# tomershay100/mp3-steganography-lib

Hardware: AMD Instinct MI355X
Metric: MP3 frames/sec (decode+re-encode) @44.1kHz stereo 128kbps, 1→8 GPU (higher is better)
Workload: dtype f64 (decode) / int32 (encode); 1 GPU; 10000-frame full decode->stego-embed->re-encode pipeline per MI355X (BASELINE configs[2]); MP3 main data + side info resident in HBM, MP3 frames out; the message cursor chain is decided and the serial chains of the rate loop are checked on the device inside every step; frames_per_gpu=10000, channels=2, message_bits=536, chain_verdict_units_to_redo=0, message_variant_entries=1874, parallelism=frames sharded over 1 GPU(s), no collective

## Files before the change

mp3-steganography-lib_amd/csrc/k_chain.hpp:

```cpp
#pragma once

namespace mp3s {

constexpr int CH_THREADS = 256;

struct ChainEl { int reset, tables, last[4]; };

__device__ __forceinline__ ChainEl chain_identity() { return ChainEl{0, 0, {-1, -1, -1, -1}}; }
__device__ __forceinline__ ChainEl chain_combine(const ChainEl &l, const ChainEl &r)
{
    if (r.reset) return r;
    ChainEl o;
    o.reset = l.reset;
    o.tables = l.tables + r.tables;
#pragma unroll
    for (int k = 0; k < 4; k++) o.last[k] = r.last[k] >= 0 ? r.last[k] : l.last[k];
    return o;
}
__device__ __forceinline__ ChainEl chain_shfl_up(const ChainEl &x, int d)
{
    ChainEl o;
    o.reset = __shfl_up(x.reset, d, 64);
    o.tables = __shfl_up(x.tables, d, 64);
#pragma unroll
    for (int k = 0; k < 4; k++) o.last[k] = __shfl_up(x.last[k], d, 64);
    return o;
}

__device__ __forceinline__ ChainEl chain_block_scan(ChainEl x, ChainEl (&wave_tot)[CH_THREADS / 64], ChainEl *total)
{
    const int lane = threadIdx.x & 63, wave = threadIdx.x >> 6;
#pragma unroll
    for (int d = 1; d < 64; d <<= 1) {
        const ChainEl o = chain_shfl_up(x, d);
        if (lane >= d) x = chain_combine(o, x);
    }
    __syncthreads();
    if (lane == 63) wave_tot[wave] = x;
    __syncthreads();
    ChainEl pre = chain_identity();
#pragma unroll
    for (int w = 0; w < CH_THREADS / 64; w++) {
        if (w < wave) pre = chain_combine(pre, wave_tot[w]);
    }
    x = chain_combine(pre, x);
    if (total) {
        ChainEl t = wave_tot[0];
#pragma unroll
        for (int w = 1; w < CH_THREADS / 64; w++) t = chain_combine(t, wave_tot[w]);
        *total = t;
    }
    return x;
}

__device__ __forceinline__ ChainEl chain_element(const mp3s_gr_out *__restrict__ gr, const mp3s_rate_frame *__restrict__ rf,
                                                 const mp3s_chain_seg *__restrict__ segs, int f, int n_frames)
{
    ChainEl e = chain_identity();
    if (f >= n_frames) return e;
    e.reset = segs[rf[f].stream].first_frame == f ? 1 : 0;
#pragma unroll
    for (int k = 0; k < 4; k++) {
        const mp3s_gr_out &g = gr[(long)f * 4 + k];
        if (g.flags & MP3S_RF_ACTIVE) { e.tables += g.n_tables; e.last[k] = f * 4 + k; }
    }
    return e;
}

__global__ __launch_bounds__(CH_THREADS) void k_chain_sum(const mp3s_gr_out *__restrict__ gr, const mp3s_rate_frame *__restrict__ rf,
                                                          const mp3s_chain_seg *__restrict__ segs, int n_frames,
                                                          ChainEl *__restrict__ agg, int32_t *__restrict__ verdict,
                                                          mp3s_chain_seg_out *__restrict__ seg_out, int32_t *__restrict__ redo,
                                                          const int32_t *__restrict__ only_after)
{
    __shared__ ChainEl wave_tot[CH_THREADS / 64];
    if (only_after && only_after[0] == 0) {
        if (redo && blockIdx.x == 0 && threadIdx.x == 0) redo[0] = 0;
        return;
    }
    const int f = blockIdx.x * CH_THREADS + threadIdx.x;
    if (f == 0) { verdict[0] = 0; verdict[1] = 0; }
    if (redo) {
        if (f == 0) redo[0] = 0;
        if (f == 0 && !only_after) redo[REDO_WORDS] = 0;
    }
    if (f < n_frames && segs[rf[f].stream].first_frame == f) seg_out[rf[f].stream].carry_used = 0;
    ChainEl total;
    chain_block_scan(chain_element(gr, rf, segs, f, n_frames), wave_tot, &total);
    if (threadIdx.x == 0) agg[blockIdx.x] = total;
}

__global__ __launch_bounds__(CH_THREADS) void k_chain_apply(mp3s_gr_out *__restrict__ gr, const mp3s_rate_frame *__restrict__ rf,
                                                            const mp3s_chain_seg *__restrict__ segs, int n_frames,
                                                            const ChainEl *__restrict__ agg, int32_t *__restrict__ cursor_in,
                                                            const int32_t *__restrict__ state_in, int32_t *__restrict__ verdict,
                                                            mp3s_chain_seg_out *__restrict__ seg_out, int32_t *__restrict__ redo_list,
                                                            const int32_t *__restrict__ only_after)
{
    if (only_after && only_after[0] == 0) return;
    __shared__ ChainEl wave_tot[CH_THREADS / 64];
    const int f = blockIdx.x * CH_THREADS + threadIdx.x;
    ChainEl before = chain_identity();
    for (int c0 = 0; c0 < (int)blockIdx.x; c0 += CH_THREADS) {
        const int j = c0 + (int)threadIdx.x;
        ChainEl total;
        chain_block_scan(j < (int)blockIdx.x ? agg[j] : chain_identity(), wave_tot, &total);
        before = chain_combine(before, total);
    }
    const ChainEl own_el = chain_element(gr, rf, segs, f, n_frames);
    const ChainEl incl = chain_block_scan(own_el, wave_tot, nullptr);
    ChainEl excl = chain_shfl_up(incl, 1);
    if ((threadIdx.x & 63) == 0) {
        excl = chain_identity();
        for (int w = 0; w < (int)(threadIdx.x >> 6); w++) excl = chain_combine(excl, wave_tot[w]);
    }
    excl = chain_combine(before, excl);
    int redo_here = 0, err_here = 0;
    if (f < n_frames) {
        const int s = rf[f].stream;
        const mp3s_chain_seg sg = segs[s];
        const bool first = sg.first_frame == f;
        if (first) excl = chain_identity();
        long cur = (long)sg.hide_begin + excl.tables;
        const long end = sg.hide_end;
        const bool hiding = sg.hide_end > sg.hide_base;
        int carry_used = first && cur < end ? 1 : 0;
#pragma unroll
        for (int k = 0; k < 4; k++) {
            const long u = (long)f * 4 + k;
            mp3s_gr_out &g = gr[u];
            int32_t ch[4];
            const bool own = excl.last[k] >= 0;
            if (own) {
                const mp3s_gr_out &p = gr[excl.last[k]];
                ch[0] = p.address[0]; ch[1] = p.address[1]; ch[2] = p.address[2]; ch[3] = p.quantizer_step;
            } else {
#pragma unroll
                for (int j = 0; j < 4; j++) ch[j] = sg.chain_in[k][j];
            }
            const int flags = g.flags;
            const bool active = flags & MP3S_RF_ACTIVE;
            if (!own && (!active || (flags & MP3S_RF_USED_ADDR_IN))) carry_used = 1;
            bool redo = false;
            if (hiding && active) {
                const long used = cursor_in[u];
                if (used != cur && (used < cur ? used : cur) < end) redo = true;
            }
            if (flags & MP3S_RF_USED_ADDR_IN) {
                const int32_t given = state_in ? state_in[u * 4] | (state_in[u * 4 + 1] << 10) | (state_in[u * 4 + 2] << 20) : g.reserved0;
                if (given != (ch[0] | (ch[1] << 10) | (ch[2] << 20))) redo = true;
            }
            redo_here += redo ? 1 : 0;
            if (redo && redo_list) {
                const int at = atomicAdd(&redo_list[0], 1);
                if (at < REDO_CAP) {
                    const int32_t c = (int32_t)(cur < (long)MP3S_NO_CURSOR ? cur : (long)MP3S_NO_CURSOR);
                    redo_list[REDO_HEAD + at] = (int32_t)u;
                    g.flags = flags | MP3S_RF_LISTED;
                    redo_list[REDO_HEAD + REDO_CAP + at] = hiding ? c : (cursor_in ? cursor_in[u] : 0);
                    if (hiding) cursor_in[u] = c;
#pragma unroll
                    for (int j = 0; j < 4; j++) redo_list[REDO_HEAD + 2 * REDO_CAP + 4 * at + j] = ch[j];
                }
            } else if (flags & MP3S_RF_LISTED) {
                g.flags = flags & ~MP3S_RF_LISTED;
            }
            if (flags & MP3S_RF_STEP_RANGE) err_here = 1;
            if (active) cur += g.n_tables;
            else {
                g.address[0] = ch[0]; g.address[1] = ch[1]; g.address[2] = ch[2];
                g.quantizer_step = ch[3];
            }
        }
        if (carry_used) atomicOr(&seg_out[s].carry_used, 1);
        if (f == sg.first_frame + sg.n_frames - 1) {
            seg_out[s].cursor = cur;
#pragma unroll
            for (int k = 0; k < 4; k++) {
                const mp3s_gr_out &g = gr[(long)f * 4 + k];
                seg_out[s].chain[k][0] = g.address[0]; seg_out[s].chain[k][1] = g.address[1];
                seg_out[s].chain[k][2] = g.address[2]; seg_out[s].chain[k][3] = g.quantizer_step;
            }
        }
    }
    const int n_redo = (int)wave_add_u32((uint32_t)redo_here);
    const bool any_err = __ballot(err_here != 0) != 0;
    if ((threadIdx.x & 63) == 0) {
        if (n_redo) atomicAdd(&verdict[0], n_redo);
        if (any_err) atomicOr(&verdict[1], 1);
    }
}

constexpr int SEL_THREADS = 1024, SEL_WAVES = SEL_THREADS / 64, SEL_D = 128;
constexpr int SEL_ROUND = SEL_THREADS;
constexpr int SEL_SAFE = 32;
constexpr int SEL_NONE = MP3S_SELECT_VARIANTS;

__host__ __device__ inline size_t select_lds_bytes(int reach)
{
    const int rs = reach < SEL_ROUND ? reach : SEL_ROUND;
    return (size_t)rs * (SEL_NONE + 1) + (size_t)(3 * rs + SEL_D + 8) + (size_t)rs + SEL_WAVES * SEL_D + 64;
}

__global__ __launch_bounds__(SEL_THREADS) void k_chain_select(const mp3s_chain_seg *__restrict__ segs, const mp3s_select_span *__restrict__ spans,
                                                              int max_reach, const uint8_t *__restrict__ hide,
                                                              const uint8_t *__restrict__ tabv, const mp3s_gr_out *__restrict__ out,
                                                              int32_t *__restrict__ cursor, int2 *__restrict__ pairs)
{
    extern __shared__ uint8_t sel_lds[];
    __shared__ int overflow, d_next, d_try, sat_round;
    const int s = blockIdx.x;
    const mp3s_select_span sp = spans[s];
    const int R = sp.reach;
    const int tid = threadIdx.x, lane = tid & 63, wave = __builtin_amdgcn_readfirstlane(tid >> 6);
    int2 *my_pairs = pairs + (long)s * max_reach;
    if (R <= 0) {
        for (int j = tid; j < max_reach; j += SEL_THREADS) my_pairs[j] = make_int2(-1, 0);
        return;
    }
    const mp3s_chain_seg sg = segs[s];
    const long c0 = sg.hide_begin, end = sg.hide_end;
    const long u0 = (long)sg.first_frame * 4;
    const int RS = min(R, SEL_ROUND);
    const long left = end - c0;
    const int tail = (int)MP3S_SELECT_TAIL_FIRST(left, (long)R), R2 = R - tail;
    const long row8 = (long)sp.first_entry + 8L * R - tail;
    uint8_t *tabs = sel_lds;
    uint8_t *code = tabs + (size_t)RS * (SEL_NONE + 1);
    uint8_t *delta = code + 3 * RS + SEL_D + 8;
    uint8_t *tot = delta + RS;
    if (tid == 0) { overflow = 0; d_next = 0; }
    int size = SEL_ROUND;
    for (int J = 0; J < R;) {
        __syncthreads();
        if (tid == 0) sat_round = 0;
        const int Rs = min(size, R - J);
        const int d0 = d_next;
        const long rel0 = 3L * J - d0 - (SEL_D - 1);
        if (c0 + rel0 >= end) {
            for (int jj = tid; jj < Rs; jj += SEL_THREADS) my_pairs[J + jj] = make_int2(-1, 0);
            J += Rs;
            continue;
        }
        for (int v = 0; v < 8; v++)
            for (int jj = tid; jj < Rs; jj += SEL_THREADS) tabs[v * RS + jj] = tabv[sp.first_entry + (long)v * R + J + jj];
        for (int v = 8; v < SEL_NONE; v++)
            for (int jj = tid; jj < Rs; jj += SEL_THREADS) tabs[v * RS + jj] = J + jj >= tail ? tabv[row8 + (long)(v - 8) * R2 + J + jj] : (uint8_t)0;
        for (int jj = tid; jj < Rs; jj += SEL_THREADS) tabs[SEL_NONE * RS + jj] = (uint8_t)out[u0 + J + jj].n_tables;
        for (int p = tid; p < 3 * Rs + SEL_D + 8; p += SEL_THREADS) {
            const long rel = rel0 + p, cur = c0 + rel;
            int v = SEL_NONE;
            if (rel >= 0) {
                if (cur + 3 <= end) v = (hide[cur] & 1) * 4 + (hide[cur + 1] & 1) * 2 + (hide[cur + 2] & 1);
                else if (cur == end - 2) v = 8;
                else if (cur == end - 1) v = 9;
            }
            code[p] = (uint8_t)v;
        }
        __syncthreads();
        auto step = [&](int jj, int d) -> int {
            const int v = code[3 * jj + (SEL_D - 1) - d];
            return v == SEL_NONE ? d : min(d + 3 - (int)tabs[v * RS + jj], SEL_D - 1);
        };
        const int chunk = (Rs + SEL_WAVES - 1) / SEL_WAVES, j0 = wave * chunk, j1 = min(Rs, j0 + chunk);
        {
            int m0 = lane, m1 = lane + 64;
            for (int jj = j0; jj < j1; jj++) { m0 = step(jj, m0); m1 = step(jj, m1); }
            tot[wave * SEL_D + lane] = (uint8_t)m0;
            tot[wave * SEL_D + 64 + lane] = (uint8_t)m1;
        }
        __syncthreads();
        {
            int d = 0;
            for (int w = 0; w < wave; w++) d = tot[w * SEL_D + d];
            bool sat = false;
            for (int jj = j0; jj < j1; jj++) {
                if (lane == 0) delta[jj] = (uint8_t)d;
                sat |= d >= SEL_D - 1;
                d = step(jj, d);
            }
            if (sat && lane == 0) sat_round = 1;
            if (wave == SEL_WAVES - 1 && lane == 0) d_try = d0 + d;
        }
        __syncthreads();
        if (sat_round) {
            if (size > SEL_SAFE) { size = SEL_SAFE; continue; }
            if (tid == 0) overflow = 1;
        }
        for (int jj = tid; jj < Rs; jj += SEL_THREADS) {
            const int p = 3 * jj + (SEL_D - 1) - (int)delta[jj];
            const int v = code[p];
            const int j = J + jj;
            if (v >= 8 && v != SEL_NONE && j < tail) overflow = 1;
            my_pairs[j] = v == SEL_NONE ? make_int2(-1, 0)
                                        : make_int2(v < 8 ? sp.first_entry + v * R + j : (int)(row8 + (long)(v - 8) * R2 + j), (int)(rel0 + p));
        }
        if (tid == 0) d_next = d_try;
        J += Rs;
        if (size == SEL_SAFE && J % SEL_ROUND == 0) size = SEL_ROUND;
    }
    __syncthreads();
    const bool bad = overflow != 0;
    for (int j = tid; j < max_reach; j += SEL_THREADS) {
        int src = -1;
        if (j < R && !bad) {
            const int2 pr = my_pairs[j];
            src = pr.x;
            if (src >= 0) cursor[u0 + j] = (int32_t)(c0 + pr.y);
        }
        my_pairs[j] = make_int2(src, (int)(u0 + j));
    }
}

}
```

mp3-steganography-lib_amd/csrc/k_rate.hpp:

```cpp
#pragma once
#ifndef MP3S_RL_STATS
#define MP3S_RL_STATS 0
#endif
#ifndef MP3S_RL_OCC
#define MP3S_RL_OCC 6
#endif
#if MP3S_RL_STATS
__device__ unsigned long long g_rl_stats[128];
extern "C" __attribute__((visibility("default"))) int mp3s_debug_rl_stats(unsigned long long *out, int clear)
{
    (void)hipDeviceSynchronize();
    int rc = (int)hipMemcpyFromSymbol(out, HIP_SYMBOL(g_rl_stats), sizeof(unsigned long long) * 128);
    if (clear) { unsigned long long z[128] = {}; rc |= (int)hipMemcpyToSymbol(HIP_SYMBOL(g_rl_stats), z, sizeof z); }
    return rc;
}
#define RL_STAT(i, v) do { if ((threadIdx.x & 63) == 0) atomicAdd(&g_rl_stats[(i)], (unsigned long long)(v)); } while (0)
#define RL_CLK() __builtin_readcyclecounter()
#else
#define RL_STAT(i, v) do { } while (0)
#endif

namespace mp3s {

#define RL_DPP(v, ctrl, rm) ((uint32_t)__builtin_amdgcn_update_dpp(0, (int)(v), ctrl, rm, 0xf, false))
// ... 359 lines not shown
    static_assert(offsetof(RlTables, hl) % 16 == 0 && offsetof(RlTables, subdiv) % 16 == 0 && sizeof(tb.subdiv) % 16 == 0, "16-byte pieces in LDS");
    constexpr int I2I_CHUNKS = (int)(sizeof(tb.int2idx) / 16), I2I_ROUNDS = (I2I_CHUNKS + RL_WAVES * 64 - 1) / (RL_WAVES * 64);
    constexpr int HL_CHUNKS = (int)(sizeof(tb.hl) / 16), SD_CHUNKS = (int)(sizeof(tb.subdiv) / 16);
    static_assert(HL_CHUNKS + SD_CHUNKS <= RL_WAVES * 64 && HL_CHUNKS % 64 == 0, "pair words and region table: one piece per thread");
    uint32_t t_c1w = 0, t_tr = 0;
    {
        typedef const __attribute__((address_space(1))) void *gsrc;
        typedef __attribute__((address_space(3))) void *ldst;
        char *const lds0 = reinterpret_cast<char *>(&tb);
        const char *const g_i2i = reinterpret_cast<const char *>(c_tab.int2idx);
#pragma unroll
        for (int r = 0; r < I2I_ROUNDS; r++) {
            const int base = (r * RL_WAVES + wave) * 64;
            if (base + lane < I2I_CHUNKS)
                __builtin_amdgcn_global_load_lds((gsrc)(g_i2i + (size_t)(base + lane) * 16), (ldst)(lds0 + offsetof(RlTables, int2idx) + base * 16), 16, 0, 0);
        }
        {
            const int base = wave * 64;
            const bool is_hl = base < HL_CHUNKS;
            const char *src = is_hl ? reinterpret_cast<const char *>(c_tab.rl_hl) + (size_t)(base + lane) * 16
                                    : reinterpret_cast<const char *>(c_tab.subdiv_lut[sr_wg]) + (size_t)(base - HL_CHUNKS + lane) * 16;
            char *dst = is_hl ? lds0 + offsetof(RlTables, hl) + base * 16 : lds0 + offsetof(RlTables, subdiv) + (base - HL_CHUNKS) * 16;
            if (is_hl || base - HL_CHUNKS + lane < SD_CHUNKS) __builtin_amdgcn_global_load_lds((gsrc)src, (ldst)dst, 16, 0, 0);
        }
        if (threadIdx.x < 16) t_c1w = c_tab.rl_c1w[threadIdx.x];
        if (threadIdx.x < 64) t_tr = c_tab.transform[threadIdx.x >> 1][threadIdx.x & 1];
    }
    auto tables_in = [&]() {
        if (threadIdx.x < 16) tb.c1w[threadIdx.x] = t_c1w;
        if (threadIdx.x < 64) tb.transform[threadIdx.x] = (uint8_t)t_tr;
        __builtin_amdgcn_s_waitcnt(0);
        __syncthreads();
    };
    if (CHAIN) tables_in();

    int li0 = blockIdx.x * RL_WAVES + wave;
    if (li0 >= n_total) { if (!CHAIN) tables_in(); return; }
    do {
    int li = li0;
    uint8_t *tables_out = nullptr;
    if (li >= n_list) {
        li -= n_list;
        tables_out = var.tables;
        unit_list = var.unit; cursor_in = var.cursor; state_in = nullptr;
        ix_out = var.ix; out = var.out; en_out = var.en;
        compact = 2;
    }
    int u = CHAIN ? __builtin_amdgcn_readfirstlane(unit_list ? unit_list[li] : li) : u_pre;
    if (u < 0 || u >= n_units) { if (CHAIN) continue; tables_in(); return; }
    bool chained = false;
    int ch_cursor = 0, ch_state[4] = {0, 0, 0, 0};
    for (int steps = 0; ; steps++) {
    if (CHAIN) __builtin_amdgcn_wave_barrier();
    const mp3s_rate_frame fr = frames[u >> 2];
    const int sr = sr_wg;
    const int max_bits = fr.max_bits;
    const int ci = compact ? li : u;
    const int cursor = chained ? ch_cursor : ((n_hide_all > 0 && cursor_in) ? cursor_in[ci] : 0);
    const int n_hide = min(n_hide_all, fr.hide_end);

    const int32_t *xr = mdct + (long)u * 576;
    uint32_t xa[2 * RL_NP];
    uint32_t negmask = 0, lmax = 0, esum = 0;
    uint32_t pk[2 * RL_NP - 1];
#pragma unroll
    for (int m = 0; m < RL_NP; m++) {
        const int p = p0 + m;
        int2 v = make_int2(0, 0);
        if (!CHAIN) v = xpre[m];
        else if (p < 288) v = *reinterpret_cast<const int2 *>(xr + 2 * p);
        const int32_t vv[2] = {v.x, v.y};
#pragma unroll
        for (int e = 0; e < 2; e++) {
            const uint32_t a = vv[e] < 0 ? (0u - (uint32_t)vv[e]) : (uint32_t)vv[e];
            xa[2 * m + e] = a;
            if (vv[e] < 0) negmask |= 1u << (2 * m + e);
            lmax = max(lmax, a);
            const int32_t sq = (int32_t)(((uint64_t)a * a + (1ull << 30)) >> 31);
            const int32_t e10 = sq >> 10;
            esum += (uint32_t)e10;
            if (2 * m + e < 2 * RL_NP - 1) pk[2 * m + e] = esum;
        }
    }
    uint32_t xrmax = lmax, etot = 0;
    {
        const uint32_t incl = wave_scan_u32(esum);
        etot = (uint32_t)__builtin_amdgcn_readlane((int)incl, 63);
        xrmax = wave_max_u32(lmax);
        const int bj = c_tab.sfb_long[sr][lane < 22 ? lane : 22];
        const int qj = (bj * 6554) >> 16, rj = bj - 10 * qj;
        uint32_t S = (uint32_t)__builtin_amdgcn_ds_bpermute(qj << 2, (int)(incl - esum)), part = 0;
#pragma unroll
        for (int k = 0; k < 2 * RL_NP - 1; k++) {
            const uint32_t v = (uint32_t)__builtin_amdgcn_ds_bpermute(qj << 2, (int)pk[k]);
            part = rj == k + 1 ? v : part;
        }
        S += part;
        const uint32_t Sn = (uint32_t)__builtin_amdgcn_update_dpp(0, (int)S, 0x130, 0xf, 0xf, false);
        const int32_t temp = lane < 21 ? (int32_t)(Sn - S) : (lane == 21 ? (int32_t)etot : 0);
        int32_t en = 0;
        if (lane < 22 && temp > 0) {
            const int k = 31 - __builtin_clz((unsigned)temp);
            en = c_tab.en_base[k] + (temp >= c_tab.en_step[k] ? 1 : 0);
        }
        if (lane < 22) en_out[(long)(compact == 2 ? li : u - out_base) * 22 + lane] = en;
        RlState st;
        st.big_values = st.count1 = st.c1sel = st.r0c = st.r1c = 0;
        const int in_a1 = __builtin_amdgcn_readfirstlane(chained ? ch_state[0] : (state_in ? state_in[(long)ci * 4 + 0] : 0));
        const int in_a2 = __builtin_amdgcn_readfirstlane(chained ? ch_state[1] : (state_in ? state_in[(long)ci * 4 + 1] : 0));
        const int in_a3 = __builtin_amdgcn_readfirstlane(chained ? ch_state[2] : (state_in ? state_in[(long)ci * 4 + 2] : 0));
        const int in_given = in_a1 | (in_a2 << 10) | (in_a3 << 20);
        st.a1 = in_a1; st.a2 = in_a2; st.a3 = in_a3;
        int qstep = chained ? ch_state[3] : (state_in ? state_in[(long)ci * 4 + 3] : 0);
        st.ts0 = st.ts1 = st.ts2 = 0;
        st.addr_fresh = false; st.used_addr_in = false;
        int32_t ix[2 * RL_NP];
#pragma unroll
        for (int e = 0; e < 2 * RL_NP; e++) ix[e] = 0;
        int bits = 0, flags = 0;
        bool err = false;

#if MP3S_RL_STATS
        const unsigned long long clk1 = RL_CLK();
#endif
        if (!CHAIN) tables_in();
#if MP3S_RL_STATS
        const unsigned long long clk2 = RL_CLK();
        unsigned long long clk3 = clk2, clk4 = clk2, clk5 = clk2;
        RL_STAT(54, clk1 - clk0); RL_STAT(55, clk2 - clk1); RL_STAT(60, 1);
        int probe_j = 0;
#endif
        if (xrmax) {
            flags |= MP3S_RF_ACTIVE;
            RL_STAT(35, 1);
            int next = -120, count = 120;
            int body_step = 1 << 20, body_bits = 0;
            uint32_t sc = rl_scale_of(next + count / 2);
            asm volatile("s_mov_b32 %0, %0" : "+s"(sc));
            {
                const uint32_t sc_lo = rl_scale_of(next + 30), sc_hi = rl_scale_of(next + 90);
                bool q_early;
                const int bit = rl_precheck(tb, xa, p0, st, next + 60, sc, xrmax, max_bits, q_early);
                if (bit >= 0) {
                    if (bit < max_bits) { count = 60; sc = sc_lo; }
                    else { next += 60; count -= 60; sc = sc_hi; }
                    asm volatile("s_mov_b32 %0, %0" : "+s"(sc));
#if MP3S_RL_STATS
                    RL_STAT(0 * 5 + 0, 1); RL_STAT(40, 1); RL_STAT(47, 1); probe_j = 1;
#endif
                }
            }
#if MP3S_RL_STATS
            clk3 = RL_CLK();
#endif
            do {
                const int half = count / 2;
                const uint32_t sc_lo = rl_scale_of(next + half / 2), sc_hi = rl_scale_of(next + half + (count - half) / 2);
                const int q = rl_quantize(tb, xa, ix, next + half, sc, xrmax);
                int bit;
                if (q < 0) { err = true; break; }
                if (q > 8192) { bit = 100000; if (q != 16384) body_step = 1 << 20; RL_STAT(probe_j * 5 + 1, 1); }
                else {
                    bool full;
                    bit = rl_body(tb, ix, p0, st, hide, n_hide, cursor, max_bits, half > 1, full);
                    if (full) { body_step = next + half; body_bits = bit; } else body_step = 1 << 20;
#if MP3S_RL_STATS
                    RL_STAT(probe_j * 5 + (full ? 4 : (bit >= max_bits ? 2 : 3)), 1);
                    RL_STAT(62, 1); if (st.count1 > 0) RL_STAT(61, 1);
#endif
                }
#if MP3S_RL_STATS
                if (bit >= max_bits) {
                    RlState st2 = st; bool qe;
                    const int pb = rl_precheck(tb, xa, p0, st2, next + half, sc, xrmax, max_bits, qe);
                    RL_STAT(40 + probe_j, 1); if (pb >= max_bits) RL_STAT(47 + probe_j, 1);
                }
                probe_j++;
#endif
                if (bit < max_bits) { count = half; sc = sc_lo; }
                else { next += half; count -= half; sc = sc_hi; }
            } while (count > 1);
            qstep = next;
#if MP3S_RL_STATS
            clk4 = RL_CLK();
#endif
            if (!err) {
                if (max_bits < 0) qstep -= 1;
                do {
                    if (qstep + 1 == body_step) {
                        qstep += 1;
                        bits = body_bits;
                        body_step = 1 << 20;
                        RL_STAT(37, 1);
                        continue;
                    }
                    int q;
                    while ((q = rl_quantize(tb, xa, ix, qstep + 1, rl_scale_of(qstep + 1), xrmax)) > 8192) qstep += 1;
                    if (q < 0) { err = true; break; }
                    qstep += 1;
                    bool full;
                    bits = rl_body(tb, ix, p0, st, hide, n_hide, cursor, max_bits + 1, false, full);
#if MP3S_RL_STATS
                    RL_STAT(36, 1); RL_STAT(full ? 39 : 38, 1); RL_STAT(62, 1); if (st.count1 > 0) RL_STAT(61, 1);
#endif
                } while (bits > max_bits);
            }
            if (err) flags |= MP3S_RF_STEP_RANGE;
#if MP3S_RL_STATS
            clk5 = RL_CLK();
            RL_STAT(56, clk3 - clk2); RL_STAT(57, clk4 - clk3); RL_STAT(58, clk5 - clk4);
#endif
        }
        if (st.used_addr_in) flags |= MP3S_RF_USED_ADDR_IN;
        if (CHAIN && !chained) flags |= MP3S_RF_LISTED;

        int16_t *ixo = ix_out + (long)(compact == 2 ? li : u - out_base) * 576;
#pragma unroll
        for (int m = 0; m < RL_NP; m++) {
            const int p = p0 + m;
            if (p < 288) {
                int a = xrmax ? ix[2 * m] : 0, b = xrmax ? ix[2 * m + 1] : 0;
                if ((negmask >> (2 * m)) & 1) a = -a;
                if ((negmask >> (2 * m + 1)) & 1) b = -b;
                *reinterpret_cast<uint32_t *>(ixo + 2 * p) = ((uint32_t)(uint16_t)(int16_t)a) | ((uint32_t)(uint16_t)(int16_t)b << 16);
            }
        }
        if (lane == 0) {
            mp3s_gr_out o;
            const bool act = xrmax != 0;
            o.part2_3_length = act ? bits : 0;
            o.big_values = act ? st.big_values : 0;
            o.count1 = act ? st.count1 : 0;
            o.quantizer_step = qstep;
            o.region0_count = act ? st.r0c : 0;
            o.region1_count = act ? st.r1c : 0;
            o.count1table_select = act ? st.c1sel : 0;
            o.table_select[0] = act ? st.ts0 : 0;
            o.table_select[1] = act ? st.ts1 : 0;
            o.table_select[2] = act ? st.ts2 : 0;
            o.address[0] = st.a1; o.address[1] = st.a2; o.address[2] = st.a3;
            o.n_tables = act ? (st.ts0 > 0) + (st.ts1 > 0) + (st.ts2 > 0) : 0;
            o.flags = flags;
            o.reserved0 = (state_in || chained) ? in_given : 0;
            o.xrmax = (int32_t)xrmax;
            o.reserved = 0;
            out[compact == 1 || compact == 2 ? li : u - out_base] = o;
            if (tables_out) tables_out[li] = (uint8_t)o.n_tables;
        }
#if MP3S_RL_STATS
        RL_STAT(59, RL_CLK() - clk5);
#endif
        if (!CHAIN) break;
        ch_state[0] = __builtin_amdgcn_readfirstlane(st.a1); ch_state[1] = __builtin_amdgcn_readfirstlane(st.a2);
        ch_state[2] = __builtin_amdgcn_readfirstlane(st.a3); ch_state[3] = __builtin_amdgcn_readfirstlane(qstep);
        bool go = false;
        int un = u;
        for (;;) {
            un += 4;
            if (++steps >= REDO_CHAIN_MAX || un >= n_units || frames[un >> 2].stream != fr.stream) break;
            const int f2 = __builtin_amdgcn_readfirstlane(__hip_atomic_load(&out[un - out_base].flags, __ATOMIC_RELAXED, __HIP_MEMORY_SCOPE_AGENT));
            if (f2 & MP3S_RF_LISTED) break;
            if (!(f2 & MP3S_RF_ACTIVE)) continue;
            const int given = __builtin_amdgcn_readfirstlane(__hip_atomic_load(&out[un - out_base].reserved0, __ATOMIC_RELAXED, __HIP_MEMORY_SCOPE_AGENT));
            go = (f2 & MP3S_RF_USED_ADDR_IN) && given != (ch_state[0] | (ch_state[1] << 10) | (ch_state[2] << 20));
            break;
        }
        if (!go) break;
        u = un; chained = true;
        ch_cursor = (n_hide_all > 0 && cursor_all) ? cursor_all[u] : 0;
    }
    }
    } while (CHAIN && (li0 += (int)gridDim.x * RL_WAVES) < n_total);
}

__global__ __launch_bounds__(RL_WAVES * 64, MP3S_RL_OCC) void k_rate_loop(
    const int32_t *__restrict__ mdct, const mp3s_rate_frame *__restrict__ frames, int n_units,
    const uint8_t *__restrict__ hide, int n_hide, const int32_t *__restrict__ cursor_in,
    const int32_t *__restrict__ state_in, const int32_t *__restrict__ unit_list, int n_list,
    int16_t *__restrict__ ix_out, mp3s_gr_out *__restrict__ out, int32_t *__restrict__ en_out, int out_base, int compact,
    RateVariants var)
{
    rate_units(mdct, frames, n_units, hide, n_hide, cursor_in, state_in, unit_list, n_list, ix_out, out, en_out, out_base, compact, var);
}

__global__ __launch_bounds__(RL_WAVES * 64, 4) void k_rate_redo(
    const int32_t *__restrict__ mdct, const mp3s_rate_frame *__restrict__ frames, int n_units,
    const uint8_t *__restrict__ hide, int n_hide, const int32_t *__restrict__ redo, int16_t *__restrict__ ix_out,
    mp3s_gr_out *__restrict__ out, int32_t *__restrict__ en_out, const int32_t *__restrict__ cursor_all)
{
    const int32_t *unit_list = redo + REDO_HEAD;
    const int n_list = min(__builtin_amdgcn_readfirstlane(__hip_atomic_load(&redo[0], __ATOMIC_RELAXED, __HIP_MEMORY_SCOPE_AGENT)), REDO_CAP);
    if ((int)blockIdx.x * RL_WAVES >= n_list) return;
    const RateVariants none = {nullptr, nullptr, 0, nullptr, nullptr, nullptr, nullptr};
    rate_units<true>(mdct, frames, n_units, hide, n_hide, unit_list + REDO_CAP, unit_list + 2 * REDO_CAP, unit_list, n_list, ix_out, out, en_out,
                  0, 3, none, cursor_all);
}

__global__ __launch_bounds__(256) void k_gather_tables(const mp3s_gr_out *__restrict__ outv, int n, uint8_t *__restrict__ tables)
{
    const int i = blockIdx.x * 256 + threadIdx.x;
    if (i < n) tables[i] = (uint8_t)outv[i].n_tables;
}

__global__ __launch_bounds__(256) void k_scatter_entries(const int2 *__restrict__ pairs, int n_pairs, const int16_t *__restrict__ ixv,
                                                         const int32_t *__restrict__ env, const mp3s_gr_out *__restrict__ outv,
                                                         int16_t *__restrict__ ix, int32_t *__restrict__ en, mp3s_gr_out *__restrict__ out)
{
    const int wave = __builtin_amdgcn_readfirstlane(threadIdx.x >> 6), lane = threadIdx.x & 63;
    const int j = blockIdx.x * 4 + wave;
    if (j >= n_pairs) return;
    const int2 pr = pairs[j];
    if (pr.x < 0) return;
    const long src = pr.x, dst = pr.y;
    const uint32_t *a = reinterpret_cast<const uint32_t *>(ixv + src * 576);
    uint32_t *b = reinterpret_cast<uint32_t *>(ix + dst * 576);
    for (int i = lane; i < 288; i += 64) b[i] = a[i];
    if (lane < 22) en[dst * 22 + lane] = env[src * 22 + lane];
    static_assert(sizeof(mp3s_gr_out) % 4 == 0, "GrInfo is copied by words");
    if (lane < (int)(sizeof(mp3s_gr_out) / 4))
        reinterpret_cast<uint32_t *>(out + dst)[lane] = reinterpret_cast<const uint32_t *>(outv + src)[lane];
}

}
```

mp3-steganography-lib_amd/csrc/mp3s_api.cpp:

```cpp
#include "mp3s_internal.h"

namespace {
thread_local std::string g_err;
}

int mp3s::fail(int code, const char *fmt, ...)
{
    char buf[512];
    va_list ap;
    va_start(ap, fmt);
    vsnprintf(buf, sizeof buf, fmt, ap);
    va_end(ap);
    g_err = buf;
    return code;
}

int max_part2_3(const mp3s_frame_side *side, long n)
{
    int m = 0;
    for (long f = 0; f < n; f++)
        for (int k = 0; k < 4; k++) m = std::max<int>(m, side[f].unit[k >> 1][k & 1].part2_3_length);
    return m;
}

void select_entries(int first_unit, int reach, int first_entry, int hide_end, int64_t bits_left, int32_t *ent_unit, int32_t *ent_cursor)
{
    const int tail = (int)MP3S_SELECT_TAIL_FIRST(bits_left, (int64_t)reach);
    int at = first_entry;
    for (int v = 0; v < MP3S_SELECT_VARIANTS; v++) {
        const int32_t cur = v < 8 ? 4 * v : hide_end - (10 - v);
        for (int j = v < 8 ? 0 : tail; j < reach; j++) {
            ent_unit[at] = first_unit + j;
            ent_cursor[at++] = cur;
        }
    }
}

extern "C" {

const char *mp3s_last_error(void) { return g_err.c_str(); }
const char *mp3s_version(void) { return "mp3s-hip 0.1 (gfx950)"; }
void mp3s_buf_free(mp3s_buf *b) { delete b; }
const void *mp3s_debug_tables(size_t *bytes)
{
    if (bytes) *bytes = sizeof(DevTables);
    return &host_tables().dev;
}

int mp3s_debug_scfsi_energies(const int32_t *xr576, int sr_idx, int32_t *en22)
{
    if (!xr576 || !en22 || sr_idx < 0 || sr_idx > 2) return fail(MP3S_E_ARG, "bad argument");
    host_scfsi_energies(xr576, sr_idx, en22);
    return MP3S_OK;
}

int mp3s_debug_parse_scanned_frame(const void *frame_side, const uint8_t *blob, int16_t *is2304, mp3s_granule_si *si4)
{
    if (!frame_side || !blob || !is2304 || !si4) return fail(MP3S_E_ARG, "null pointer");
    const int rc = parse_scanned_frame(*static_cast<const mp3s_frame_side *>(frame_side), blob, is2304, si4);
    return rc ? fail(rc, "malformed main data") : MP3S_OK;
}

int mp3s_debug_walk_rate(const uint8_t *file, size_t len, double seconds, double *frames_per_s, int64_t *frames_per_pass)
{
    if (!file || !frames_per_s || seconds <= 0) return fail(MP3S_E_ARG, "bad argument");
    std::vector<FrameRef> refs(len / 24 + 16);
    std::vector<uint8_t> tables(refs.size() * 4);
    const double t0 = now_ms();
    int64_t frames = 0, per_pass = 0;
    double t = t0;
    do {
        FrameWalker w;
        if (w.open(file, len)) return fail(MP3S_E_MALFORMED, "malformed or unsupported MP3 stream");
        w.tables_wanted = 1000;
        long n = 0;
        while (!w.ended && !w.irregular && (size_t)n < refs.size()) n += w.next(refs.data() + n, (long)refs.size() - n, tables.data() + (size_t)n * 4, 0, 0);
        if (w.irregular) return fail(MP3S_E_UNSUPPORTED, "not a stream the walk takes");
        frames += n; per_pass = n;
        t = now_ms();
    } while (t - t0 < seconds * 1e3);
    *frames_per_s = (double)frames / ((t - t0) * 1e-3);
    if (frames_per_pass) *frames_per_pass = per_pass;
    return MP3S_OK;
}

int mp3s_device_count(int *n)
{
    if (!n) return fail(MP3S_E_ARG, "n is null");
    int k = 0;
    *n = hipGetDeviceCount(&k) == hipSuccess && k > 0 ? k : 0;
    return MP3S_OK;
}

int mp3s_ctx_create(int device, mp3s_ctx **out)
{
    if (!out) return fail(MP3S_E_ARG, "out is null");
    *out = nullptr;
    int n = 0;
    hipError_t e = hipGetDeviceCount(&n);
    if (e != hipSuccess || n <= 0)
        return fail(MP3S_E_NO_DEVICE, "no HIP device available (%s); the transforms have no CPU fallback",
                    e == hipSuccess ? "device count 0" : hipGetErrorString(e));
    if (device < 0 || device >= n) return fail(MP3S_E_ARG, "device %d out of range (0..%d)", device, n - 1);
    e = hipSetDevice(device);
    if (e != hipSuccess) return fail(MP3S_E_NO_DEVICE, "hipSetDevice(%d): %s", device, hipGetErrorString(e));
    mp3s_ctx *c = new mp3s_ctx();
    c->device = device;
    {
        auto env = [](const char *name, int64_t dflt) { const char *v = getenv(name); return v && *v ? (int64_t)atoll(v) : dflt; };
        c->opt[MP3S_OPT_SELECT] = getenv("MP3S_NO_SELECT") ? 0 : 1;
        c->opt[MP3S_OPT_REDO] = getenv("MP3S_NO_REDO") ? 0 : 1;
        c->opt[MP3S_OPT_FAST_IMDCT] = env("MP3S_FAST_IMDCT", 1) != 0;
        c->opt[MP3S_OPT_PIPE_TAIL] = std::min<int64_t>(2, std::max<int64_t>(0, env("MP3S_PIPE_TAIL", 1)));
        c->opt[MP3S_OPT_CHUNK_FRAMES] = std::max<int64_t>(0, env("MP3S_CHUNK_FRAMES", 0));
        c->opt[MP3S_OPT_DEVICE_PARSE] = env("MP3S_DEVICE_PARSE", 1) != 0;
        c->opt[MP3S_OPT_FILE_PIPELINE] = env("MP3S_FILE_PIPELINE", 1) != 0;
        c->opt[MP3S_OPT_SCAN_THREADS] = std::max<int64_t>(0, env("MP3S_SCAN_THREADS", 0));
        c->opt[MP3S_OPT_FIRST_CHUNK_FRAMES] = std::max<int64_t>(0, env("MP3S_FIRST_CHUNK_FRAMES", 0));
        c->opt[MP3S_OPT_FILE_UP] = getenv("MP3S_NO_FILE_UP") ? 0 : 1;
        c->opt[MP3S_OPT_HUF_LANES] = std::max<int64_t>(0, env("MP3S_HUF_LANES", 0));
        c->opt[MP3S_OPT_NUMA] = getenv("MP3S_NO_NUMA") ? 0 : 1;
        c->opt[MP3S_OPT_FLOAT_FAST] = env("MP3S_FLOAT_FAST", 0) != 0;
        c->opt[MP3S_OPT_FAIL_CHUNK] = 0;
        c->opt[MP3S_OPT_FUSED_DECODE] = env("MP3S_FUSED_DECODE", 1) != 0;
        c->opt[MP3S_OPT_FUSED_ENCODE] = env("MP3S_FUSED_ENCODE", 0) != 0;
        c->opt[MP3S_OPT_PIPE_DEC] = env("MP3S_PIPE_DEC", 0) != 0;
        c->opt[MP3S_OPT_RATE_SIGNALS] = env("MP3S_RATE_SIGNALS", 0) != 0;
        c->opt[MP3S_OPT_PIPE_SIGNALS] = env("MP3S_PIPE_SIGNALS", 0) & 3;
    }
    if (hipStreamCreateWithFlags(&c->stream, hipStreamNonBlocking) != hipSuccess ||
        hipEventCreate(&c->ev0) != hipSuccess || hipEventCreate(&c->ev1) != hipSuccess ||
        hipEventCreateWithFlags(&c->ev_order, hipEventDisableTiming) != hipSuccess) {
        mp3s_ctx_destroy(c);
        return fail(MP3S_E_NO_DEVICE, "stream/event creation failed");
    }
    if (hipMalloc((void **)&c->d_sync, 32) != hipSuccess || hipMemsetAsync(c->d_sync, 0, 32, c->stream) != hipSuccess) {
        mp3s_ctx_destroy(c);
        return fail(MP3S_E_NO_DEVICE, "device scratch allocation failed");
    }
    const int rc = dev_upload_tables(c->stream);
    if (rc) {
        mp3s_ctx_destroy(c);
        return fail(MP3S_E_NO_DEVICE, "constant table upload failed: %s (is this a gfx950 device?)",
                    hipGetErrorString((hipError_t)rc));
    }
    *out = c;
    return MP3S_OK;
}

void mp3s_ctx_destroy(mp3s_ctx *c)
{
    if (!c) return;
    hipSetDevice(c->device);
    destroy_own_pipe(c);
    if (c->stream) hipStreamSynchronize(c->stream);
    if (c->scratch) hipFree(c->scratch);
    if (c->scratch_enc) hipFree(c->scratch_enc);
    if (c->d_sync) hipFree(c->d_sync);
    for (void *q : c->pool) if (q) hipFree(q);
    if (c->ev0) hipEventDestroy(c->ev0);
    if (c->ev1) hipEventDestroy(c->ev1);
    if (c->ev_order) hipEventDestroy(c->ev_order);
    if (c->ev_sel) hipEventDestroy(c->ev_sel);
    if (c->stream) hipStreamDestroy(c->stream);
    delete c;
}

int mp3s_ctx_host_share(mp3s_ctx *c, mp3s_host_share *out)
{
    if (!out) return fail(MP3S_E_ARG, "null pointer");
    size_t held = 0, cap = 0;
    PinnedBlock::pool_state(&held, &cap);
    out->pinned_pooled_bytes = held; out->pinned_pool_cap_bytes = cap;
    out->local_world_size = local_world_size();
    out->cpus_allowed = host_cpus_allowed();
    out->gpu_node_cpus = c ? (int32_t)gpu_node_cpus(c->device).size() : 0;
    out->reserved = 0;
    return MP3S_OK;
}

int mp3s_ctx_set_option(mp3s_ctx *c, int option, int64_t value)
{
    if (!c || option <= 0 || option >= MP3S_OPT_COUNT) return fail(MP3S_E_ARG, "unknown option %d", option);
    if (value < 0 || ((option == MP3S_OPT_CHUNK_FRAMES || option == MP3S_OPT_FIRST_CHUNK_FRAMES) && value != 0 && value < 4) || (option == MP3S_OPT_SCAN_THREADS && value > 64))
        return fail(MP3S_E_ARG, "option %d: value %lld out of range", option, (long long)value);
    const bool number = option == MP3S_OPT_CHUNK_FRAMES || option == MP3S_OPT_SCAN_THREADS || option == MP3S_OPT_FIRST_CHUNK_FRAMES ||
                        option == MP3S_OPT_HUF_LANES || option == MP3S_OPT_FAIL_CHUNK || option == MP3S_OPT_PIPE_SIGNALS;
    c->opt[option] = number ? value : (option == MP3S_OPT_PIPE_TAIL ? std::min<int64_t>(value, 2) : (value != 0));
    return MP3S_OK;
}

int mp3s_ctx_run_stats(mp3s_ctx *c, mp3s_run_stats *out)
{
    if (!c || !out) return fail(MP3S_E_ARG, "null pointer");
    *out = c->run_stats;
    own_pipe_lanes(c, out);
    return MP3S_OK;
}

int mp3s_ctx_get_option(mp3s_ctx *c, int option, int64_t *value)
{
    if (!c || !value || option <= 0 || option >= MP3S_OPT_COUNT) return fail(MP3S_E_ARG, "unknown option %d", option);
    *value = c->opt[option];
    return MP3S_OK;
}

int mp3s_device_name(mp3s_ctx *c, char *buf, size_t n)
{
    if (!c || !buf || !n) return fail(MP3S_E_ARG, "bad argument");
    hipDeviceProp_t p;
    HIPCHK(hipGetDeviceProperties(&p, c->device));
    snprintf(buf, n, "%s (%s, %d CUs)", p.name, p.gcnArchName, p.multiProcessorCount);
    return MP3S_OK;
}

int mp3s_device_pci(mp3s_ctx *c, char *buf, size_t n)
{
    if (!c || !buf || n < 16) return fail(MP3S_E_ARG, "bad argument");
    HIPCHK(hipDeviceGetPCIBusId(buf, (int)n, c->device));
    for (char *p = buf; *p; p++) *p = (char)tolower(*p);
    return MP3S_OK;
}

int mp3s_sync(mp3s_ctx *c)
{
    if (!c) return fail(MP3S_E_ARG, "ctx is null");
    HIPCHK(hipStreamSynchronize(c->stream));
    return MP3S_OK;
}

int mp3s_ctx_wait(mp3s_ctx *c, mp3s_ctx *other)
{
    if (!c || !other) return fail(MP3S_E_ARG, "ctx is null");
    if (c == other) return MP3S_OK;
    if (c->device != other->device) return fail(MP3S_E_ARG, "contexts on different devices");
    HIPCHK(hipEventRecord(other->ev_order, other->stream));
    HIPCHK(hipStreamWaitEvent(c->stream, other->ev_order, 0));
    return MP3S_OK;
}

int mp3s_ctx_wait_last(mp3s_ctx *c, mp3s_ctx *other)
{
    if (!c || !other) return fail(MP3S_E_ARG, "ctx is null");
    if (c == other) return MP3S_OK;
    if (c->device != other->device) return fail(MP3S_E_ARG, "contexts on different devices");
    HIPCHK(hipStreamWaitEvent(c->stream, other->ev_order, 0));
    return MP3S_OK;
}

int mp3s_dev_alloc(mp3s_ctx *c, size_t bytes, void **dptr)
{
    if (!c || !dptr) return fail(MP3S_E_ARG, "bad argument");
    HIPCHK(hipSetDevice(c->device));
    hipError_t e = hipMalloc(dptr, bytes ? bytes : 16);
    if (e != hipSuccess) return fail(MP3S_E_NOMEM, "hipMalloc(%zu): %s", bytes, hipGetErrorString(e));
    return MP3S_OK;
}
int mp3s_dev_free(mp3s_ctx *c, void *dptr)
{
    if (!c) return fail(MP3S_E_ARG, "ctx is null");
    if (dptr) { HIPCHK(hipStreamSynchronize(c->stream)); HIPCHK(hipFree(dptr)); }
    return MP3S_OK;
}
int mp3s_dev_upload(mp3s_ctx *c, void *dptr, const void *host, size_t bytes)
{
    if (!c || (!dptr && bytes) || (!host && bytes)) return fail(MP3S_E_ARG, "bad argument");
    if (!bytes) return MP3S_OK;
    HIPCHK(hipMemcpyAsync(dptr, host, bytes, hipMemcpyHostToDevice, c->stream));
    HIPCHK(hipStreamSynchronize(c->stream));
    return MP3S_OK;
}
int mp3s_dev_download(mp3s_ctx *c, void *host, const void *dptr, size_t bytes)
{
    if (!c || (!dptr && bytes) || (!host && bytes)) return fail(MP3S_E_ARG, "bad argument");
    if (!bytes) return MP3S_OK;
    HIPCHK(hipMemcpyAsync(host, dptr, bytes, hipMemcpyDeviceToHost, c->stream));
    HIPCHK(hipStreamSynchronize(c->stream));
    return MP3S_OK;
}
int mp3s_dev_memset(mp3s_ctx *c, void *dptr, int value, size_t bytes)
{
    if (!c || !dptr) return fail(MP3S_E_ARG, "bad argument");
    HIPCHK(hipMemsetAsync(dptr, value, bytes, c->stream));
    return MP3S_OK;
}
int mp3s_dev_copy(mp3s_ctx *c, void *d_dst, const void *d_src, size_t bytes)
{
    if (!c || !d_dst || !d_src) return fail(MP3S_E_ARG, "bad argument");
    if (bytes) HIPCHK(hipMemcpyAsync(d_dst, d_src, bytes, hipMemcpyDeviceToDevice, c->stream));
    return MP3S_OK;
}
int mp3s_timer_start(mp3s_ctx *c)
{
    if (!c) return fail(MP3S_E_ARG, "ctx is null");
    HIPCHK(hipEventRecord(c->ev0, c->stream));
    return MP3S_OK;
}
int mp3s_timer_stop(mp3s_ctx *c, float *ms)
{
    if (!c || !ms) return fail(MP3S_E_ARG, "bad argument");
    HIPCHK(hipEventRecord(c->ev1, c->stream));
    HIPCHK(hipEventSynchronize(c->ev1));
    HIPCHK(hipEventElapsedTime(ms, c->ev0, c->ev1));
    return MP3S_OK;
}

int mp3s_synth_mode(mp3s_ctx *c, double eps_scale, int64_t *exact_samples)
{
    if (!c || eps_scale < 0) return fail(MP3S_E_ARG, "bad argument");
    HIPCHK(hipStreamSynchronize(c->stream));
    int32_t n = 0;
    HIPCHK(hipMemcpy(&n, c->d_sync + 2, 4, hipMemcpyDeviceToHost));
    HIPCHK(hipMemset(c->d_sync + 2, 0, 4));
    if (exact_samples) *exact_samples = n;
    c->synth_eps_scale = eps_scale;
    return MP3S_OK;
}

int mp3s_bench_copy(mp3s_ctx *c, size_t bytes, int iters, double *gb_per_s)
{
    if (!c || !gb_per_s || bytes < 4096 || iters < 1) return fail(MP3S_E_ARG, "bad argument");
    HIPCHK(hipSetDevice(c->device));
    bytes &= ~(size_t)15;
    void *a = nullptr, *b = nullptr;
    if (hipMalloc(&a, bytes) != hipSuccess || hipMalloc(&b, bytes) != hipSuccess) { if (a) hipFree(a); return fail(MP3S_E_NOMEM, "hipMalloc(%zu) x 2", bytes); }
    int rc = MP3S_OK;
    float ms = 0;
    if (hipMemsetAsync(a, 1, bytes, c->stream) != hipSuccess || launch_copy(c->stream, a, b, bytes) != 0) rc = fail(MP3S_E_HIP, "copy launch failed");
    if (!rc && hipEventRecord(c->ev0, c->stream) != hipSuccess) rc = fail(MP3S_E_HIP, "event");
    for (int i = 0; i < iters && !rc; i++) if (launch_copy(c->stream, i & 1 ? b : a, i & 1 ? a : b, bytes) != 0) rc = fail(MP3S_E_HIP, "copy launch failed");
    if (!rc && (hipEventRecord(c->ev1, c->stream) != hipSuccess || hipEventSynchronize(c->ev1) != hipSuccess ||
                hipEventElapsedTime(&ms, c->ev0, c->ev1) != hipSuccess)) rc = fail(MP3S_E_HIP, "event");
    hipStreamSynchronize(c->stream);
    hipFree(a); hipFree(b);
    if (!rc) *gb_per_s = 2.0 * (double)bytes * iters / (ms * 1e-3) / 1e9;
    return rc;
}

int mp3s_profile_enable(mp3s_ctx *c, int on)
{
    if (!c) return fail(MP3S_E_ARG, "ctx is null");
    HIPCHK(hipStreamSynchronize(c->stream));
    c->prof.enabled = on != 0;
    c->prof.n_pairs = 0;
    for (int k = 0; k < K_COUNT; k++) { c->prof.total_ms[k] = 0; c->prof.count[k] = 0; }
    return MP3S_OK;
}

int mp3s_profile_select(mp3s_ctx *c, unsigned mask)
{
    if (!c) return fail(MP3S_E_ARG, "ctx is null");
    c->prof.mask = mask;
    return MP3S_OK;
}

int mp3s_profile_collect(mp3s_ctx *c, double *total_ms, int64_t *launches, int n)
{
    if (!c || !total_ms || !launches || n < K_COUNT) return fail(MP3S_E_ARG, "bad argument (need %d slots)", (int)K_COUNT);
    HIPCHK(hipStreamSynchronize(c->stream));
    Profiler &p = c->prof;
    for (int i = 0; i < p.n_pairs; i++) {
        float ms = 0;
        HIPCHK(hipEventElapsedTime(&ms, p.ev[2 * i], p.ev[2 * i + 1]));
        p.total_ms[p.kid[i]] += ms;
        p.count[p.kid[i]] += 1;
    }
    p.n_pairs = 0;
    if (p.dropped) {
        const long lost = p.dropped;
        p.dropped = 0;
        return fail(MP3S_E_ARG, "%ld timed launches had no event pair left (collect at least every %d launches)", lost, Profiler::MAX_PAIRS);
    }
    for (int k = 0; k < K_COUNT; k++) { total_ms[k] = p.total_ms[k]; launches[k] = p.count[k]; }
    static_assert(K_COUNT == MP3S_N_KERNELS, "kernel list out of sync with mp3s.h");
    return MP3S_OK;
}

int mp3s_decode_transform_dev(mp3s_ctx *c, const int16_t *d_is, const mp3s_granule_si *d_si, const mp3s_frame_hdr *d_hdr,
                              int n_frames, int nch, int n_halo, int out_format, void *d_pcm)
{
    if (!c || !d_is || !d_si || !d_hdr || !d_pcm) return fail(MP3S_E_ARG, "null pointer");
    if (n_frames <= 0 || nch < 1 || nch > 2 || n_halo < 0 || n_halo >= n_frames || out_format < 0 || out_format > 2)
        return fail(MP3S_E_ARG, "bad sizes: n_frames=%d nch=%d n_halo=%d fmt=%d", n_frames, nch, n_halo, out_format);
    int rc = c->ensure_scratch(dec_scratch_bytes(n_frames, nch));
    if (rc) return rc;
    if (int pe = guard_probe_usable(c, out_format)) return pe;
    const int e = launch_decode(c->stream, d_is, d_si, d_hdr, n_frames, nch, n_halo, out_format, d_pcm, c->scratch, &c->prof, 0,
                                c->synth_eps_scale, c->d_sync, c->opt[MP3S_OPT_FAST_IMDCT] != 0, c->opt[MP3S_OPT_FLOAT_FAST] != 0,
                                c->opt[MP3S_OPT_FUSED_DECODE] != 0, nullptr, [&]() -> const GuardProbe * {
                                    if (!c->guard_probe.x) return nullptr;
                                    c->guard_probe.base = 0;
                                    return &c->guard_probe; }());
    if (e) return fail(MP3S_E_HIP, "decode launch: %s", hipGetErrorString((hipError_t)e));
    return MP3S_OK;
}

int mp3s_debug_guard_margin(mp3s_ctx *c, double *d_x, double *d_eps, int64_t capacity)
{
    if (!c) return fail(MP3S_E_ARG, "null context");
    if ((d_x == nullptr) != (d_eps == nullptr) || (d_x && capacity <= 0)) return fail(MP3S_E_ARG, "both arrays and their capacity, or neither");
    HIPCHK(hipStreamSynchronize(c->stream));
    c->guard_probe = GuardProbe{d_x, d_eps, 0, d_x ? capacity : 0};
    return MP3S_OK;
}



static int check_hdr(const mp3s_frame_hdr *hdr, int n)
{
    for (int f = 0; f < n; f++) {
        if (hdr[f].stream_first > (uint32_t)f) return fail(MP3S_E_ARG, "hdr[%d].stream_first=%u points forward", f, hdr[f].stream_first);
        if (f && hdr[f].stream_first != (uint32_t)f && hdr[f].stream_first != hdr[f - 1].stream_first)
            return fail(MP3S_E_ARG, "hdr[%d].stream_first is not monotone", f);
        if (hdr[f].sr_idx > 2) return fail(MP3S_E_ARG, "hdr[%d].sr_idx=%d", f, hdr[f].sr_idx);
    }
    if (n && hdr[0].stream_first != 0) return fail(MP3S_E_ARG, "hdr[0].stream_first must be 0");
    return 0;
}

int mp3s_decode_transform(mp3s_ctx *c, const int16_t *is, const mp3s_granule_si *si, const mp3s_frame_hdr *hdr,
                          int n_frames, int nch, int n_halo, int out_format, void *pcm)
{
    if (!c || !is || !si || !hdr || !pcm) return fail(MP3S_E_ARG, "null pointer");
    if (n_frames <= 0 || n_halo < 0 || n_halo >= n_frames) return fail(MP3S_E_ARG, "bad sizes");
    int rc = check_hdr(hdr, n_frames);
    if (rc) return rc;
    for (size_t i = 0; i < (size_t)n_frames * 2304; i++)
        if (is[i] > 8206 || is[i] < -8206) return fail(MP3S_E_ARG, "is[%zu]=%d outside +-8206", i, is[i]);
    HIPCHK(hipSetDevice(c->device));
    void *d_is = nullptr, *d_si = nullptr, *d_hdr = nullptr, *d_pcm = nullptr;
    const size_t b_is = (size_t)n_frames * 2304 * 2, b_si = (size_t)n_frames * 4 * sizeof(mp3s_granule_si),
                 b_hdr = (size_t)n_frames * sizeof(mp3s_frame_hdr),
                 b_pcm = (size_t)(n_frames - n_halo) * 1152 * nch * pcm_elem(out_format);
    rc = MP3S_OK;
    if (hipMalloc(&d_is, b_is) != hipSuccess || hipMalloc(&d_si, b_si) != hipSuccess ||
        hipMalloc(&d_hdr, b_hdr) != hipSuccess || hipMalloc(&d_pcm, b_pcm) != hipSuccess)
        rc = fail(MP3S_E_NOMEM, "hipMalloc failed for a %d-frame batch", n_frames);
    if (!rc) rc = mp3s_dev_upload(c, d_is, is, b_is);
    if (!rc) rc = mp3s_dev_upload(c, d_si, si, b_si);
    if (!rc) rc = mp3s_dev_upload(c, d_hdr, hdr, b_hdr);
    if (!rc) rc = mp3s_decode_transform_dev(c, (const int16_t *)d_is, (const mp3s_granule_si *)d_si,
                                            (const mp3s_frame_hdr *)d_hdr, n_frames, nch, n_halo, out_format, d_pcm);
    if (!rc) rc = mp3s_dev_download(c, pcm, d_pcm, b_pcm);
    hipStreamSynchronize(c->stream);
    hipFree(d_is); hipFree(d_si); hipFree(d_hdr); hipFree(d_pcm);
    return rc;
}

int mp3s_encode_transform_dev(mp3s_ctx *c, const int16_t *d_pcm, const mp3s_frame_hdr *d_hdr, int n_frames, int32_t *d_mdct)
{
    if (!c || !d_pcm || !d_hdr || !d_mdct) return fail(MP3S_E_ARG, "null pointer");
    if (n_frames <= 0) return fail(MP3S_E_ARG, "n_frames=%d", n_frames);
    if (!host_tables().analysis_plan_ok)
        return fail(MP3S_E_TABLES, "the analysis filter table built on this host does not repeat itself where the kernel shares products "
                                   "(csrc/analysis_plan.h: run tools/gen_analysis_plan.py here and rebuild)");
    const bool fused = c->opt[MP3S_OPT_FUSED_ENCODE] != 0;
    int rc = fused ? MP3S_OK : c->ensure_scratch_enc(enc_scratch_bytes(n_frames));
    if (rc) return rc;
    const int e = launch_encode(c->stream, d_pcm, d_hdr, n_frames, d_mdct, c->scratch_enc, &c->prof, fused);
    if (e) return fail(MP3S_E_HIP, "encode launch: %s", hipGetErrorString((hipError_t)e));
    return MP3S_OK;
}

int mp3s_encode_transform(mp3s_ctx *c, const int16_t *pcm, const mp3s_frame_hdr *hdr, int n_frames, int32_t *mdct)
{
    if (!c || !pcm || !hdr || !mdct) return fail(MP3S_E_ARG, "null pointer");
    if (n_frames <= 0) return fail(MP3S_E_ARG, "n_frames=%d", n_frames);
    int rc = check_hdr(hdr, n_frames);
    if (rc) return rc;
    HIPCHK(hipSetDevice(c->device));
    void *d_pcm = nullptr, *d_hdr = nullptr, *d_mdct = nullptr;
    const size_t b_pcm = (size_t)n_frames * 1152 * 2 * 2, b_hdr = (size_t)n_frames * sizeof(mp3s_frame_hdr),
                 b_mdct = (size_t)n_frames * 2304 * 4;
    if (hipMalloc(&d_pcm, b_pcm) != hipSuccess || hipMalloc(&d_hdr, b_hdr) != hipSuccess ||
        hipMalloc(&d_mdct, b_mdct) != hipSuccess)
        rc = fail(MP3S_E_NOMEM, "hipMalloc failed for a %d-frame batch", n_frames);
    if (!rc) rc = mp3s_dev_upload(c, d_pcm, pcm, b_pcm);
    if (!rc) rc = mp3s_dev_upload(c, d_hdr, hdr, b_hdr);
    if (!rc) rc = mp3s_encode_transform_dev(c, (const int16_t *)d_pcm, (const mp3s_frame_hdr *)d_hdr, n_frames, (int32_t *)d_mdct);
    if (!rc) rc = mp3s_dev_download(c, mdct, d_mdct, b_mdct);
    hipStreamSynchronize(c->stream);
    hipFree(d_pcm); hipFree(d_hdr); hipFree(d_mdct);
    return rc;
}

int mp3s_rate_loop_dev(mp3s_ctx *c, const int32_t *d_mdct, const mp3s_rate_frame *d_frames, int n_frames,
                       const uint8_t *d_hide_bits, int n_hide, const int32_t *d_cursor_in, const int32_t *d_state_in,
                       const int32_t *d_unit_list, int n_list, int16_t *d_ix, mp3s_gr_out *d_out, int32_t *d_en)
{
    if (!c || !d_mdct || !d_frames || !d_ix || !d_out || !d_en) return fail(MP3S_E_ARG, "null pointer");
    if (n_frames <= 0 || n_hide < 0 || (n_hide > 0 && (!d_hide_bits || !d_cursor_in)))
        return fail(MP3S_E_ARG, "bad sizes / missing hide inputs");
    const int e = launch_rate(c->stream, d_mdct, d_frames, n_frames, d_hide_bits, n_hide, d_cursor_in, d_state_in,
                              d_unit_list, n_list, d_ix, d_out, d_en, &c->prof, 0, 0, nullptr,
                              c->rate_done ? c->rate_done : (c->opt[MP3S_OPT_RATE_SIGNALS] ? c->ev_order : nullptr));
    if (e) return fail(MP3S_E_HIP, "rate launch: %s", hipGetErrorString((hipError_t)e));
    return MP3S_OK;
}



void mp3s_select_patterns(uint8_t out[32])
{
    for (int v = 0; v < 8; v++) { out[4 * v] = (v >> 2) & 1; out[4 * v + 1] = (v >> 1) & 1; out[4 * v + 2] = v & 1; out[4 * v + 3] = 0; }
}

int mp3s_select_plan(const mp3s_chain_seg *segs, int n_segs, mp3s_select_span *spans, int32_t *ent_unit, int32_t *ent_cursor, int cap)
{
    return select_plan(segs, n_segs, spans, ent_unit, ent_cursor, cap, nullptr);
}

}

int select_plan(const mp3s_chain_seg *segs, int n_segs, mp3s_select_span *spans, int32_t *ent_unit, int32_t *ent_cursor, int cap,
                const int32_t *min_reach)
{
    if (!segs || !spans || n_segs <= 0 || cap < 0 || ((ent_unit == nullptr) != (ent_cursor == nullptr))) return fail(MP3S_E_ARG, "bad argument");
    int used = 0;
    for (int i = 0; i < n_segs; i++) {
        const mp3s_chain_seg &g = segs[i];
        spans[i].first_entry = used; spans[i].reach = 0;
        const int64_t left = (int64_t)g.hide_end - g.hide_begin;
        if (left <= 0 || g.n_frames <= 0 || g.hide_base < 32) continue;
        const int64_t reach = std::min<int64_t>((int64_t)g.n_frames * 4, std::max<int64_t>(left * 5 / 14 + 32, min_reach ? min_reach[i] : 0));
        if (reach > MP3S_SELECT_MAX_REACH || (int64_t)used + MP3S_SELECT_ENTRIES(left, reach) > cap) continue;
        spans[i].reach = (int32_t)reach;
        if (ent_unit) select_entries(g.first_frame * 4, (int)reach, used, g.hide_end, left, ent_unit, ent_cursor);
        used += (int)MP3S_SELECT_ENTRIES(left, reach);
    }
    return used;
}

extern "C" {

int mp3s_rate_variants_dev(mp3s_ctx *c, const int32_t *d_mdct, const mp3s_rate_frame *d_frames, int n_frames, const uint8_t *d_hide_bits,
                           int n_hide, const int32_t *d_cursor, const int32_t *d_ent_unit, const int32_t *d_ent_cursor, int n_entries,
                           int16_t *d_ix, mp3s_gr_out *d_out, int32_t *d_en, int16_t *d_ixv, mp3s_gr_out *d_outv, int32_t *d_env)
{
    if (!c || !d_mdct || !d_frames || !d_ix || !d_out || !d_en || !d_hide_bits || !d_cursor || !d_ent_unit || !d_ent_cursor || !d_ixv ||
        !d_outv || !d_env)
        return fail(MP3S_E_ARG, "null pointer");
    if (n_frames <= 0 || n_hide < 32 || n_entries <= 0) return fail(MP3S_E_ARG, "bad sizes");
    if (c->sel_pending && hipStreamWaitEvent(c->stream, c->ev_sel, 0) != hipSuccess) return fail(MP3S_E_HIP, "ordering behind the previous selection failed");
    c->sel_pending = false;
    const RateVariantArgs va = {d_ent_unit, d_ent_cursor, n_entries, d_ixv, d_outv, d_env, (uint8_t *)(d_outv + n_entries)};
    const int e = launch_rate(c->stream, d_mdct, d_frames, n_frames, d_hide_bits, n_hide, d_cursor, nullptr, nullptr, 0, d_ix, d_out, d_en,
                              &c->prof, 0, 0, &va, c->rate_done ? c->rate_done : (c->opt[MP3S_OPT_RATE_SIGNALS] ? c->ev_order : nullptr));
    if (e) return fail(MP3S_E_HIP, "rate launch: %s", hipGetErrorString((hipError_t)e));
    return MP3S_OK;
}

int mp3s_select_dev(mp3s_ctx *c, const uint8_t *d_hide_bits, int32_t *d_cursor, const mp3s_chain_seg *d_segs, const mp3s_select_span *d_spans,
                    int n_segs, int max_reach, const int32_t *d_ent_unit, const int32_t *d_ent_cursor, int n_entries, int16_t *d_ix,
                    mp3s_gr_out *d_out, int32_t *d_en, int16_t *d_ixv, mp3s_gr_out *d_outv, int32_t *d_env)
{
    if (!c || !d_ix || !d_out || !d_en || !d_hide_bits || !d_cursor || !d_segs || !d_spans || !d_ent_unit || !d_ent_cursor || !d_ixv ||
        !d_outv || !d_env)
        return fail(MP3S_E_ARG, "null pointer");
    if (n_segs <= 0 || n_entries <= 0 || max_reach <= 0 || max_reach > MP3S_SELECT_MAX_REACH) return fail(MP3S_E_ARG, "bad sizes");
    const RateVariantArgs va = {d_ent_unit, d_ent_cursor, n_entries, d_ixv, d_outv, d_env, (uint8_t *)(d_outv + n_entries)};
    void *d_pairs = c->grab(29, (size_t)n_segs * max_reach * 8);
    if (!d_pairs) return fail(MP3S_E_NOMEM, "hipMalloc failed for the selection scratch");
    const int e = launch_select(c->stream, d_segs, d_spans, n_segs, max_reach, d_hide_bits, va, d_ix, d_en, d_out, d_cursor, d_pairs, &c->prof);
    if (e) return fail(MP3S_E_HIP, "select launch: %s", hipGetErrorString((hipError_t)e));
    return MP3S_OK;
}

int mp3s_rate_select_dev(mp3s_ctx *c, const int32_t *d_mdct, const mp3s_rate_frame *d_frames, int n_frames, const uint8_t *d_hide_bits,
                         int n_hide, int32_t *d_cursor, const mp3s_chain_seg *d_segs, const mp3s_select_span *d_spans, int n_segs,
                         int max_reach, const int32_t *d_ent_unit, const int32_t *d_ent_cursor, int n_entries, int16_t *d_ix,
                         mp3s_gr_out *d_out, int32_t *d_en, int16_t *d_ixv, mp3s_gr_out *d_outv, int32_t *d_env)
{
    if (!d_segs || !d_spans) return fail(MP3S_E_ARG, "null pointer");
    if (n_segs <= 0 || max_reach <= 0 || max_reach > MP3S_SELECT_MAX_REACH) return fail(MP3S_E_ARG, "bad sizes");
    const int rc = mp3s_rate_variants_dev(c, d_mdct, d_frames, n_frames, d_hide_bits, n_hide, d_cursor, d_ent_unit, d_ent_cursor, n_entries, d_ix,
                                          d_out, d_en, d_ixv, d_outv, d_env);
    if (rc) return rc;
    return mp3s_select_dev(c, d_hide_bits, d_cursor, d_segs, d_spans, n_segs, max_reach, d_ent_unit, d_ent_cursor, n_entries, d_ix, d_out, d_en,
                           d_ixv, d_outv, d_env);
}

int mp3s_chain_resolve_dev(mp3s_ctx *c, mp3s_gr_out *d_gr, const mp3s_rate_frame *d_frames, int n_frames, const mp3s_chain_seg *d_segs,
                           int n_segs, const int32_t *d_cursor_in, const int32_t *d_state_in, int32_t *d_verdict,
                           mp3s_chain_seg_out *d_seg_out)
{
    if (!c || !d_gr || !d_frames || !d_segs || !d_verdict || !d_seg_out) return fail(MP3S_E_ARG, "null pointer");
    if (n_frames <= 0 || n_segs <= 0) return fail(MP3S_E_ARG, "bad sizes");
    void *d_agg = c->grab(30, chain_agg_bytes(n_frames));
    if (!d_agg) return fail(MP3S_E_NOMEM, "hipMalloc failed for the chain scratch");
    const int e = launch_chain(c->stream, d_gr, d_frames, n_frames, d_segs, d_cursor_in, d_state_in, d_agg, d_verdict, d_seg_out, &c->prof);
    if (e) return fail(MP3S_E_HIP, "chain launch: %s", hipGetErrorString((hipError_t)e));
    return MP3S_OK;
}

int mp3s_chain_redo_dev(mp3s_ctx *c, const int32_t *d_mdct, const mp3s_rate_frame *d_frames, int n_frames, const uint8_t *d_hide_bits, int n_hide,
                        int32_t *d_cursor, const mp3s_chain_seg *d_segs, int n_segs, int16_t *d_ix, mp3s_gr_out *d_gr, int32_t *d_en,
                        int32_t *d_verdict, mp3s_chain_seg_out *d_seg_out)
{
    if (!c || !d_mdct || !d_gr || !d_frames || !d_segs || !d_verdict || !d_seg_out || !d_ix || !d_en) return fail(MP3S_E_ARG, "null pointer");
    if (n_frames <= 0 || n_segs <= 0 || n_hide < 0 || (n_hide > 0 && (!d_hide_bits || !d_cursor))) return fail(MP3S_E_ARG, "bad sizes");
    void *d_agg = c->grab(30, chain_agg_bytes(n_frames));
    if (!d_agg) return fail(MP3S_E_NOMEM, "hipMalloc failed for the chain scratch");
    const ChainRedoArgs redo = {d_mdct, d_hide_bits, n_hide, d_ix, d_en};
    const int e = launch_chain(c->stream, d_gr, d_frames, n_frames, d_segs, d_cursor, nullptr, d_agg, d_verdict, d_seg_out, &c->prof, &redo);
    if (e) return fail(MP3S_E_HIP, "chain launch: %s", hipGetErrorString((hipError_t)e));
    return MP3S_OK;
}

int mp3s_huffman_decode_dev(mp3s_ctx *c, const uint8_t *d_blob, const mp3s_frame_side *d_side, int n_frames, int nch,
                            int max_part2_3_length, int16_t *d_is, mp3s_granule_si *d_si, int32_t *d_status)
{
    if (!c || !d_blob || !d_side || !d_is || !d_si || !d_status) return fail(MP3S_E_ARG, "null pointer");
    if (n_frames <= 0 || nch < 1 || nch > 2 || max_part2_3_length < 0) return fail(MP3S_E_ARG, "bad sizes");
    if (max_part2_3_length == 0 || max_part2_3_length > 4095) max_part2_3_length = 4095;
    const int e = launch_huffman(c->stream, d_blob, d_side, n_frames, nch, max_part2_3_length, d_is, d_si, d_status, c->d_sync + 4, &c->prof, false, (int)c->opt[MP3S_OPT_HUF_LANES]);
    if (e) return fail(MP3S_E_HIP, "huffman launch: %s", hipGetErrorString((hipError_t)e));
    return MP3S_OK;
}

int mp3s_pack_frames_dev(mp3s_ctx *c, const int16_t *d_ix, const mp3s_gr_out *d_gr, const int32_t *d_en, int n_frames,
                         int samplerate, int bitrate_kbps, const uint32_t *d_frame_off, const uint8_t *d_padding,
                         uint8_t *d_mp3, int32_t *d_scfsi, int32_t *d_status)
{
    if (!c || !d_ix || !d_gr || !d_en || !d_frame_off || !d_padding || !d_mp3 || !d_scfsi || !d_status)
        return fail(MP3S_E_ARG, "null pointer");
    int sri, bri, whole;
    if (n_frames <= 0 || stream_params(samplerate, bitrate_kbps, &sri, &bri, &whole))
        return fail(MP3S_E_UNSUPPORTED, "unsupported samplerate/bitrate %d/%d", samplerate, bitrate_kbps);
    const int e = launch_pack(c->stream, d_ix, d_gr, d_en, n_frames, sri, bri, whole, d_frame_off, d_padding, d_mp3, d_scfsi,
                              d_status, c->d_sync, &c->prof);
    if (e) return fail(MP3S_E_HIP, "pack launch: %s", hipGetErrorString((hipError_t)e));
    return MP3S_OK;
}

int mp3s_scan_stream(const uint8_t *file, size_t len, mp3s_buf **owner, mp3s_scanned *out)
{
    if (!file || !owner || !out) return fail(MP3S_E_ARG, "null pointer");
    mp3s_buf *b = new mp3s_buf();
    const int rc = parse_stream(file, len, b->parsed, &b->scanned);
    if (rc) { delete b; return fail(rc, "malformed or unsupported MP3 stream"); }
    const ParsedStream &p = b->parsed;
    out->n_frames = p.n_frames; out->nch = p.nch; out->sampling_rate = p.sampling_rate; out->bit_rate = p.bit_rate;
    out->n_bits = (int32_t)p.bits.size(); out->dup_last_frame = p.dup_last_frame;
    out->gpu_ok = b->scanned.gpu_ok ? 1 : 0;
    out->max_part2_3_length = max_part2_3(b->scanned.side.data(), p.n_frames);
    out->side = b->scanned.side.data(); out->hdr = p.hdr.data();
    out->blob = b->scanned.blob.data(); out->blob_len = b->scanned.blob.size();
    out->bits = p.bits.data(); out->frame_size = p.frame_size.data();
    *owner = b;
    return MP3S_OK;
}

int mp3s_walk_stream(const uint8_t *file, size_t len, mp3s_buf **owner, mp3s_walked *out)
{
    if (!file || !owner || !out) return fail(MP3S_E_ARG, "null pointer");
    std::memset(out, 0, sizeof *out);
    std::unique_ptr<mp3s_buf> b(new mp3s_buf());
    FrameWalker w;
    const int rc = w.open(file, len);
    if (rc) return fail(rc, "malformed or unsupported MP3 stream");
    const size_t cap = len / 24 + 16;
    b->bytes.resize(cap * 20);
    FrameRef *refs = reinterpret_cast<FrameRef *>(b->bytes.data());
    uint8_t *tables = b->bytes.data() + cap * 16;
    std::memset(tables, 0, cap * 4);
    w.tables_wanted = 0x7fffffffffffffffL;
    long n = 0;
    while (!w.ended && !w.irregular && (size_t)n < cap) n += w.next(refs + n, (long)(cap - (size_t)n), tables + (size_t)n * 4, 0, 0);
    *owner = b.release();
    if (w.irregular || !w.ended) return MP3S_OK;
    out->regular = 1;
    out->n_frames = (int32_t)n; out->nch = w.nch; out->sampling_rate = w.sampling_rate; out->bit_rate = w.bit_rate;
    out->dup_last_frame = w.dup_last ? 1 : 0; out->max_part2_3_length = w.max_p23; out->any_silent = w.any_silent ? 1 : 0;
    out->blob_len = n > 0 ? (size_t)refs[n - 1].md_off + refs[n - 1].md_len + 8 : 0; out->refs = refs; out->tables = tables;
    out->stream.base = 0; out->stream.end = (uint32_t)len; out->stream.first_frame = 0; out->stream.n_frames = (uint32_t)n;
    if (n > 0) FrameWalker::history(refs, 0, out->stream.prev_size);
    return MP3S_OK;
}

int mp3s_parse_frames_dev(mp3s_ctx *c, const uint8_t *d_image, uint32_t image_base, const mp3s_frame_ref *d_refs, const mp3s_stream_ref *d_streams,
                          int n_frames, uint32_t md_base, mp3s_frame_side *d_side, mp3s_frame_hdr *d_hdr, uint8_t *d_blob, uint64_t *d_tsel,
                          int32_t *d_status)
{
    if (!c || !d_image || !d_refs || !d_streams || !d_side || !d_hdr || !d_blob || !d_status) return fail(MP3S_E_ARG, "null pointer");
    if (n_frames <= 0) return fail(MP3S_E_ARG, "n_frames=%d", n_frames);
    const int e = launch_parse(c->stream, d_image, image_base, d_refs, d_streams, n_frames, md_base, d_side, d_hdr, d_blob, d_tsel, d_status);
    if (e) return fail(MP3S_E_HIP, "parse launch: %s", hipGetErrorString((hipError_t)e));
    return MP3S_OK;
}

int mp3s_stego_bits(const uint64_t *tsel, int64_t n_frames, int nch, uint8_t carry[4], mp3s_buf **owner, const uint8_t **bits, size_t *n_bits)
{
    if ((!tsel && n_frames) || n_frames < 0 || nch < 1 || nch > 2 || !carry || !owner || !bits || !n_bits) return fail(MP3S_E_ARG, "bad argument");
    mp3s_buf *b = new mp3s_buf();
    stego_bits_from_tsel(tsel, (long)n_frames, nch, carry, b->bits);
    *bits = b->bits.data(); *n_bits = b->bits.size(); *owner = b;
    return MP3S_OK;
}

int mp3s_parse_stream(const uint8_t *file, size_t len, mp3s_buf **owner, mp3s_parsed *out)
{
    if (!file || !owner || !out) return fail(MP3S_E_ARG, "null pointer");
    mp3s_buf *b = new mp3s_buf();
    const int rc = parse_stream(file, len, b->parsed);
    if (rc) { delete b; return fail(rc, "malformed or unsupported MP3 stream"); }
    const ParsedStream &p = b->parsed;
    out->n_frames = p.n_frames; out->nch = p.nch; out->sampling_rate = p.sampling_rate; out->bit_rate = p.bit_rate;
    out->n_bits = (int32_t)p.bits.size(); out->dup_last_frame = p.dup_last_frame;
    out->is = p.is.data(); out->si = p.si.data(); out->hdr = p.hdr.data(); out->bits = p.bits.data();
    out->table_select = p.table_select.data(); out->frame_size = p.frame_size.data();
    *owner = b;
    return MP3S_OK;
}

int mp3s_rate_frames(int samplerate, int bitrate_kbps, int nch, int n_frames, mp3s_rate_frame *out, int32_t *padding)
{
    if (!out || n_frames < 0) return fail(MP3S_E_ARG, "bad argument");
    const int rc = rate_frames(samplerate, bitrate_kbps, nch, n_frames, out, padding);
    if (rc) return fail(rc, "unsupported samplerate/bitrate %d/%d", samplerate, bitrate_kbps);
    return MP3S_OK;
}

int mp3s_format_stream(int samplerate, int bitrate_kbps, int n_frames, const int16_t *ix, const mp3s_gr_out *gr,
                       const int32_t *scfsi, mp3s_buf **owner, const uint8_t **mp3, size_t *mp3_len)
{
    if (!ix || !gr || !scfsi || !owner || !mp3 || !mp3_len) return fail(MP3S_E_ARG, "null pointer");
    mp3s_buf *b = new mp3s_buf();
    const int rc = format_stream(samplerate, bitrate_kbps, n_frames, ix, gr, scfsi, b->bytes);
    if (rc) { delete b; return fail(rc, "format_stream failed"); }
    *owner = b; *mp3 = b->bytes.data(); *mp3_len = b->bytes.size();
    return MP3S_OK;
}

int mp3s_wav_parse(const uint8_t *file, size_t len, int bitrate_kbps, mp3s_wav_info *out)
{
    if ((!file && len) || !out) return fail(MP3S_E_ARG, "null pointer");
    const char *msg = "";
    const int rc = wav_parse(file, len, bitrate_kbps, out, &msg);
    return rc ? fail(rc, "%s", msg) : MP3S_OK;
}

int mp3s_wav_header(int64_t n_rows, int nch, int rate, uint8_t *out44)
{
    if (!out44 || n_rows < 0 || nch < 1 || nch > 2 || rate < 0) return fail(MP3S_E_ARG, "bad argument");
    wav_header(n_rows, nch, rate, out44);
    return MP3S_OK;
}

int mp3s_message_frame(const uint8_t *utf8, size_t n, mp3s_buf **owner, const uint8_t **bits, size_t *n_bits)
{
    if ((!utf8 && n) || !owner || !bits || !n_bits) return fail(MP3S_E_ARG, "null pointer");
    mp3s_buf *b = new mp3s_buf();
    message_frame(utf8, n, b->bits);
    *bits = b->bits.data(); *n_bits = b->bits.size(); *owner = b;
    return MP3S_OK;
}

int mp3s_message_reveal(const uint8_t *bits, size_t n_bits, mp3s_buf **owner, const uint8_t **text, size_t *n_text)
{
    if ((!bits && n_bits) || !owner || !text || !n_text) return fail(MP3S_E_ARG, "null pointer");
    mp3s_buf *b = new mp3s_buf();
    message_reveal(bits, n_bits, b->bytes);
    *text = b->bytes.data(); *n_text = b->bytes.size(); *owner = b;
    return MP3S_OK;
}

int mp3s_reveal_message(const uint8_t *mp3, size_t len, mp3s_buf **owner, mp3s_file *out)
{
    if (!mp3 || !owner || !out) return fail(MP3S_E_ARG, "null pointer");
    mp3s_buf *b = new mp3s_buf();
    const int rc = parse_stream(mp3, len, b->parsed, &b->scanned);
    if (rc) { delete b; return fail(rc, "malformed or unsupported MP3 stream"); }
    message_reveal(b->parsed.bits.data(), b->parsed.bits.size(), b->bytes);
    std::memset(out, 0, sizeof *out);
    out->data = b->bytes.data(); out->len = b->bytes.size();
    out->kbps = b->parsed.bit_rate / 1000; out->sampling_rate = b->parsed.sampling_rate; out->channels = b->parsed.nch;
    out->n_frames = b->parsed.n_frames; out->n_bits = (int32_t)b->parsed.bits.size(); out->bits = b->parsed.bits.data();
    *owner = b;
    return MP3S_OK;
}

}
```

mp3-steganography-lib_amd/csrc/mp3s_device.h:

```cpp
#pragma once
#include <hip/hip_runtime_api.h>
#include <stddef.h>
#include <stdint.h>

#include "../../include/mp3s.h"

namespace mp3s {

#ifndef MP3S_DEC_SYNTH_TW
#define MP3S_DEC_SYNTH_TW 2
#endif
constexpr int DEC_SYNTH_TW = MP3S_DEC_SYNTH_TW;
constexpr int DEC_SYNTH_FAST_TW = 2;

enum KernelId { K_DEC_IMDCT = 0, K_DEC_SYNTH, K_ENC_ANALYSIS, K_ENC_MDCT, K_RATE_LOOP, K_DEC_HUFFMAN, K_ENC_PACK, K_CHAIN, K_COUNT };
struct Profiler {
    static constexpr int MAX_PAIRS = 8192;
    hipEvent_t ev[2 * MAX_PAIRS];
    int kid[MAX_PAIRS];
    int n_pairs = 0, n_created = 0;
    long dropped = 0;
    bool enabled = false;
    unsigned mask = ~0u;
    double total_ms[K_COUNT] = {0};
    long count[K_COUNT] = {0};
    int begin(hipStream_t s, int k);
    void end(hipStream_t s, int pair);
    bool attach(int k, hipEvent_t *start, hipEvent_t *stop);
};

int dev_upload_tables(hipStream_t stream);

struct GuardProbe { double *x, *eps; int64_t base, cap; };
size_t dec_scratch_bytes(int n_frames, int nch);
int launch_decode(hipStream_t stream, const int16_t *d_is, const mp3s_granule_si *d_si, const mp3s_frame_hdr *d_hdr,
                  int n_frames, int nch, int n_halo, int out_format, void *d_pcm, void *d_scratch, Profiler *prof,
                  int sf_base = 0 ,
                  double synth_eps_scale = 1.0 ,
                  int32_t *d_sync = nullptr ,
                  bool fast_imdct = true ,
                  bool float_fast = false ,
                  bool fused = true ,
                  hipEvent_t done = nullptr ,
                  const GuardProbe *probe = nullptr );

size_t enc_scratch_bytes(int n_frames);
int launch_encode(hipStream_t stream, const int16_t *d_pcm, const mp3s_frame_hdr *d_hdr, int n_frames, int32_t *d_mdct,
                  void *d_scratch, Profiler *prof, bool fused = false );

struct RateVariantArgs {
    const int32_t *d_unit, *d_cursor;
    int n;
    int16_t *d_ix; mp3s_gr_out *d_out; int32_t *d_en;
    uint8_t *d_tables;
};
inline size_t variant_out_bytes(int n) { return (size_t)n * sizeof(mp3s_gr_out) + (((size_t)n + 15) & ~(size_t)15); }
int launch_rate(hipStream_t stream, const int32_t *d_mdct, const mp3s_rate_frame *d_frames, int n_frames,
                const uint8_t *d_hide, int n_hide, const int32_t *d_cursor, const int32_t *d_state,
                const int32_t *d_list, int n_list, int16_t *d_ix, mp3s_gr_out *d_out, int32_t *d_en, Profiler *prof,
                int out_base = 0 ,
                int compact = 0 ,
                const RateVariantArgs *variants = nullptr,
                hipEvent_t done = nullptr );

struct ChainRedoArgs { const int32_t *d_mdct; const uint8_t *d_hide; int n_hide; int16_t *d_ix; int32_t *d_en; };
size_t chain_agg_bytes(int n_frames);
int launch_chain(hipStream_t stream, mp3s_gr_out *d_gr, const mp3s_rate_frame *d_frames, int n_frames, const mp3s_chain_seg *d_segs,
                 const int32_t *d_cursor, const int32_t *d_state, void *d_agg, int32_t *d_verdict, mp3s_chain_seg_out *d_seg_out,
                 Profiler *prof, const ChainRedoArgs *redo = nullptr);

int launch_select(hipStream_t stream, const mp3s_chain_seg *d_segs, const mp3s_select_span *d_spans, int n_segs, int max_reach,
                  const uint8_t *d_hide, const RateVariantArgs &v, int16_t *d_ix, int32_t *d_en, mp3s_gr_out *d_out, int32_t *d_cursor,
                  void *d_pairs , Profiler *prof);

using FrameRef = mp3s_frame_ref;
using StreamRef = mp3s_stream_ref;
constexpr int kParseInherits = 1, kParseMismatch = 2;
int launch_parse(hipStream_t stream, const uint8_t *d_image, uint32_t image_base, const FrameRef *d_refs, const StreamRef *d_streams, int n_frames,
                 uint32_t md_base, mp3s_frame_side *d_side, mp3s_frame_hdr *d_hdr, uint8_t *d_blob, uint64_t *d_tsel, int32_t *d_status);

struct WavRun { uint64_t src; uint32_t first_frame, n_frames; };
constexpr size_t kWavSlack = 32;
int launch_wav_gather(hipStream_t stream, const uint8_t *d_image, const WavRun *d_runs, int n_runs, int max_frames , int16_t *d_pcm);

constexpr size_t kPlaceEntry = 4912;
int launch_place_frames(hipStream_t stream, const uint8_t *d_entries, int n_entries, int16_t *d_is, mp3s_granule_si *d_si);
int launch_copy(hipStream_t stream, const void *d_src, void *d_dst, size_t bytes);
int launch_spin(hipStream_t stream, int microseconds);
int launch_noop(hipStream_t stream);

int launch_huffman(hipStream_t stream, const uint8_t *d_blob, const mp3s_frame_side *d_side, int n_frames, int nch, int max_bits,
                   int16_t *d_is, mp3s_granule_si *d_si, int32_t *d_status, int32_t *d_sync ,
                   Profiler *prof,
                   bool per_frame = false ,
                   int lanes_opt = 0 );
int launch_gather_tables(hipStream_t stream, const mp3s_gr_out *d_outv, int n, uint8_t *d_tables);
int launch_scatter(hipStream_t stream, const int32_t *d_pairs, int n_pairs, const int16_t *d_ixv, const int32_t *d_env,
                   const mp3s_gr_out *d_outv, int16_t *d_ix, int32_t *d_en, mp3s_gr_out *d_out);
int launch_pack(hipStream_t stream, const int16_t *d_ix, const mp3s_gr_out *d_gr, const int32_t *d_en, int n_frames, int sri,
                int bri, int whole_slots, const uint32_t *d_frame_off, const uint8_t *d_padding, uint8_t *d_mp3,
                int32_t *d_scfsi, int32_t *d_status, int32_t *d_sync , Profiler *prof,
                int f_begin = 0, int f_end = -1 );

}
```

mp3-steganography-lib_amd/csrc/mp3s_device.hip:

```cpp
#include <hip/hip_runtime.h>
#include <hip/hip_ext.h>
#include <atomic>
#include <stdint.h>
#include <stdlib.h>

#include "../../include/mp3s.h"
#include "mp3s_device.h"
#include "mp3s_host.h"
#include "mp3s_tables.h"

namespace mp3s {
__constant__ DevTables c_tab;
}

#include "k_sync.hpp"
#include "k_decode.hpp"
#include "k_decode_stream.hpp"
#include "k_encode.hpp"
#include "k_rate.hpp"
#include "k_huffman.hpp"
#include "k_parse.hpp"
#include "k_pack.hpp"
#include "k_chain.hpp"
#include "k_wav.hpp"

namespace mp3s {

int Profiler::begin(hipStream_t s, int k)
{
    if (!enabled || !((mask >> k) & 1u)) return -1;
    if (n_pairs >= MAX_PAIRS) { dropped++; return -1; }
    while (n_created < 2 * (n_pairs + 1)) {
        if (hipEventCreate(&ev[n_created]) != hipSuccess) { dropped++; return -1; }
        n_created++;
    }
    kid[n_pairs] = k;
    (void)hipEventRecord(ev[2 * n_pairs], s);
    return n_pairs++;
}
void Profiler::end(hipStream_t s, int pair)
{
    if (pair >= 0) (void)hipEventRecord(ev[2 * pair + 1], s);
}
bool Profiler::attach(int k, hipEvent_t *start, hipEvent_t *stop)
{
    if (!enabled || !((mask >> k) & 1u)) return false;
    if (n_pairs >= MAX_PAIRS) { dropped++; return false; }
    while (n_created < 2 * (n_pairs + 1)) {
        if (hipEventCreate(&ev[n_created]) != hipSuccess) { dropped++; return false; }
        n_created++;
    }
    kid[n_pairs] = k;
    *start = ev[2 * n_pairs]; *stop = ev[2 * n_pairs + 1];
    n_pairs++;
    return true;
}

int dev_upload_tables(hipStream_t stream)
{
    const HostTables &h = host_tables();
    hipError_t e = hipMemcpyToSymbolAsync(HIP_SYMBOL(c_tab), &h.dev, sizeof(DevTables), 0, hipMemcpyHostToDevice, stream);
    if (e != hipSuccess) return (int)e;
    return (int)hipStreamSynchronize(stream);
}

static size_t dec_S_bytes(int n_frames, int nch) { return (size_t)nch * (size_t)n_frames * 36 * 32 * sizeof(double); }
static size_t dec_G_bytes(int n_frames) { return (size_t)n_frames * 2 * 2 * sizeof(double); }
size_t dec_scratch_bytes(int n_frames, int nch)
{
    return dec_S_bytes(n_frames, nch) + dec_G_bytes(n_frames) + (size_t)nch * (size_t)n_frames * 36 * sizeof(uint2);
}

int launch_decode(hipStream_t stream, const int16_t *d_is, const mp3s_granule_si *d_si, const mp3s_frame_hdr *d_hdr,
                  int n_frames, int nch, int n_halo, int out_format, void *d_pcm, void *d_scratch, Profiler *prof, int sf_base,
                  double synth_eps_scale, int32_t *d_sync, bool fast_imdct, bool float_fast, bool fused, hipEvent_t done, const GuardProbe *probe)
{
    const long T = (long)n_frames * 36;
    double *S = (double *)d_scratch;
    double *G = (double *)((char *)d_scratch + dec_S_bytes(n_frames, nch));
    uint2 *fix_list = (uint2 *)((char *)G + dec_G_bytes(n_frames));
    const int n_gran = n_frames * 2;
    const bool fast = out_format == MP3S_PCM_I16 && synth_eps_scale > 0 && d_sync;
    const bool fast32 = out_format == MP3S_PCM_F32 && float_fast;
    if (fused && ((fast && fast_imdct) || fast32)) {
        int run = 16;
        {
            double best = 1e30;
            for (int r = 4; r <= 16; r++) {
                const long waves = (n_gran + r - 1) / r;
                const long rounds = (waves + 2047) / 2048;
                const double cost = (double)rounds * (r + 1.6);
                if (cost < best) { best = cost; run = r; }
            }
        }
        const int runs = (n_gran + run - 1) / run;
        const dim3 grid((runs + ST_WAVES - 1) / ST_WAVES), block(ST_WAVES * 64);
        const int pf = prof ? prof->begin(stream, K_DEC_SYNTH) : -1;
        if (fast32) {
            if (nch == 2) hipLaunchKernelGGL((k_dec_stream<2, true>), grid, block, 0, stream, d_is, d_si, d_hdr, n_gran, run, n_halo, d_pcm, sf_base, 1.0, (uint2 *)nullptr, (int32_t *)nullptr, (double *)nullptr, (double *)nullptr, 0L, 0L);
            else hipLaunchKernelGGL((k_dec_stream<1, true>), grid, block, 0, stream, d_is, d_si, d_hdr, n_gran, run, n_halo, d_pcm, sf_base, 1.0, (uint2 *)nullptr, (int32_t *)nullptr, (double *)nullptr, (double *)nullptr, 0L, 0L);
        } else {
            if (probe && probe->x) {
                if (nch == 2) hipLaunchKernelGGL((k_dec_stream<2, false, true>), grid, block, 0, stream, d_is, d_si, d_hdr, n_gran, run, n_halo, d_pcm, sf_base, synth_eps_scale, fix_list, d_sync + 6, probe->x, probe->eps, (long)probe->base, (long)probe->cap);
                else hipLaunchKernelGGL((k_dec_stream<1, false, true>), grid, block, 0, stream, d_is, d_si, d_hdr, n_gran, run, n_halo, d_pcm, sf_base, synth_eps_scale, fix_list, d_sync + 6, probe->x, probe->eps, (long)probe->base, (long)probe->cap);
            } else if (nch == 2) hipLaunchKernelGGL((k_dec_stream<2, false>), grid, block, 0, stream, d_is, d_si, d_hdr, n_gran, run, n_halo, d_pcm, sf_base, synth_eps_scale, fix_list, d_sync + 6, (double *)nullptr, (double *)nullptr, 0L, 0L);
            else hipLaunchKernelGGL((k_dec_stream<1, false>), grid, block, 0, stream, d_is, d_si, d_hdr, n_gran, run, n_halo, d_pcm, sf_base, synth_eps_scale, fix_list, d_sync + 6, (double *)nullptr, (double *)nullptr, 0L, 0L);
            const int fix_groups = (int)((T * nch + DEC_A_WAVES - 1) / DEC_A_WAVES) < 128 ? (int)((T * nch + DEC_A_WAVES - 1) / DEC_A_WAVES) : 128;
            if (done)
                hipExtLaunchKernelGGL(k_dec_fixup, dim3(fix_groups), dim3(DEC_A_WAVES * 64), 0, stream, nullptr, done, 0, d_is, d_si, d_hdr, n_gran, nch, T, n_halo,
                                      sf_base, (int16_t *)d_pcm, (const uint2 *)fix_list, d_sync + 6, d_sync + 2);
            else
                hipLaunchKernelGGL(k_dec_fixup, dim3(fix_groups), dim3(DEC_A_WAVES * 64), 0, stream, d_is, d_si, d_hdr, n_gran, nch, T, n_halo,
                                   sf_base, (int16_t *)d_pcm, (const uint2 *)fix_list, d_sync + 6, d_sync + 2);
            done = nullptr;
        }
        if (prof) prof->end(stream, pf);
        if (done && hipEventRecord(done, stream) != hipSuccess) return (int)hipErrorUnknown;
        return (int)hipGetLastError();
    }
    int run = 8;
    {
        double best = 1e30;
        for (int r = 2; r <= 8; r++) {
            const long waves = (n_gran + r - 1) / r;
            const long rounds = (waves + 3071) / 3072;
            const double cost = (double)rounds * (r + 0.55);
            if (cost < best) { best = cost; run = r; }
        }
    }
    const int runs = (n_gran + run - 1) / run;
    int pp = prof ? prof->begin(stream, K_DEC_IMDCT) : -1;
    if ((fast && fast_imdct) || fast32)
        hipLaunchKernelGGL(k_dec_imdct<true>, dim3((runs + DEC_A_WAVES - 1) / DEC_A_WAVES), dim3(DEC_A_WAVES * 64), 0, stream,
                           d_is, d_si, d_hdr, n_gran, nch, run, S, T, sf_base, fast32 ? (double *)nullptr : G);
    else
        hipLaunchKernelGGL(k_dec_imdct<false>, dim3((runs + DEC_A_WAVES - 1) / DEC_A_WAVES), dim3(DEC_A_WAVES * 64), 0, stream,
                           d_is, d_si, d_hdr, n_gran, nch, run, S, T, sf_base, (double *)nullptr);
    if (prof) prof->end(stream, pp);
    constexpr int TW = DEC_SYNTH_TW;
    pp = prof ? prof->begin(stream, K_DEC_SYNTH) : -1;
    if (fast32) {
        constexpr int W = DEC_SYNTH_FAST_TW;
        hipLaunchKernelGGL((k_dec_synth_fast<W, true>), dim3((unsigned)((T + (W * 64 - 15) - 1) / (W * 64 - 15))), dim3(W * 64 * nch), 0, stream,
                           (const double *)S, T, d_hdr, nch, n_halo, (int16_t *)d_pcm, sf_base, 1.0, (const double *)nullptr, n_gran, (uint2 *)nullptr, (int32_t *)nullptr);
    } else if (fast) {
        constexpr int ftw = DEC_SYNTH_FAST_TW;
        const double *Gk = fast_imdct ? G : nullptr;
#define MP3S_FAST_LAUNCH(W)                                                                                                        \
        hipLaunchKernelGGL(k_dec_synth_fast<W>, dim3((unsigned)((T + (W * 64 - 15) - 1) / (W * 64 - 15))), dim3(W * 64 * nch), 0, stream, \
                           (const double *)S, T, d_hdr, nch, n_halo, (int16_t *)d_pcm, sf_base, synth_eps_scale, Gk, n_gran, fix_list, d_sync + 6)
        MP3S_FAST_LAUNCH(ftw);
#undef MP3S_FAST_LAUNCH
        const int fix_groups = (int)((T * nch + DEC_A_WAVES - 1) / DEC_A_WAVES) < 128 ? (int)((T * nch + DEC_A_WAVES - 1) / DEC_A_WAVES) : 128;
        hipLaunchKernelGGL(k_dec_fixup, dim3(fix_groups), dim3(DEC_A_WAVES * 64), 0, stream, d_is, d_si, d_hdr, n_gran, nch, T, n_halo,
                           sf_base, (int16_t *)d_pcm, (const uint2 *)fix_list, d_sync + 6, d_sync + 2);
    } else {
        const int out_per_tile = TW * 64 - 15;
        const int tiles = (int)((T + out_per_tile - 1) / out_per_tile);
        hipLaunchKernelGGL(k_dec_synth<TW>, dim3(tiles), dim3(TW * 64 * nch), 0, stream, (const double *)S, T, d_hdr, nch,
                           n_halo, out_format, d_pcm, sf_base);
    }
    if (prof) prof->end(stream, pp);
    if (done && hipEventRecord(done, stream) != hipSuccess) return (int)hipErrorUnknown;
    return (int)hipGetLastError();
}

size_t enc_scratch_bytes(int n_frames)
{
    return (size_t)2 * 32 * (size_t)n_frames * 36 * sizeof(int32_t);
}

int launch_encode(hipStream_t stream, const int16_t *d_pcm, const mp3s_frame_hdr *d_hdr, int n_frames, int32_t *d_mdct,
                  void *d_scratch, Profiler *prof, bool fused)
{
    if (fused) {
        const long n_gran = (long)n_frames * 2;
        const int pf = prof ? prof->begin(stream, K_ENC_ANALYSIS) : -1;
        hipLaunchKernelGGL(k_enc_fused, dim3((unsigned)((n_gran + EF_GR - 1) / EF_GR)), dim3(EF_WAVES * 64), 0, stream, d_pcm, d_hdr, n_frames, d_mdct);
        if (prof) prof->end(stream, pf);
        return (int)hipGetLastError();
    }
    const long Ts = (long)n_frames * 36;
    int32_t *SB = (int32_t *)d_scratch;
    const long waves = 2 * ((Ts + 63) / 64);
    int pp = prof ? prof->begin(stream, K_ENC_ANALYSIS) : -1;
    hipLaunchKernelGGL(k_enc_analysis, dim3((unsigned)((waves + 3) / 4)), dim3(256), 0, stream, d_pcm, d_hdr, n_frames, SB,
                       Ts);
    if (prof) prof->end(stream, pp);
    pp = prof ? prof->begin(stream, K_ENC_MDCT) : -1;
    hipLaunchKernelGGL(k_enc_mdct, dim3((n_frames + 3) / 4), dim3(256), 0, stream, (const int32_t *)SB, Ts, d_hdr, n_frames,
                       d_mdct);
    if (prof) prof->end(stream, pp);
    return (int)hipGetLastError();
}

int launch_rate(hipStream_t stream, const int32_t *d_mdct, const mp3s_rate_frame *d_frames, int n_frames,
                const uint8_t *d_hide, int n_hide, const int32_t *d_cursor, const int32_t *d_state,
                const int32_t *d_list, int n_list, int16_t *d_ix, mp3s_gr_out *d_out, int32_t *d_en, Profiler *prof, int out_base, int compact,
                const RateVariantArgs *variants, hipEvent_t done)
{
    const int n_units = n_frames * 4;
    if (compact && !d_list) return (int)hipErrorInvalidValue;
    const int n = d_list ? n_list : n_units;
    RateVariants var = {nullptr, nullptr, 0, nullptr, nullptr, nullptr, nullptr};
    if (variants && variants->n > 0) var = RateVariants{variants->d_unit, variants->d_cursor, variants->n, variants->d_ix, variants->d_out, variants->d_en, variants->d_tables};
    if (n + var.n <= 0) return done ? (int)hipEventRecord(done, stream) : 0;
    hipEvent_t t_start = nullptr, t_stop = nullptr;
    const bool timed = prof && prof->attach(K_RATE_LOOP, &t_start, &t_stop);
    if (timed || done)
        hipExtLaunchKernelGGL(k_rate_loop, dim3((n + var.n + RL_WAVES - 1) / RL_WAVES), dim3(RL_WAVES * 64), 0, stream, timed ? t_start : nullptr, timed ? t_stop : done, 0,
                              d_mdct, d_frames, n_units, d_hide, n_hide, d_cursor, d_state, d_list, n, d_ix, d_out, d_en, out_base, compact, var);
    else
        hipLaunchKernelGGL(k_rate_loop, dim3((n + var.n + RL_WAVES - 1) / RL_WAVES), dim3(RL_WAVES * 64), 0, stream, d_mdct, d_frames,
                           n_units, d_hide, n_hide, d_cursor, d_state, d_list, n, d_ix, d_out, d_en, out_base, compact, var);
    if (timed && done && hipEventRecord(done, stream) != hipSuccess) return (int)hipErrorUnknown;
    return (int)hipGetLastError();
}

static size_t chain_scan_bytes(int n_frames) { return ((size_t)((n_frames + CH_THREADS - 1) / CH_THREADS) * sizeof(ChainEl) + 31) & ~(size_t)15; }
constexpr int kRedoRounds = 1;
size_t chain_agg_bytes(int n_frames) { return chain_scan_bytes(n_frames) + (size_t)2 * REDO_WORDS * 4; }

int launch_chain(hipStream_t stream, mp3s_gr_out *d_gr, const mp3s_rate_frame *d_frames, int n_frames, const mp3s_chain_seg *d_segs,
                 const int32_t *d_cursor, const int32_t *d_state, void *d_agg, int32_t *d_verdict, mp3s_chain_seg_out *d_seg_out,
                 Profiler *prof, const ChainRedoArgs *redo)
{
    if (n_frames <= 0) return 0;
    const int blocks = (n_frames + CH_THREADS - 1) / CH_THREADS;
    int32_t *d_redo = redo ? (int32_t *)((uint8_t *)d_agg + chain_scan_bytes(n_frames)) : nullptr;
    int32_t *cursor = const_cast<int32_t *>(d_cursor);
    const int pp = prof ? prof->begin(stream, K_CHAIN) : -1;
    hipLaunchKernelGGL(k_chain_sum, dim3(blocks), dim3(CH_THREADS), 0, stream, (const mp3s_gr_out *)d_gr, d_frames, d_segs, n_frames,
                       (ChainEl *)d_agg, d_verdict, d_seg_out, d_redo, (const int32_t *)nullptr);
    hipLaunchKernelGGL(k_chain_apply, dim3(blocks), dim3(CH_THREADS), 0, stream, d_gr, d_frames, d_segs, n_frames,
                       (const ChainEl *)d_agg, cursor, d_state, d_verdict, d_seg_out, d_redo, (const int32_t *)nullptr);
    if (redo) {
        int32_t *lists[2] = {d_redo, d_redo + REDO_WORDS};
        for (int round = 0; round < kRedoRounds; round++) {
            const int32_t *cur = lists[round & 1];
            int32_t *nxt = round + 1 < kRedoRounds ? lists[(round + 1) & 1] : nullptr;
            hipLaunchKernelGGL(k_rate_redo, dim3(REDO_GROUPS), dim3(RL_WAVES * 64), 0, stream, redo->d_mdct, d_frames, n_frames * 4,
                               redo->d_hide, redo->n_hide, cur, redo->d_ix, d_gr, redo->d_en, (const int32_t *)d_cursor);
            hipLaunchKernelGGL(k_chain_sum, dim3(blocks), dim3(CH_THREADS), 0, stream, (const mp3s_gr_out *)d_gr, d_frames, d_segs, n_frames,
                               (ChainEl *)d_agg, d_verdict, d_seg_out, nxt, cur);
            hipLaunchKernelGGL(k_chain_apply, dim3(blocks), dim3(CH_THREADS), 0, stream, d_gr, d_frames, d_segs, n_frames,
                               (const ChainEl *)d_agg, cursor, d_state, d_verdict, d_seg_out, nxt, cur);
        }
    }
    if (prof) prof->end(stream, pp);
    return (int)hipGetLastError();
}

int launch_select(hipStream_t stream, const mp3s_chain_seg *d_segs, const mp3s_select_span *d_spans, int n_segs, int max_reach,
                  const uint8_t *d_hide, const RateVariantArgs &v, int16_t *d_ix, int32_t *d_en, mp3s_gr_out *d_out, int32_t *d_cursor,
                  void *d_pairs, Profiler *prof)
{
    if (n_segs <= 0 || max_reach <= 0 || v.n <= 0) return 0;
    if (max_reach > MP3S_SELECT_MAX_REACH || (int64_t)n_segs * max_reach > 0x3fffffff) return (int)hipErrorInvalidValue;
    const int pp = prof ? prof->begin(stream, K_CHAIN) : -1;
    hipLaunchKernelGGL(k_chain_select, dim3(n_segs), dim3(SEL_THREADS), select_lds_bytes(max_reach), stream, d_segs, d_spans, max_reach,
                       d_hide, (const uint8_t *)v.d_tables, (const mp3s_gr_out *)d_out, d_cursor, (int2 *)d_pairs);
    const int n_pairs = n_segs * max_reach;
    hipLaunchKernelGGL(k_scatter_entries, dim3((n_pairs + 3) / 4), dim3(256), 0, stream, (const int2 *)d_pairs, n_pairs,
                       (const int16_t *)v.d_ix, (const int32_t *)v.d_en, (const mp3s_gr_out *)v.d_out, d_ix, d_en, d_out);
    if (prof) prof->end(stream, pp);
    return (int)hipGetLastError();
}

int launch_gather_tables(hipStream_t stream, const mp3s_gr_out *d_outv, int n, uint8_t *d_tables)
{
    if (n <= 0) return 0;
    hipLaunchKernelGGL(k_gather_tables, dim3((n + 255) / 256), dim3(256), 0, stream, d_outv, n, d_tables);
    return (int)hipGetLastError();
}

int launch_scatter(hipStream_t stream, const int32_t *d_pairs, int n_pairs, const int16_t *d_ixv, const int32_t *d_env,
                   const mp3s_gr_out *d_outv, int16_t *d_ix, int32_t *d_en, mp3s_gr_out *d_out)
{
    if (n_pairs <= 0) return 0;
    hipLaunchKernelGGL(k_scatter_entries, dim3((n_pairs + 3) / 4), dim3(256), 0, stream, (const int2 *)d_pairs, n_pairs, d_ixv, d_env,
                       d_outv, d_ix, d_en, d_out);
    return (int)hipGetLastError();
}

int launch_huffman(hipStream_t stream, const uint8_t *d_blob, const mp3s_frame_side *d_side, int n_frames, int nch, int max_bits,
                   int16_t *d_is, mp3s_granule_si *d_si, int32_t *d_status, int32_t *d_sync, Profiler *prof, bool per_frame, int lanes_opt)
{
    const long units = (long)n_frames * 4;
    const int W = huf_words_for(max_bits);
    int dev = 0;
    (void)hipGetDevice(&dev);
    const int dslot = dev >= 0 && dev < 64 ? dev : 0;
    static std::atomic<int> lds_of_device[64];
    int lds_max = lds_of_device[dslot].load(std::memory_order_relaxed);
    if (lds_max == 0) {
        if (hipDeviceGetAttribute(&lds_max, hipDeviceAttributeMaxSharedMemoryPerBlock, dev) != hipSuccess || lds_max < 64 * 1024) lds_max = 64 * 1024;
        lds_of_device[dslot].store(lds_max, std::memory_order_relaxed);
    }
    const size_t kLdsMax = (size_t)lds_max;
    auto dyn = [&](int cols, int wv) { return ((size_t)(W + 17) * cols + 17 * wv) * 4; };
    auto fits = [&](int cols) { return dyn(cols, 8) + HUF_TAB_N * 2 + 256 <= kLdsMax; };
    int lanes = 16, waves = 4;
    if (fits(128)) { lanes = 32; waves = 4; }
    if (fits(256) && units > 32 * 1024) { lanes = 64; waves = 4; }
    if (lanes_opt > 0) {
        const int a = lanes_opt;
        if (a == 64 && fits(256)) { lanes = 64; waves = 4; }
        if (a == 62 && fits(128)) { lanes = 64; waves = 2; }
        if (a == 32 && fits(128)) { lanes = 32; waves = 4; }
        if (a == 16) { lanes = 16; waves = 4; }
        if (a == 8) { lanes = 8; waves = 8; }
    }
    static const bool trace = getenv("MP3S_TRACE") != nullptr;
    if (trace) fprintf(stderr, "[mp3s] huffman launch: %ld units, W %d, %d waves x %d lanes, %zu bytes of dynamic LDS\n", units, W, waves, lanes, dyn(waves * lanes, waves));
    const int pp = prof ? prof->begin(stream, K_DEC_HUFFMAN) : -1;
#define MP3S_HUF_LAUNCH(WV, LN)                                                                                         \
    do {                                                                                                                \
        static std::atomic<unsigned long long> asked{0};                                                              \
        if (!(asked.load(std::memory_order_relaxed) & (1ull << dslot))) {                                               \
            (void)hipFuncSetAttribute(reinterpret_cast<const void *>(&k_dec_huffman<WV, LN>), hipFuncAttributeMaxDynamicSharedMemorySize, \
                                      (int)(kLdsMax - HUF_TAB_N * 2 - 256));                                            \
            asked.fetch_or(1ull << dslot, std::memory_order_relaxed);                                                   \
        }                                                                                                               \
        hipLaunchKernelGGL((k_dec_huffman<WV, LN>), dim3((unsigned)((units + WV * LN - 1) / (WV * LN))), dim3(WV * 64), \
                           dyn(WV * LN, WV), stream, d_blob, d_side, n_frames, nch, W, max_bits, d_is, d_si, d_status, per_frame ? 1 : 0, d_sync); \
    } while (0)
    if (lanes == 64 && waves == 4) MP3S_HUF_LAUNCH(4, 64);
    else if (lanes == 64) MP3S_HUF_LAUNCH(2, 64);
    else if (lanes == 32) MP3S_HUF_LAUNCH(4, 32);
    else if (lanes == 8) MP3S_HUF_LAUNCH(8, 8);
    else MP3S_HUF_LAUNCH(4, 16);
#undef MP3S_HUF_LAUNCH
    if (prof) prof->end(stream, pp);
    return (int)hipGetLastError();
}

static_assert(sizeof(ParseFrameRef) == sizeof(FrameRef) && sizeof(ParseStreamRef) == sizeof(StreamRef), "frame / stream references out of sync with mp3s_host.h");

int launch_parse(hipStream_t stream, const uint8_t *d_image, uint32_t image_base, const FrameRef *d_refs, const StreamRef *d_streams, int n_frames,
                 uint32_t md_base, mp3s_frame_side *d_side, mp3s_frame_hdr *d_hdr, uint8_t *d_blob, uint64_t *d_tsel, int32_t *d_status)
{
    if (n_frames <= 0) return 0;
    hipLaunchKernelGGL(k_dec_parse, dim3((n_frames + PARSE_WAVES - 1) / PARSE_WAVES), dim3(PARSE_WAVES * 64), 0, stream, d_image, image_base,
                       reinterpret_cast<const ParseFrameRef *>(d_refs), reinterpret_cast<const ParseStreamRef *>(d_streams), n_frames, md_base, d_side,
                       d_hdr, d_blob, d_tsel, d_status);
    return (int)hipGetLastError();
}

__global__ __launch_bounds__(256) void k_place_frames(const uint8_t *__restrict__ entries, int n_entries, int16_t *__restrict__ is,
                                                      mp3s_granule_si *__restrict__ si)
{
    const uint8_t *e = entries + (size_t)blockIdx.x * 4912;
    const int f = *reinterpret_cast<const int32_t *>(e);
    const uint32_t *src = reinterpret_cast<const uint32_t *>(e + 16);
    uint32_t *d_is = reinterpret_cast<uint32_t *>(is + (size_t)f * 2304), *d_si = reinterpret_cast<uint32_t *>(si + (size_t)f * 4);
    for (int i = threadIdx.x; i < 1152; i += 256) d_is[i] = src[i];
    for (int i = threadIdx.x; i < 72; i += 256) d_si[i] = src[1152 + i];
}
int launch_place_frames(hipStream_t stream, const uint8_t *d_entries, int n_entries, int16_t *d_is, mp3s_granule_si *d_si)
{
    if (n_entries <= 0) return 0;
    hipLaunchKernelGGL(k_place_frames, dim3(n_entries), dim3(256), 0, stream, d_entries, n_entries, d_is, d_si);
    return (int)hipGetLastError();
}

__global__ void k_spin(long long ticks, int *sink)
{
    const long long t0 = wall_clock64();
    int it = 0;
    while (wall_clock64() - t0 < ticks && it < (1 << 22)) it++;
    if (sink && it < 0) *sink = it;
}
__global__ void k_noop() {}
int launch_spin(hipStream_t stream, int microseconds)
{
    hipLaunchKernelGGL(k_spin, dim3(1), dim3(64), 0, stream, (long long)microseconds * 100, (int *)nullptr);
    return (int)hipGetLastError();
}
int launch_noop(hipStream_t stream)
{
    hipLaunchKernelGGL(k_noop, dim3(1), dim3(64), 0, stream);
    return (int)hipGetLastError();
}

__global__ __launch_bounds__(256) void k_copy16(const uint4 *__restrict__ src, uint4 *__restrict__ dst, size_t n16)
{
    const size_t stride = (size_t)gridDim.x * blockDim.x;
    for (size_t i = (size_t)blockIdx.x * blockDim.x + threadIdx.x; i < n16; i += stride) dst[i] = src[i];
}
int launch_copy(hipStream_t stream, const void *d_src, void *d_dst, size_t bytes)
{
    hipLaunchKernelGGL(k_copy16, dim3(256 * 16), dim3(256), 0, stream, (const uint4 *)d_src, (uint4 *)d_dst, bytes / 16);
    return (int)hipGetLastError();
}

int launch_wav_gather(hipStream_t stream, const uint8_t *d_image, const WavRun *d_runs, int n_runs, int max_frames, int16_t *d_pcm)
{
    if (n_runs <= 0 || max_frames <= 0) return 0;
    const unsigned gx = (unsigned)std::min<size_t>(((size_t)max_frames * 288 + 255) / 256, 2048);
    for (int r0 = 0; r0 < n_runs; r0 += 32768)
        hipLaunchKernelGGL(k_wav_gather, dim3(gx, (unsigned)std::min(n_runs - r0, 32768)), dim3(256), 0, stream, d_image, d_runs, r0, d_pcm);
    return (int)hipGetLastError();
}

int launch_pack(hipStream_t stream, const int16_t *d_ix, const mp3s_gr_out *d_gr, const int32_t *d_en, int n_frames, int sri,
                int bri, int whole_slots, const uint32_t *d_frame_off, const uint8_t *d_padding, uint8_t *d_mp3,
                int32_t *d_scfsi, int32_t *d_status, int32_t *d_sync, Profiler *prof, int f_begin, int f_end)
{
    const int pp = prof ? prof->begin(stream, K_ENC_PACK) : -1;
    if (f_end < 0 || f_end > n_frames) f_end = n_frames;
    const int count = f_end - f_begin;
    const int groups = count >= 8192 ? 2048 : (count + 3) / 4;
    if (count > 0)
        hipLaunchKernelGGL(k_enc_pack, dim3(groups), dim3(256), 0, stream,
                           d_ix, d_gr, d_en, f_end, sri, bri, whole_slots,
                           d_frame_off, d_padding, d_mp3, d_scfsi, d_status, d_sync, f_begin);
    if (prof) prof->end(stream, pp);
    return (int)hipGetLastError();
}

}
```

mp3-steganography-lib_amd/csrc/mp3s_encode_pipeline.cpp:

```cpp
#include <sys/stat.h>
#include <unistd.h>
#include <cerrno>
#include "mp3s_internal.h"

static inline size_t up16(size_t x) { return (x + 15) & ~(size_t)15; }

static int64_t cursor0(const EncSeg &s)
{
    return s.carry_in ? std::min<int64_t>(std::max<int64_t>(s.carry_in->cursor, 0), kNoCursor) : 0;
}

int enc_layout(std::vector<EncSeg> &segs, int samplerate, int bitrate_kbps, EncLayout &L, bool select)
{
    if (bitrate_kbps <= 0) return fail(MP3S_E_UNSUPPORTED, "bitrate %d", bitrate_kbps);
    if (stream_params(samplerate, bitrate_kbps, &L.sri, &L.bri, &L.whole))
        return fail(MP3S_E_UNSUPPORTED, "unsupported samplerate/bitrate %d/%d", samplerate, bitrate_kbps);
    L.samplerate = samplerate; L.kbps = bitrate_kbps;
    int64_t n64 = 0, hide64 = kPatternBytes;
    for (auto &s : segs) {
        if (s.n_frames <= 0 || s.n_hide < 0 || (s.n_hide > 0 && !s.hide)) return fail(MP3S_E_ARG, "bad stream in the encode batch");
        s.first = (int)n64; s.hide_base = (int)hide64;
        n64 += s.n_frames; hide64 += s.n_hide;
        if (n64 > 0x7fffffff / 8 || hide64 >= kNoCursor - 8) return fail(MP3S_E_ARG, "encode batch too large");
    }
    if (n64 <= 0) return fail(MP3S_E_ARG, "empty encode batch");
    L.lead = segs[0].lead;
    if (L.lead < 0 || L.lead > 2 || (segs.size() > 1 && (L.lead || segs[0].first_frame || segs[0].carry_in)))
        return fail(MP3S_E_ARG, "a block of a longer stream is encoded on its own");
    L.n = (int)n64; L.units = L.n * 4; L.n_hide = (int)hide64; L.n_all = L.n + L.lead; L.n_segs = (int)segs.size();
    L.o_rf = up16((size_t)L.n_all * sizeof(mp3s_frame_hdr));
    L.o_cur = L.o_rf + up16((size_t)L.n * sizeof(mp3s_rate_frame));
    L.o_hide = L.o_cur + up16((size_t)L.units * 4);
    L.o_segs = L.o_hide + up16((size_t)L.n_hide);
    L.o_off = L.o_segs + up16((size_t)L.n_segs * sizeof(mp3s_chain_seg));
    L.o_pad = L.o_off + up16(((size_t)L.n + 1) * 4);
    std::vector<mp3s_chain_seg> cs(segs.size());
    std::vector<mp3s_select_span> spans(segs.size());
    for (size_t si = 0; si < segs.size(); si++) {
        const EncSeg &s = segs[si];
        cs[si] = mp3s_chain_seg();
        cs[si].first_frame = s.first; cs[si].n_frames = s.n_frames; cs[si].hide_base = s.hide_base;
        cs[si].hide_begin = (int32_t)((int64_t)s.hide_base + cursor0(s)); cs[si].hide_end = s.hide_base + s.n_hide;
    }
    const int budget = !select ? 0 : (int)std::min<int64_t>((int64_t)L.units * MP3S_SELECT_VARIANTS, 6000000);
    L.redo = false;
    for (const EncSeg &s : segs) {
        const size_t known = s.n_guess < 0 ? (size_t)s.n_frames * 4 : (size_t)std::min(s.n_guess, s.n_frames * 4);
        if (s.any_silent >= 0 ? s.any_silent != 0 : (!s.tables_guess || known < (size_t)s.n_frames * 4 || std::memchr(s.tables_guess, 0, known))) L.redo = true;
    }
    std::vector<int32_t> min_reach(segs.size(), 0);
    for (size_t si = 0; si < segs.size(); si++) {
        const EncSeg &s = segs[si];
        const int64_t left = (int64_t)cs[si].hide_end - cs[si].hide_begin;
        if (!s.tables_guess || left <= 0) continue;
        const int64_t need = left + left / 16 + 48;
        int64_t offered = 0, j = 0;
        const int64_t known = s.n_guess < 0 ? (int64_t)s.n_frames * 4 : std::min<int64_t>(s.n_guess, (int64_t)s.n_frames * 4);
        while (j < known && offered < need) offered += s.tables_guess[j++];
        if (offered < need) j += (need - offered) * 5 / 14;
        min_reach[si] = (int32_t)std::min<int64_t>((int64_t)s.n_frames * 4, j + 32);
    }
    L.n_entries = select_plan(cs.data(), L.n_segs, spans.data(), nullptr, nullptr, budget, min_reach.data());
    L.max_reach = 0;
    for (size_t si = 0; si < segs.size(); si++) {
        segs[si].reach = spans[si].reach; segs[si].first_entry = spans[si].first_entry;
        L.max_reach = std::max(L.max_reach, spans[si].reach);
    }
    L.o_spans = L.o_pad + up16((size_t)L.n);
    L.o_ent = L.o_spans + up16((size_t)L.n_segs * sizeof(mp3s_select_span));
    L.bytes = L.o_ent + up16((size_t)L.n_entries * 8);
    return MP3S_OK;
}

bool enc_variant_buffers(mp3s_ctx *c, const EncLayout &L, EncDev &d)
{
    if (L.n_entries <= 0) { d.d_ixv = nullptr; d.d_outv = nullptr; d.d_env = nullptr; return true; }
    d.d_ixv = (int16_t *)c->grab(kSlotVariants + 1, (size_t)L.n_entries * 1152);
    d.d_outv = (mp3s_gr_out *)c->grab(kSlotVariants + 2, variant_out_bytes(L.n_entries));
    d.d_env = (int32_t *)c->grab(kSlotVariants + 3, (size_t)L.n_entries * 88);
    return d.d_ixv && d.d_outv && d.d_env;
}

int enc_fill(std::vector<EncSeg> &segs, EncLayout &L, uint8_t *dst)
{
    std::memset(dst, 0, L.bytes);
    mp3s_frame_hdr *hdr = (mp3s_frame_hdr *)dst;
    mp3s_rate_frame *rf = (mp3s_rate_frame *)(dst + L.o_rf);
    int32_t *cursor = (int32_t *)(dst + L.o_cur);
    uint8_t *hide_all = dst + L.o_hide;
    mp3s_chain_seg *cs = (mp3s_chain_seg *)(dst + L.o_segs);
    uint32_t *off = (uint32_t *)(dst + L.o_off);
    uint8_t *pad8 = dst + L.o_pad;
    mp3s_select_span *spans = (mp3s_select_span *)(dst + L.o_spans);
    mp3s_select_patterns(hide_all);
    std::vector<int32_t> padding;
    L.bytes_before = 0;
    for (size_t si = 0; si < segs.size(); si++) {
        EncSeg &s = segs[si];
        padding.resize((size_t)s.n_frames);
        const int rc = rate_frames(L.samplerate, L.kbps, 2, s.n_frames, rf + s.first, padding.data(), s.first_frame, &L.bytes_before);
        if (rc) return fail(rc, "unsupported samplerate/bitrate %d/%d", L.samplerate, L.kbps);
        for (int f = s.first; f < s.first + s.n_frames; f++) {
            rf[f].hide_end = s.hide_base + s.n_hide;
            rf[f].stream = (int32_t)si;
            pad8[f] = (uint8_t)padding[(size_t)(f - s.first)];
        }
        for (int f = s.first; f < s.first + s.n_frames + L.lead; f++) {
            hdr[f].sr_idx = (uint8_t)L.sri; hdr[f].nch = 2; hdr[f].ms_stereo = 0; hdr[f].flags = 0; hdr[f].stream_first = (uint32_t)s.first;
        }
        if (s.n_hide) std::memcpy(hide_all + s.hide_base, s.hide, (size_t)s.n_hide);
        const int64_t c0 = cursor0(s);
        const bool long_msg = s.reach > 0 || s.n_hide - c0 > kLongMessageBits;
        int64_t ahead = 0;
        for (int j = 0; j < s.n_frames * 4; j++) {
            cursor[(size_t)s.first * 4 + j] = long_msg ? kNoCursor : (int32_t)std::min<int64_t>((int64_t)s.hide_base + c0 + ahead, kNoCursor);
            ahead += s.tables_guess && (s.n_guess < 0 || j < s.n_guess) ? s.tables_guess[j] : 3;
        }
        spans[si].first_entry = s.first_entry; spans[si].reach = s.reach;
        cs[si].first_frame = s.first; cs[si].n_frames = s.n_frames;
        cs[si].hide_base = s.hide_base; cs[si].hide_begin = (int32_t)((int64_t)s.hide_base + c0);
        cs[si].hide_end = s.hide_base + s.n_hide;
        if (s.carry_in) std::memcpy(cs[si].chain_in, s.carry_in->chain, sizeof cs[si].chain_in);
    }
    if (L.n_entries > 0) {
        int32_t *ent = (int32_t *)(dst + L.o_ent);
        for (const auto &s : segs)
            if (s.reach > 0) select_entries(s.first * 4, s.reach, s.first_entry, s.hide_base + s.n_hide, (int64_t)s.n_hide - cursor0(s), ent, ent + L.n_entries);
    }
    off[0] = 0;
    for (int f = 0; f < L.n; f++) off[f + 1] = off[f] + (uint32_t)(L.whole + pad8[f]);
    L.mp3_bytes = off[L.n];
    for (auto &s : segs) {
        s.mp3_off = off[s.first];
        s.mp3_len = off[s.first + s.n_frames] - off[s.first];
        if (s.last) s.mp3_len -= std::min<size_t>(s.mp3_len, (size_t)((L.bytes_before + (int64_t)s.mp3_len) % 4));
    }
    return MP3S_OK;
}

void tables_guess_of(const mp3s_frame_side *side, long n_frames, int extra, std::vector<uint8_t> &out)
{
    out.resize((size_t)(n_frames + extra) * 4);
    for (long f = 0; f < n_frames + extra; f++) {
        const mp3s_frame_side &fs = side[f < n_frames ? f : n_frames - 1];
        for (int ch = 0; ch < 2; ch++)
            for (int gr = 0; gr < 2; gr++) {
                const mp3s_unit_side &u = fs.unit[gr][ch];
                int n = 0;
                if (u.big_values) for (int r = 0; r < (u.window_switching ? 2 : 3); r++) n += u.table_select[r] != 0;
                out[(size_t)f * 4 + ch * 2 + gr] = (uint8_t)n;
            }
    }
}

int enc_issue(mp3s_ctx *c, const EncLayout &L, const EncDev &d, hipStream_t tail, hipEvent_t tail_from, hipEvent_t rate_after, hipEvent_t pcm_read)
{
    const mp3s_frame_hdr *d_hdr = (const mp3s_frame_hdr *)d.d_in;
    const mp3s_rate_frame *d_rf = (const mp3s_rate_frame *)(d.d_in + L.o_rf);
    const int32_t *d_cur = (const int32_t *)(d.d_in + L.o_cur);
    const uint8_t *d_hide = d.d_in + L.o_hide;
    const mp3s_chain_seg *d_segs = (const mp3s_chain_seg *)(d.d_in + L.o_segs);
    const int32_t *d_mdct = d.d_mdct_all + (size_t)L.lead * 2304;
    int rc = mp3s_encode_transform_dev(c, d.d_pcm, d_hdr, L.n_all, d.d_mdct_all);
    if (!rc && pcm_read && hipEventRecord(pcm_read, c->stream) != hipSuccess) rc = fail(MP3S_E_HIP, "event record failed");
    if (!rc && rate_after && hipStreamWaitEvent(c->stream, rate_after, 0) != hipSuccess) rc = fail(MP3S_E_HIP, "ordering behind the previous tail failed");
    const bool select_on_tail = tail && L.n_entries > 0;
    const bool rate_signals = tail && tail_from && (select_on_tail || L.n_entries <= 0) && (c->opt[MP3S_OPT_PIPE_SIGNALS] & 2);
    if (rate_signals) c->rate_done = tail_from;
    if (!rc && L.n_entries > 0) {
        const int32_t *d_ent = (const int32_t *)(d.d_in + L.o_ent);
        if (!rc && !select_on_tail)
            rc = mp3s_rate_select_dev(c, d_mdct, d_rf, L.n, d_hide, L.n_hide, const_cast<int32_t *>(d_cur), d_segs,
                                      (const mp3s_select_span *)(d.d_in + L.o_spans), L.n_segs, L.max_reach, d_ent, d_ent + L.n_entries,
                                      L.n_entries, d.d_ix, d.d_out, d.d_en, d.d_ixv, d.d_outv, d.d_env);
        else if (!rc)
            rc = mp3s_rate_variants_dev(c, d_mdct, d_rf, L.n, d_hide, L.n_hide, d_cur, d_ent, d_ent + L.n_entries, L.n_entries, d.d_ix, d.d_out, d.d_en,
                                        d.d_ixv, d.d_outv, d.d_env);
    } else if (!rc)
        rc = mp3s_rate_loop_dev(c, d_mdct, d_rf, L.n, d_hide, L.n_hide, d_cur, nullptr, nullptr, 0, d.d_ix, d.d_out, d.d_en);
    c->rate_done = nullptr;
    hipStream_t ts = c->stream;
    if (!rc && tail) {
        if ((!rate_signals && hipEventRecord(tail_from, c->stream) != hipSuccess) || hipStreamWaitEvent(tail, tail_from, 0) != hipSuccess)
            rc = fail(MP3S_E_HIP, "ordering the tail stream failed");
        ts = tail;
    }
    if (!rc && select_on_tail) {
        const int32_t *d_ent = (const int32_t *)(d.d_in + L.o_ent);
        hipStream_t keep = c->stream;
        c->stream = ts;
        rc = mp3s_select_dev(c, d_hide, const_cast<int32_t *>(d_cur), d_segs, (const mp3s_select_span *)(d.d_in + L.o_spans), L.n_segs, L.max_reach,
                             d_ent, d_ent + L.n_entries, L.n_entries, d.d_ix, d.d_out, d.d_en, d.d_ixv, d.d_outv, d.d_env);
        c->stream = keep;
        if (!rc && !c->ev_sel && hipEventCreateWithFlags(&c->ev_sel, hipEventDisableTiming) != hipSuccess) rc = fail(MP3S_E_HIP, "event creation failed");
        if (!rc && hipEventRecord(c->ev_sel, ts) != hipSuccess) rc = fail(MP3S_E_HIP, "event record failed");
        if (!rc) c->sel_pending = true;
    }
    if (!rc) {
        const ChainRedoArgs redo = {d_mdct, d_hide, L.n_hide, d.d_ix, d.d_en};
        const int e = launch_chain(ts, d.d_out, d_rf, L.n, d_segs, d_cur, nullptr, d.d_agg, d.d_small,
                                   (mp3s_chain_seg_out *)((uint8_t *)d.d_small + kSmallHead), &c->prof, !c->opt[MP3S_OPT_REDO] || !L.redo ? nullptr : &redo);
        if (e) rc = fail(MP3S_E_HIP, "chain launch: %s", hipGetErrorString((hipError_t)e));
    }
    if (!rc) {
        const bool halves = d.direct_status && d.pack_half && d.pack_split > 0 && d.pack_split < L.n;
        int e = launch_pack(ts, d.d_ix, d.d_out, d.d_en, L.n, L.sri, L.bri, L.whole, (const uint32_t *)(d.d_in + L.o_off), d.d_in + L.o_pad, d.d_mp3,
                            d.d_sc, d.d_small + 2, d.direct_status ? nullptr : c->d_sync, &c->prof, 0, halves ? d.pack_split : -1);
        if (!e && halves) {
            if (hipEventRecord(d.pack_half, ts) != hipSuccess) e = (int)hipErrorUnknown;
            else e = launch_pack(ts, d.d_ix, d.d_out, d.d_en, L.n, L.sri, L.bri, L.whole, (const uint32_t *)(d.d_in + L.o_off), d.d_in + L.o_pad, d.d_mp3,
                                 d.d_sc, d.d_small + 2, nullptr, &c->prof, d.pack_split, -1);
        }
        if (e) rc = fail(MP3S_E_HIP, "pack launch: %s", hipGetErrorString((hipError_t)e));
    }
    return rc;
}

int enc_resolve(mp3s_ctx *c, const EncLayout &L, std::vector<EncSeg> &segs, const uint8_t *in, const EncDev &d, mp3s_buf *b, bool have_gr,
                int *passes_out)
{
    const int n = L.n, units = L.units, n_hide = L.n_hide, samplerate = L.samplerate, bitrate_kbps = L.kbps;
    const uint8_t *hide_all = in + L.o_hide;
    const uint8_t *const d_in = d.d_in;
    int16_t *const d_ix = d.d_ix; mp3s_gr_out *const d_out = d.d_out; int32_t *const d_en = d.d_en; uint8_t *const d_mp3 = d.d_mp3;
    int32_t *const d_sc = d.d_sc, *const d_small = d.d_small;
    const int32_t *d_mdct = d.d_mdct_all + (size_t)L.lead * 2304;
    const mp3s_rate_frame *d_rf = (const mp3s_rate_frame *)(d_in + L.o_rf);
    const uint8_t *d_hide = d_in + L.o_hide;
    const size_t total = segs.back().mp3_off + segs.back().mp3_len;
    void *d_redo = c->grab(kSlotRedo, (size_t)units * 24);
    if (!d_redo || !b->big[0].reserve(L.mp3_bytes)) return fail(MP3S_E_NOMEM, "memory for resolving %d units", units);
    b->mp3 = b->big[0].data();
    int rc = MP3S_OK;
    double t_mark = trace_on() ? now_ms() : 0;
    auto mark = [&](const char *what) {
        if (!trace_on()) return;
        const double t = now_ms();
        fprintf(stderr, "mp3s:   resolve: %-28s %.3f ms\n", what, t - t_mark);
        t_mark = t;
    };
    if (!b->big[1].reserve((size_t)units * sizeof(mp3s_gr_out))) return fail(MP3S_E_NOMEM, "host memory for %d units", units);
    mp3s_gr_out *const gr = b->gr_out = (mp3s_gr_out *)b->big[1].data();
    if (!have_gr) rc = mp3s_dev_download(c, gr, d_out, (size_t)units * sizeof(mp3s_gr_out));
    b->scfsi.assign((size_t)n * 8, 0);
    std::vector<int32_t> &cursor = c->h_cursor, &state = c->h_state;
    cursor.assign((const int32_t *)(in + L.o_cur), (const int32_t *)(in + L.o_cur) + units);
    if (!rc && (L.n_entries > 0 || (L.redo && c->opt[MP3S_OPT_REDO]))) rc = mp3s_dev_download(c, cursor.data(), d_in + L.o_cur, (size_t)units * 4);
    state.assign((size_t)units * 4, 0);
    int passes = 1;
    std::vector<int32_t> list, redo_in;
    std::vector<mp3s_gr_out> tmp;
    struct Pending { int unit; int64_t cur; };
    std::vector<Pending> pend(segs.size());
    std::vector<int32_t> &want = c->h_want, &state_want = c->h_state_want;
    want.assign(units, 0); state_want.assign((size_t)units * 4, 0);
    auto walk = [&]() {
        list.clear();
        for (size_t si = 0; si < segs.size(); si++) {
            EncSeg &s = segs[si];
            pend[si] = {-1, 0};
            int64_t cur = s.hide_base + cursor0(s);
            const int64_t end = (int64_t)s.hide_base + s.n_hide;
            int32_t chain[4][4] = {};
            if (s.carry_in) std::memcpy(chain, s.carry_in->chain, sizeof chain);
            bool own[4] = {false, false, false, false};
            s.carry_used = cur < end;
            for (int u = s.first * 4; u < (s.first + s.n_frames) * 4; u++) {
                const int k = u & 3;
                mp3s_gr_out &g = gr[u];
                bool redo = false;
                const bool active = g.flags & MP3S_RF_ACTIVE;
                if (!own[k] && (!active || (g.flags & MP3S_RF_USED_ADDR_IN))) s.carry_used = true;
                if (active) own[k] = true;
                if (s.n_hide > 0 && active) {
                    const int64_t used = cursor[u];
                    if (used != cur && std::min<int64_t>(used, cur) < end) {
                        redo = true;
                        if (pend[si].unit < 0) pend[si] = {u, cur};
                    }
                }
                if ((g.flags & MP3S_RF_USED_ADDR_IN) &&
                    (state[(size_t)u * 4] != chain[k][0] || state[(size_t)u * 4 + 1] != chain[k][1] ||
                     state[(size_t)u * 4 + 2] != chain[k][2]))
                    redo = true;
                if (redo) list.push_back(u);
                want[u] = (int32_t)std::min<int64_t>(cur, kNoCursor);
                for (int j = 0; j < 4; j++) state_want[(size_t)u * 4 + j] = chain[k][j];
                if (active) {
                    cur += g.n_tables;
                    chain[k][0] = g.address[0]; chain[k][1] = g.address[1]; chain[k][2] = g.address[2];
                    chain[k][3] = g.quantizer_step;
                } else {
                    g.address[0] = chain[k][0]; g.address[1] = chain[k][1]; g.address[2] = chain[k][2];
                    g.quantizer_step = chain[k][3];
                }
                if (g.flags & MP3S_RF_STEP_RANGE) return fail(MP3S_E_STEP_RANGE, "quantizer step left the table in unit %d", u);
            }
            s.hide_offset = cur - s.hide_base;
            s.carry_out.cursor = s.hide_offset;
            std::memcpy(s.carry_out.chain, chain, sizeof chain);
        }
        return (int)MP3S_OK;
    };
    std::vector<uint8_t> tables_of;
    auto run_entries = [&](const std::vector<int32_t> &units_of, const std::vector<int32_t> &cursor_of, void *d_entries, int compact,
                           int16_t *ix_to, mp3s_gr_out *out_to, int32_t *en_to, uint8_t *d_tables) {
        const size_t nl = units_of.size();
        redo_in.resize(nl * 6);
        for (size_t i = 0; i < nl; i++) {
            const int u = units_of[i];
            redo_in[i] = u;
            redo_in[nl + i] = cursor_of[i];
            for (int j = 0; j < 4; j++) redo_in[2 * nl + 4 * i + j] = state_want[(size_t)u * 4 + j];
        }
        int r = mp3s_dev_upload(c, d_entries, redo_in.data(), nl * 24);
        if (!r) {
            const int32_t *dr = (const int32_t *)d_entries;
            const int e = launch_rate(c->stream, d_mdct, d_rf, n, d_hide, n_hide, dr + nl, dr + 2 * nl, dr, (int)nl, ix_to, out_to, en_to,
                                      &c->prof, 0, compact);
            if (e) r = fail(MP3S_E_HIP, "rate launch: %s", hipGetErrorString((hipError_t)e));
        }
        if (d_tables) {
            if (!r && launch_gather_tables(c->stream, out_to, (int)nl, d_tables)) r = fail(MP3S_E_HIP, "gathering the table counts failed");
            tables_of.resize(nl);
            if (!r) r = mp3s_dev_download(c, tables_of.data(), d_tables, nl);
        } else {
            tmp.resize(nl);
            if (!r) r = mp3s_dev_download(c, tmp.data(), out_to, nl * sizeof(mp3s_gr_out));
        }
        passes++;
        return r;
    };
    mark("GrInfo down");
    if (!rc) rc = walk();
    mark("walk");
    if (!rc && list.size() > kFewUnits) {
        struct Span { size_t seg; int unit, count; int64_t cur; size_t entry; };
        std::vector<Span> spans;
        std::vector<int32_t> ent_unit, ent_cursor, pairs;
        void *d_ent = nullptr, *d_ixv = nullptr, *d_outv = nullptr, *d_env = nullptr, *d_pairs = nullptr;
        for (bool more = true; more && !rc;) {
            spans.clear(); ent_unit.clear(); ent_cursor.clear(); pairs.clear();
            for (size_t si = 0; si < segs.size(); si++) {
                if (pend[si].unit < 0) continue;
                const EncSeg &s = segs[si];
                const int64_t end = (int64_t)s.hide_base + s.n_hide;
                if (pend[si].cur + 3 > end) { pend[si].unit = -1; continue; }
                const int room = (kVariantEntries - (int)ent_unit.size()) / 8;
                const int count = (int)std::min<int64_t>({(int64_t)(s.first + s.n_frames) * 4 - pend[si].unit, (end - pend[si].cur) * 5 / 14 + 32, (int64_t)room});
                if (count <= 0) continue;
                spans.push_back({si, pend[si].unit, count, pend[si].cur, ent_unit.size()});
                for (int v = 0; v < 8; v++)
                    for (int j = 0; j < count; j++) { ent_unit.push_back(pend[si].unit + j); ent_cursor.push_back(4 * v); }
            }
            if (spans.empty()) break;
            const size_t ne = ent_unit.size();
            int slot = kSlotVariants;
            auto alloc = [&](void **p, size_t bytes) { *p = c->grab(slot++, bytes); return *p != nullptr; };
            if (!alloc(&d_ent, ne * 24) || !alloc(&d_ixv, ne * 1152) || !alloc(&d_outv, ne * sizeof(mp3s_gr_out)) ||
                !alloc(&d_env, ne * 88) || !alloc(&d_pairs, ne))
                rc = fail(MP3S_E_NOMEM, "hipMalloc failed for the message variants");
            mark("variant entries listed");
            if (!rc) rc = run_entries(ent_unit, ent_cursor, d_ent, 2, (int16_t *)d_ixv, (mp3s_gr_out *)d_outv, (int32_t *)d_env, (uint8_t *)d_pairs);
            mark("variants: up, launch, down");
            more = false;
            for (const Span &sp : spans) {
                if (rc) break;
                const EncSeg &s = segs[sp.seg];
                const int64_t end = (int64_t)s.hide_base + s.n_hide;
                int64_t cur = sp.cur;
                int j = 0;
                for (; j < sp.count && cur + 3 <= end; j++) {
                    const int u = sp.unit + j;
                    const int v = (hide_all[cur] & 1) * 4 + (hide_all[cur + 1] & 1) * 2 + (hide_all[cur + 2] & 1);
                    const size_t e = sp.entry + (size_t)v * sp.count + j;
                    cursor[u] = (int32_t)cur;
                    for (int q = 0; q < 4; q++) state[(size_t)u * 4 + q] = state_want[(size_t)u * 4 + q];
                    pairs.push_back((int32_t)e); pairs.push_back(u);
                    cur += tables_of[e];
                }
                if (j == sp.count && cur < end && sp.unit + sp.count < (s.first + s.n_frames) * 4) { pend[sp.seg] = {sp.unit + sp.count, cur}; more = true; }
                else pend[sp.seg].unit = -1;
            }
            for (size_t si = 0; si < segs.size(); si++) more |= pend[si].unit >= 0;
            mark("variants: select");
            if (!rc && !pairs.empty()) {
                rc = mp3s_dev_upload(c, d_pairs, pairs.data(), pairs.size() * 4);
                mark("variants: pairs up");
                if (!rc) {
                    const int e = launch_scatter(c->stream, (const int32_t *)d_pairs, (int)(pairs.size() / 2), (const int16_t *)d_ixv,
                                                 (const int32_t *)d_env, (const mp3s_gr_out *)d_outv, (int16_t *)d_ix, (int32_t *)d_en, d_out);
                    if (e) rc = fail(MP3S_E_HIP, "scatter: %s", hipGetErrorString((hipError_t)e));
                }
                if (!rc && hipStreamSynchronize(c->stream) != hipSuccess) rc = fail(MP3S_E_HIP, "sync failed");
            }
            mark("variants: select, scatter");
        }
        if (!rc) rc = mp3s_dev_download(c, gr, d_out, (size_t)units * sizeof(mp3s_gr_out));
        mark("GrInfo down");
        if (!rc) rc = walk();
        mark("walk");
    }
    std::vector<int32_t> cur_of;
    while (!rc && !list.empty()) {
        if (passes > units + 16) { rc = fail(MP3S_E_HIP, "rate-loop chain did not converge"); break; }
        cur_of.resize(list.size());
        for (size_t i = 0; i < list.size(); i++) cur_of[i] = want[list[i]];
        const std::vector<int32_t> units_of = list;
        rc = run_entries(units_of, cur_of, d_redo, 1, (int16_t *)d_ix, (mp3s_gr_out *)d_out, (int32_t *)d_en, nullptr);
        if (!rc)
            for (size_t i = 0; i < units_of.size(); i++) {
                const int u = units_of[i];
                gr[u] = tmp[i];
                cursor[u] = cur_of[i];
                for (int q = 0; q < 4; q++) state[(size_t)u * 4 + q] = state_want[(size_t)u * 4 + q];
            }
        if (!rc) rc = walk();
    }
    mark("exact re-runs");
    if (!rc) {
        rc = mp3s_dev_upload(c, d_out, gr, (size_t)units * sizeof(mp3s_gr_out));
        if (!rc) rc = mp3s_pack_frames_dev(c, (const int16_t *)d_ix, (const mp3s_gr_out *)d_out, (const int32_t *)d_en, n, samplerate,
                                           bitrate_kbps, (const uint32_t *)((uint8_t *)d_in + L.o_off), (const uint8_t *)d_in + L.o_pad,
                                           (uint8_t *)d_mp3, (int32_t *)d_sc, (int32_t *)d_small + 2);
        int32_t st = 0;
        if (!rc) rc = mp3s_dev_download(c, &st, (int32_t *)d_small + 2, sizeof st);
        if (!rc && st) rc = fail(MP3S_E_HIP, "bit packer reported status %d", st);
        if (!rc) rc = mp3s_dev_download(c, b->mp3, d_mp3, total);
        if (!rc) rc = mp3s_dev_download(c, b->scfsi.data(), d_sc, (size_t)n * 8 * 4);
    }
    mark("GrInfo up, pack, bytes down");
    if (passes_out) *passes_out = passes;
    return rc;
}


int encode_batch(mp3s_ctx *c, const int16_t *pcm, const int16_t *pcm_dev, std::vector<EncSeg> &segs, int samplerate, int bitrate_kbps,
                 mp3s_buf *b, int *passes_out, bool want_gr)
{
    EncLayout L;
    int rc = enc_layout(segs, samplerate, bitrate_kbps, L, c->opt[MP3S_OPT_SELECT] != 0);
    if (rc) return rc;
    const int n = L.n, units = L.units, n_all = L.n_all;
    HIPCHK(hipSetDevice(c->device));
    std::vector<uint8_t> &in = c->h_in;
    in.resize(L.bytes);
    rc = enc_fill(segs, L, in.data());
    if (rc) return rc;
    void *d_pcm = nullptr, *d_in = nullptr, *d_mdct_all = nullptr, *d_ix = nullptr, *d_out = nullptr, *d_en = nullptr,
         *d_agg = nullptr, *d_mp3 = nullptr, *d_sc = nullptr, *d_small = nullptr;
    auto cleanup = [&]() { hipStreamSynchronize(c->stream); };
    int slot = 8;
    auto alloc = [&](void **p, size_t bytes) { *p = c->grab(slot++, bytes); return *p != nullptr; };
    if (pcm_dev) { d_pcm = const_cast<int16_t *>(pcm_dev); slot++; }
    else if (!alloc(&d_pcm, (size_t)n_all * 2304 * 2)) d_pcm = nullptr;
    if (!d_pcm || !alloc(&d_in, L.bytes) || !alloc(&d_mdct_all, (size_t)n_all * 2304 * 4) || (slot++ , false) ||
        !alloc(&d_ix, (size_t)n * 2304 * 2) || !alloc(&d_out, (size_t)units * sizeof(mp3s_gr_out)) || !alloc(&d_en, (size_t)units * 22 * 4) ||
        !alloc(&d_agg, chain_agg_bytes(n)) || !alloc(&d_mp3, L.mp3_bytes + 16) || !alloc(&d_sc, (size_t)n * 8 * 4) ||
        !alloc(&d_small, small_bytes(L.n_segs))) {
        cleanup();
        return fail(MP3S_E_NOMEM, "hipMalloc failed for a %d-frame encode", n);
    }
    const size_t total = segs.back().mp3_off + segs.back().mp3_len;
    if (!b->big[0].reserve(L.mp3_bytes) || !b->big[2].reserve(small_bytes(L.n_segs)) ||
        (want_gr && !b->big[1].reserve((size_t)units * sizeof(mp3s_gr_out)))) {
        cleanup();
        return fail(MP3S_E_NOMEM, "host memory for a %d-frame encode", n);
    }
    b->mp3 = b->big[0].data();
    int32_t *const small = (int32_t *)b->big[2].data();
    const mp3s_chain_seg_out *const seg_out = (const mp3s_chain_seg_out *)(b->big[2].data() + kSmallHead);
    if (want_gr) b->scfsi.assign((size_t)n * 8, 0);
    if (!pcm_dev && hipMemcpyAsync(d_pcm, pcm, (size_t)n_all * 2304 * 2, hipMemcpyHostToDevice, c->stream) != hipSuccess) rc = fail(MP3S_E_HIP, "PCM upload failed");
    if (!rc && hipMemcpyAsync(d_in, in.data(), L.bytes, hipMemcpyHostToDevice, c->stream) != hipSuccess) rc = fail(MP3S_E_HIP, "input upload failed");
    EncDev dev;
    dev.d_pcm = (const int16_t *)d_pcm; dev.d_in = (const uint8_t *)d_in; dev.d_mdct_all = (int32_t *)d_mdct_all; dev.d_ix = (int16_t *)d_ix;
    dev.d_out = (mp3s_gr_out *)d_out; dev.d_en = (int32_t *)d_en; dev.d_agg = d_agg; dev.d_mp3 = (uint8_t *)d_mp3; dev.d_sc = (int32_t *)d_sc;
    dev.d_small = (int32_t *)d_small;
    if (!rc && !enc_variant_buffers(c, L, dev)) rc = fail(MP3S_E_NOMEM, "hipMalloc failed for %d variant entries", L.n_entries);
    if (!rc) rc = enc_issue(c, L, dev);
    auto down = [&](void *dst, const void *src, size_t bytes) {
        if (!rc && bytes && hipMemcpyAsync(dst, src, bytes, hipMemcpyDeviceToHost, c->stream) != hipSuccess) rc = fail(MP3S_E_HIP, "download failed");
    };
    down(small, d_small, small_bytes(L.n_segs));
    down(b->mp3, d_mp3, total);
    if (want_gr) {
        down(b->big[1].data(), d_out, (size_t)units * sizeof(mp3s_gr_out));
        down(b->scfsi.data(), d_sc, (size_t)n * 8 * 4);
    }
    if (!rc && hipStreamSynchronize(c->stream) != hipSuccess) rc = fail(MP3S_E_HIP, "sync failed");
    if (rc) { cleanup(); return rc; }
    if (want_gr) b->gr_out = (mp3s_gr_out *)b->big[1].data();
    if (small[0] == 0 && small[1] == 0) {
        if (small[2]) { cleanup(); return fail(MP3S_E_HIP, "bit packer reported status %d", small[2]); }
        for (size_t si = 0; si < segs.size(); si++) {
            EncSeg &s = segs[si];
            s.hide_offset = seg_out[si].cursor - s.hide_base;
            s.carry_out.cursor = s.hide_offset;
            std::memcpy(s.carry_out.chain, seg_out[si].chain, sizeof s.carry_out.chain);
            s.carry_used = seg_out[si].carry_used != 0;
        }
        if (passes_out) *passes_out = 1;
        return MP3S_OK;
    }
// ... 408 lines not shown
```

mp3-steganography-lib_amd/csrc/mp3s_internal.h:

```cpp
#pragma once
#include <hip/hip_runtime_api.h>

#include <algorithm>
#include <atomic>
#include <chrono>
#include <cstdarg>
#include <cstdio>
#include <cstdlib>
#include <cstring>
#include <memory>
#include <mutex>
#include <string>
#include <thread>
#include <vector>

#include "../../include/mp3s.h"
#include "mp3s_device.h"
#include "mp3s_host.h"

namespace mp3s {
int fail(int code, const char *fmt, ...) __attribute__((format(printf, 2, 3)));
}

using namespace mp3s;

#define HIPCHK(call)                                                                                 \
    do {                                                                                             \
        hipError_t e_ = (call);                                                                      \
        if (e_ != hipSuccess) return fail(MP3S_E_HIP, "%s: %s", #call, hipGetErrorString(e_));       \
    } while (0)

struct mp3s_pipe;
struct mp3s_ctx {
    int device = 0;
    int64_t opt[MP3S_OPT_COUNT] = {0};
    mp3s_run_stats run_stats = {0, 0, 0, 0, 0};
    mp3s_pipe *own_pipe = nullptr;
    std::vector<mp3s_pipe *> parked_pipes;
    int sink_fd = -1; size_t sink_done = 0, sink_base = 0; bool sink_early = false;
    hipStream_t stream = nullptr;
    hipEvent_t ev0 = nullptr, ev1 = nullptr, ev_order = nullptr;
    hipEvent_t ev_sel = nullptr; bool sel_pending = false;
    hipEvent_t rate_done = nullptr;
    int32_t *d_sync = nullptr;
    double synth_eps_scale = 1.0;
    GuardProbe guard_probe = {nullptr, nullptr, 0, 0};
    void *scratch = nullptr; size_t scratch_bytes = 0;
    Profiler prof;
    static constexpr int kPoolSlots = 32;
    void *pool[kPoolSlots] = {nullptr};
    size_t pool_bytes[kPoolSlots] = {0};
    void *grab(int slot, size_t bytes)
    {
        if (bytes < 16) bytes = 16;
        if (pool_bytes[slot] >= bytes) return pool[slot];
        if (pool[slot]) { hipStreamSynchronize(stream); hipFree(pool[slot]); pool[slot] = nullptr; pool_bytes[slot] = 0; }
        const size_t want = bytes + bytes / 4;
        if (hipMalloc(&pool[slot], want) != hipSuccess) { pool[slot] = nullptr; return nullptr; }
        pool_bytes[slot] = want;
        return pool[slot];
    }
    std::vector<int32_t> h_cursor, h_state, h_want, h_state_want;
    std::vector<uint8_t> h_in;
    std::vector<mp3s_frame_hdr> h_hdr;
    std::vector<mp3s_frame_side> h_side;
    std::vector<uint8_t> h_blob;
    ScannedStream spare_scan;
    std::vector<FrameRef> h_refs;
    std::vector<uint8_t> h_tables;
    int ensure_scratch(size_t bytes)
    {
        if (bytes <= scratch_bytes) return 0;
        if (scratch) { hipFree(scratch); scratch = nullptr; scratch_bytes = 0; }
        hipError_t e = hipMalloc(&scratch, bytes);
        if (e != hipSuccess) return fail(MP3S_E_NOMEM, "hipMalloc(%zu) for scratch: %s", bytes, hipGetErrorString(e));
        scratch_bytes = bytes;
        return 0;
    }
    void *scratch_enc = nullptr; size_t scratch_enc_bytes = 0;
    int ensure_scratch_enc(size_t bytes)
    {
        if (bytes <= scratch_enc_bytes) return 0;
        if (scratch_enc) { hipFree(scratch_enc); scratch_enc = nullptr; scratch_enc_bytes = 0; }
        hipError_t e = hipMalloc(&scratch_enc, bytes);
        if (e != hipSuccess) return fail(MP3S_E_NOMEM, "hipMalloc(%zu) for scratch: %s", bytes, hipGetErrorString(e));
        scratch_enc_bytes = bytes;
        return 0;
    }
};

inline int guard_probe_usable(const mp3s_ctx *c, int out_format)
{
    if (!c->guard_probe.x || out_format != MP3S_PCM_I16) return MP3S_OK;
    if (c->opt[MP3S_OPT_FUSED_DECODE] && c->opt[MP3S_OPT_FAST_IMDCT] && c->synth_eps_scale > 0 && c->d_sync) return MP3S_OK;
    return fail(MP3S_E_ARG, "the guard probe is set (mp3s_debug_guard_margin) and this int16 decode would not run the stream kernel that fills it "
                            "(MP3S_OPT_FUSED_DECODE / MP3S_OPT_FAST_IMDCT off, or the guard's scale is 0)");
}

int local_world_size();

class PinnedBlock {
public:
    PinnedBlock() = default;
    PinnedBlock(const PinnedBlock &) = delete;
    PinnedBlock &operator=(const PinnedBlock &) = delete;
    ~PinnedBlock() { release(); }
    bool reserve(size_t bytes)
    {
        if (bytes <= cap_) return true;
        release();
        if (bytes > kMaxPinned) {
            p_ = (uint8_t *)std::malloc(bytes);
            if (!p_) return false;
            cap_ = bytes; pinned_ = false;
            return true;
        }
        pinned_ = true;
        {
            std::lock_guard<std::mutex> g(mu());
            auto &fl = free_list();
            size_t best = fl.size();
            const size_t too_big = std::max(4 * bytes, bytes + ((size_t)1 << 20));
            for (size_t i = 0; i < fl.size(); i++)
                if (fl[i].second >= bytes && fl[i].second <= too_big && (best == fl.size() || fl[i].second < fl[best].second)) best = i;
            if (best < fl.size()) { p_ = fl[best].first; cap_ = fl[best].second; fl.erase(fl.begin() + best); return true; }
        }
        const size_t want = bytes + bytes / 8 + (1 << 16);
        void *q = nullptr;
        if (hipHostMalloc(&q, want, hipHostMallocDefault) != hipSuccess) return false;
        p_ = (uint8_t *)q; cap_ = want;
        return true;
    }
    uint8_t *data() const { return p_; }
    static void pool_state(size_t *held, size_t *cap)
    {
        std::lock_guard<std::mutex> g(mu());
        size_t h = 0;
        for (auto &e : free_list()) h += e.second;
        *held = h; *cap = pool_cap();
    }

private:
    void release()
    {
        if (!p_) return;
        if (!pinned_) { std::free(p_); p_ = nullptr; cap_ = 0; return; }
        std::lock_guard<std::mutex> g(mu());
        auto &fl = free_list();
        size_t held = 0;
        for (auto &e : fl) held += e.second;
        if (fl.size() < 48 && held + cap_ <= pool_cap()) fl.emplace_back(p_, cap_);
        else hipHostFree(p_);
        p_ = nullptr; cap_ = 0;
    }
    static std::mutex &mu() { static std::mutex *m = new std::mutex(); return *m; }
    static std::vector<std::pair<uint8_t *, size_t>> &free_list()
    {
        static auto *v = new std::vector<std::pair<uint8_t *, size_t>>();
        return *v;
    }
    static constexpr size_t kMaxPinned = (size_t)4 << 30;
    static size_t pool_cap()
    {
        static const size_t cap = std::max<size_t>((size_t)1 << 30, kMaxPinned / (size_t)local_world_size());
        return cap;
    }
    uint8_t *p_ = nullptr;
    size_t cap_ = 0;
    bool pinned_ = true;
};

struct mp3s_multi {
    std::vector<std::pair<const uint8_t *, size_t>> files;
    std::vector<ParsedStream> parsed;
    std::vector<ScannedStream> scanned;
    PinnedBlock arena[3];
    size_t head_room = 0;
    std::vector<const uint8_t *> pcm;
    struct Window { long first, count; bool keep_dup; };
    std::vector<Window> window;
    std::vector<std::vector<uint8_t>> all_bits;
    const StreamIndex *index = nullptr;
};

struct mp3s_buf {
    std::shared_ptr<mp3s_multi> multi;
    ParsedStream parsed;
    ScannedStream scanned;
    std::vector<uint8_t> bytes;
    std::vector<uint8_t> bits;
    std::vector<int32_t> scfsi;
    std::vector<std::unique_ptr<mp3s_buf>> parts;
    PinnedBlock big[3];
    uint8_t *mp3 = nullptr;
    mp3s_gr_out *gr_out = nullptr;
};

inline bool trace_on() { static const bool on = getenv("MP3S_TRACE") != nullptr; return on; }
inline double now_ms() { return std::chrono::duration<double, std::milli>(std::chrono::steady_clock::now().time_since_epoch()).count(); }

template <class F>
void parallel_files(int n, size_t total_bytes, F f)
{
    const unsigned hw = std::thread::hardware_concurrency();
    const int workers = (int)std::min<size_t>({(size_t)n, (size_t)std::min(hw ? hw : 1u, 16u), total_bytes / (256u << 10) + 1});
    if (workers <= 1) {
        for (int i = 0; i < n; i++) f(i);
        return;
    }
    std::atomic<int> next{0};
    auto run = [&]() { for (int i; (i = next.fetch_add(1)) < n;) f(i); };
    std::vector<std::thread> pool;
    for (int w = 1; w < workers; w++) pool.emplace_back(run);
    run();
    for (auto &t : pool) t.join();
}

constexpr int kDecodeChunk = 16384;
inline size_t pcm_elem(int fmt) { return fmt == MP3S_PCM_I16 ? 2 : (fmt == MP3S_PCM_F32 ? 4 : 8); }
int max_part2_3(const mp3s_frame_side *side, long n);
void cut_window(ParsedStream &p, ScannedStream &sc, long first, long count);
int front_end(mp3s_multi &m, int i);
int decode_transform_chunk(mp3s_ctx *c, const int16_t *d_is, const mp3s_granule_si *d_si, const mp3s_frame_hdr *d_hdr, long first, int cnt,
                           int nch, int halo, int out_format, void *d_pcm, hipStream_t stream = nullptr ,
                           hipEvent_t done = nullptr );
int decode_group(mp3s_ctx *c, mp3s_multi &m, const std::vector<int> &idx, int nch, int out_format, void *d_keep = nullptr);

constexpr int kLongMessageBits = 1024;
constexpr int32_t kNoCursor = MP3S_NO_CURSOR;
constexpr int kPatternBytes = 32;
constexpr int kVariantEntries = 65536;
constexpr size_t kFewUnits = 8;

struct EncSeg {
    int n_frames = 0;
    const uint8_t *hide = nullptr;
    int n_hide = 0;
    int lead = 0;
    int64_t first_frame = 0;
    bool last = true;
    const mp3s_carry *carry_in = nullptr;
    const uint8_t *tables_guess = nullptr;
    int n_guess = -1;
    int any_silent = -1;
    int first = 0, hide_base = 0;
    int reach = 0, first_entry = 0;
    int64_t hide_offset = 0;
    size_t mp3_off = 0, mp3_len = 0;
    mp3s_carry carry_out = {};
    bool carry_used = false;
};
struct EncLayout {
    int n = 0, n_all = 0, lead = 0, units = 0, n_hide = 0, n_segs = 0;
    int n_entries = 0, max_reach = 0;
    bool redo = true;
    int sri = 0, bri = 0, whole = 0, samplerate = 0, kbps = 0;
    size_t o_rf = 0, o_cur = 0, o_hide = 0, o_segs = 0, o_off = 0, o_pad = 0, o_spans = 0, o_ent = 0, bytes = 0;
    size_t mp3_bytes = 0;
    int64_t bytes_before = 0;
};
constexpr size_t kSmallHead = 32;
inline size_t small_bytes(int n_segs) { return kSmallHead + (size_t)n_segs * sizeof(mp3s_chain_seg_out); }
int enc_layout(std::vector<EncSeg> &segs, int samplerate, int bitrate_kbps, EncLayout &L, bool select = true );
int enc_fill(std::vector<EncSeg> &segs, EncLayout &L, uint8_t *dst);
struct EncDev {
    const int16_t *d_pcm = nullptr;
    const uint8_t *d_in = nullptr;
    int32_t *d_mdct_all = nullptr;
    int16_t *d_ix = nullptr; mp3s_gr_out *d_out = nullptr; int32_t *d_en = nullptr;
    void *d_agg = nullptr;
    uint8_t *d_mp3 = nullptr; int32_t *d_sc = nullptr;
    int32_t *d_small = nullptr;
    bool direct_status = false;
    int pack_split = 0; hipEvent_t pack_half = nullptr;
    int16_t *d_ixv = nullptr; mp3s_gr_out *d_outv = nullptr; int32_t *d_env = nullptr;
};
void select_entries(int first_unit, int reach, int first_entry, int hide_end, int64_t bits_left, int32_t *ent_unit, int32_t *ent_cursor);
bool enc_variant_buffers(mp3s_ctx *c, const EncLayout &L, EncDev &d);
int enc_issue(mp3s_ctx *c, const EncLayout &L, const EncDev &d, hipStream_t tail = nullptr ,
              hipEvent_t tail_from = nullptr, hipEvent_t rate_after = nullptr ,
              hipEvent_t pcm_read = nullptr );
constexpr int kSlotRedo = 11, kSlotVariants = 19;
int enc_resolve(mp3s_ctx *c, const EncLayout &L, std::vector<EncSeg> &segs, const uint8_t *in, const EncDev &d, mp3s_buf *b, bool have_gr,
                int *passes_out);
int encode_batch(mp3s_ctx *c, const int16_t *pcm, const int16_t *pcm_dev, std::vector<EncSeg> &segs, int samplerate, int bitrate_kbps,
                 mp3s_buf *b, int *passes_out, bool want_gr = true);
int select_plan(const mp3s_chain_seg *segs, int n_segs, mp3s_select_span *spans, int32_t *ent_unit, int32_t *ent_cursor, int cap,
                const int32_t *min_reach);
void tables_guess_of(const mp3s_frame_side *side, long n_frames, int extra, std::vector<uint8_t> &out);

int wav_encode_check(const uint8_t *wav, size_t len, int bitrate_kbps, const uint8_t *hide_bits, int n_hide, mp3s_wav_info *w, int64_t *count);

constexpr int kRunFallback = 1;
constexpr int kRunHide = 0, kRunClear = 1, kRunDecode = 2;
struct RunResult {
    int64_t n_frames = 0, n_rows = 0;
    int nch = 0, sampling_rate = 0, bit_rate = 0, kbps = 0;
    const uint8_t *mp3 = nullptr; size_t mp3_len = 0;
    int64_t hide_offset = 0; int too_long = 0;
    const uint8_t *pcm = nullptr;
    const uint8_t *bits = nullptr; size_t n_bits = 0;
};
int run_file(mp3s_ctx *c, const uint8_t *mp3, size_t len, int mode, const uint8_t *utf8, size_t n_msg, int out_format, mp3s_buf **owner, RunResult *out);
void destroy_own_pipe(mp3s_ctx *c);
void pipe_quiesce(mp3s_pipe *P);
void own_pipe_lanes(const mp3s_ctx *c, mp3s_run_stats *out);

int host_cpus_allowed();
int local_world_size();
int default_scan_threads(const mp3s_ctx *c);
std::vector<int> gpu_node_cpus(int device);
```

Measured before the change: 19.49 million frames/s.

## Fuse chain sum/apply into one lookback kernel and fold redo check and scatter

Replaces the two-kernel chain scan (sum then apply) with a single k_chain_check that publishes per-block aggregates and spins on a ready bitmask, capped at 64 blocks, before walking its own block. The redo rerun is merged with a serial single-block recheck in k_redo_check, and the entry scatter is folded into the tail of k_chain_select. Together these cut kernel launches and inter-kernel gaps in the per-step tail. In exchange the code relies on all blocks being co-resident for the spin-wait, falls back to a forced redo on spin timeout, and runs the recheck walk serially in one workgroup.

```diff
diff --git a/mp3-steganography-lib_amd/csrc/k_chain.hpp b/mp3-steganography-lib_amd/csrc/k_chain.hpp
--- a/mp3-steganography-lib_amd/csrc/k_chain.hpp
+++ b/mp3-steganography-lib_amd/csrc/k_chain.hpp
@@ -90,32 +90,22 @@
     if (threadIdx.x == 0) agg[blockIdx.x] = total;
 }
 
-__global__ __launch_bounds__(CH_THREADS) void k_chain_apply(mp3s_gr_out *__restrict__ gr, const mp3s_rate_frame *__restrict__ rf,
-                                                            const mp3s_chain_seg *__restrict__ segs, int n_frames,
-                                                            const ChainEl *__restrict__ agg, int32_t *__restrict__ cursor_in,
-                                                            const int32_t *__restrict__ state_in, int32_t *__restrict__ verdict,
-                                                            mp3s_chain_seg_out *__restrict__ seg_out, int32_t *__restrict__ redo_list,
-                                                            const int32_t *__restrict__ only_after)
-{
-    if (only_after && only_after[0] == 0) return;
-    __shared__ ChainEl wave_tot[CH_THREADS / 64];
-    const int f = blockIdx.x * CH_THREADS + threadIdx.x;
-    ChainEl before = chain_identity();
-    for (int c0 = 0; c0 < (int)blockIdx.x; c0 += CH_THREADS) {
-        const int j = c0 + (int)threadIdx.x;
-        ChainEl total;
-        chain_block_scan(j < (int)blockIdx.x ? agg[j] : chain_identity(), wave_tot, &total);
-        before = chain_combine(before, total);
-    }
+__device__ __forceinline__ void chain_walk_block(mp3s_gr_out *__restrict__ gr, const mp3s_rate_frame *__restrict__ rf,
+                                                 const mp3s_chain_seg *__restrict__ segs, int n_frames, int block, const ChainEl &before,
+                                                 ChainEl (&wave_tot)[CH_THREADS / 64], int32_t *__restrict__ cursor_in,
+                                                 const int32_t *__restrict__ state_in, mp3s_chain_seg_out *__restrict__ seg_out,
+                                                 int32_t *__restrict__ redo_list, int &redo_here, int &err_here, ChainEl *total)
+{
+    const int f = block * CH_THREADS + (int)threadIdx.x;
     const ChainEl own_el = chain_element(gr, rf, segs, f, n_frames);
-    const ChainEl incl = chain_block_scan(own_el, wave_tot, nullptr);
+    const ChainEl incl = chain_block_scan(own_el, wave_tot, total);
     ChainEl excl = chain_shfl_up(incl, 1);
     if ((threadIdx.x & 63) == 0) {
         excl = chain_identity();
         for (int w = 0; w < (int)(threadIdx.x >> 6); w++) excl = chain_combine(excl, wave_tot[w]);
     }
     excl = chain_combine(before, excl);
-    int redo_here = 0, err_here = 0;
+    redo_here = 0; err_here = 0;
     if (f < n_frames) {
         const int s = rf[f].stream;
         const mp3s_chain_seg sg = segs[s];
@@ -161,6 +151,8 @@
                     if (hiding) cursor_in[u] = c;
 #pragma unroll
                     for (int j = 0; j < 4; j++) redo_list[REDO_HEAD + 2 * REDO_CAP + 4 * at + j] = ch[j];
+                } else if (flags & MP3S_RF_LISTED) {
+                    g.flags = flags & ~MP3S_RF_LISTED;
                 }
             } else if (flags & MP3S_RF_LISTED) {
                 g.flags = flags & ~MP3S_RF_LISTED;
@@ -183,6 +175,26 @@
             }
         }
     }
+}
+
+__global__ __launch_bounds__(CH_THREADS) void k_chain_apply(mp3s_gr_out *__restrict__ gr, const mp3s_rate_frame *__restrict__ rf,
+                                                            const mp3s_chain_seg *__restrict__ segs, int n_frames,
+                                                            const ChainEl *__restrict__ agg, int32_t *__restrict__ cursor_in,
+                                                            const int32_t *__restrict__ state_in, int32_t *__restrict__ verdict,
+                                                            mp3s_chain_seg_out *__restrict__ seg_out, int32_t *__restrict__ redo_list,
+                                                            const int32_t *__restrict__ only_after)
+{
+    if (only_after && only_after[0] == 0) return;
+    __shared__ ChainEl wave_tot[CH_THREADS / 64];
+    ChainEl before = chain_identity();
+    for (int c0 = 0; c0 < (int)blockIdx.x; c0 += CH_THREADS) {
+        const int j = c0 + (int)threadIdx.x;
+        ChainEl total;
+        chain_block_scan(j < (int)blockIdx.x ? agg[j] : chain_identity(), wave_tot, &total);
+        before = chain_combine(before, total);
+    }
+    int redo_here, err_here;
+    chain_walk_block(gr, rf, segs, n_frames, (int)blockIdx.x, before, wave_tot, cursor_in, state_in, seg_out, redo_list, redo_here, err_here, nullptr);
     const int n_redo = (int)wave_add_u32((uint32_t)redo_here);
     const bool any_err = __ballot(err_here != 0) != 0;
     if ((threadIdx.x & 63) == 0) {
@@ -191,6 +203,134 @@
     }
 }
 
+constexpr int CHK_MAX_BLOCKS = 64;
+constexpr int CHK_SPINS = 1 << 20;
+struct ChainLook { unsigned long long ready; int32_t done, reserved; };
+
+__global__ __launch_bounds__(CH_THREADS) void k_chain_check(mp3s_gr_out *__restrict__ gr, const mp3s_rate_frame *__restrict__ rf,
+                                                            const mp3s_chain_seg *__restrict__ segs, int n_frames, ChainEl *agg,
+                                                            int2 *part, int32_t *__restrict__ cursor_in, const int32_t *__restrict__ state_in,
+                                                            int32_t *__restrict__ verdict, mp3s_chain_seg_out *__restrict__ seg_out,
+                                                            int32_t *__restrict__ redo, ChainLook *look)
+{
+    __shared__ ChainEl wave_tot[CH_THREADS / 64];
+    __shared__ int sh_ok, sh_redo, sh_err, sh_last;
+    const int b = blockIdx.x, tid = threadIdx.x, f = b * CH_THREADS + tid;
+    if (tid == 0) { sh_ok = 1; sh_redo = 0; sh_err = 0; }
+    if (redo && f == 0) { redo[0] = 0; redo[1] = 0; redo[REDO_WORDS] = 0; }
+    if (f < n_frames && segs[rf[f].stream].first_frame == f) seg_out[rf[f].stream].carry_used = 0;
+    __threadfence();
+    ChainEl total;
+    chain_block_scan(chain_element(gr, rf, segs, f, n_frames), wave_tot, &total);
+    if (tid == 0) {
+        __hip_atomic_store(&agg[b].reset, total.reset, __ATOMIC_RELAXED, __HIP_MEMORY_SCOPE_AGENT);
+        __hip_atomic_store(&agg[b].tables, total.tables, __ATOMIC_RELAXED, __HIP_MEMORY_SCOPE_AGENT);
+#pragma unroll
+        for (int k = 0; k < 4; k++) __hip_atomic_store(&agg[b].last[k], total.last[k], __ATOMIC_RELAXED, __HIP_MEMORY_SCOPE_AGENT);
+        __hip_atomic_fetch_or(&look->ready, 1ull << b, __ATOMIC_RELEASE, __HIP_MEMORY_SCOPE_AGENT);
+        const unsigned long long need = (1ull << b) - 1ull;
+        int spins = 0;
+        while ((__hip_atomic_load(&look->ready, __ATOMIC_ACQUIRE, __HIP_MEMORY_SCOPE_AGENT) & need) != need) {
+            if (++spins > CHK_SPINS) { sh_ok = 0; break; }
+            __builtin_amdgcn_s_sleep(2);
+        }
+    }
+    __syncthreads();
+    const bool ok = sh_ok != 0;
+    int redo_here = 0, err_here = 0;
+    if (ok) {
+        ChainEl e = chain_identity();
+        if (tid < b) {
+            e.reset = __hip_atomic_load(&agg[tid].reset, __ATOMIC_RELAXED, __HIP_MEMORY_SCOPE_AGENT);
+            e.tables = __hip_atomic_load(&agg[tid].tables, __ATOMIC_RELAXED, __HIP_MEMORY_SCOPE_AGENT);
+#pragma unroll
+            for (int k = 0; k < 4; k++) e.last[k] = __hip_atomic_load(&agg[tid].last[k], __ATOMIC_RELAXED, __HIP_MEMORY_SCOPE_AGENT);
+        }
+        ChainEl before;
+        chain_block_scan(e, wave_tot, &before);
+        chain_walk_block(gr, rf, segs, n_frames, b, before, wave_tot, cursor_in, state_in, seg_out, redo, redo_here, err_here, nullptr);
+    } else if (tid == 0) redo_here = 1 << 20;
+    const int n_redo = (int)wave_add_u32((uint32_t)redo_here);
+    const bool any_err = __ballot(err_here != 0) != 0;
+    if ((tid & 63) == 0) {
+        if (n_redo) atomicAdd(&sh_redo, n_redo);
+        if (any_err) atomicOr(&sh_err, 1);
+    }
+    __threadfence();
+    __syncthreads();
+    if (tid == 0) {
+        __hip_atomic_store(&part[b].x, sh_redo, __ATOMIC_RELAXED, __HIP_MEMORY_SCOPE_AGENT);
+        __hip_atomic_store(&part[b].y, sh_err, __ATOMIC_RELAXED, __HIP_MEMORY_SCOPE_AGENT);
+        sh_last = __hip_atomic_fetch_add(&look->done, 1, __ATOMIC_ACQ_REL, __HIP_MEMORY_SCOPE_AGENT) == (int)gridDim.x - 1;
+    }
+    __syncthreads();
+    if (sh_last && tid < 64) {
+        int r = 0, e = 0;
+        if (tid < (int)gridDim.x) {
+            r = __hip_atomic_load(&part[tid].x, __ATOMIC_RELAXED, __HIP_MEMORY_SCOPE_AGENT);
+            e = __hip_atomic_load(&part[tid].y, __ATOMIC_RELAXED, __HIP_MEMORY_SCOPE_AGENT);
+        }
+        r = (int)wave_add_u32((uint32_t)r);
+        const bool any = __ballot(e != 0) != 0;
+        if (tid == 0) {
+            verdict[0] = r; verdict[1] = any ? 1 : 0;
+            __hip_atomic_store(&look->ready, 0ull, __ATOMIC_RELAXED, __HIP_MEMORY_SCOPE_AGENT);
+            __hip_atomic_store(&look->done, 0, __ATOMIC_RELAXED, __HIP_MEMORY_SCOPE_AGENT);
+        }
+    }
+}
+
+__global__ __launch_bounds__(RL_WAVES * 64, 4) void k_redo_check(
+    const int32_t *__restrict__ mdct, const mp3s_rate_frame *__restrict__ frames, int n_frames,
+    const uint8_t *__restrict__ hide, int n_hide, int32_t *redo, int16_t *__restrict__ ix_out,
+    mp3s_gr_out *out, int32_t *__restrict__ en_out, int32_t *cursor_all, const mp3s_chain_seg *__restrict__ segs,
+    int32_t *__restrict__ verdict, mp3s_chain_seg_out *__restrict__ seg_out)
+{
+    static_assert(RL_WAVES * 64 == CH_THREADS, "the check walks a block of frames with the workgroup of a re-run");
+    const int n_want = __builtin_amdgcn_readfirstlane(__hip_atomic_load(&redo[0], __ATOMIC_RELAXED, __HIP_MEMORY_SCOPE_AGENT));
+    if (n_want == 0) return;
+    const int n_list = min(n_want, REDO_CAP);
+    if ((int)blockIdx.x * RL_WAVES < n_list) {
+        const RateVariants none = {nullptr, nullptr, 0, nullptr, nullptr, nullptr, nullptr};
+        const int32_t *unit_list = redo + REDO_HEAD;
+        rate_units<true>(mdct, frames, n_frames * 4, hide, n_hide, unit_list + REDO_CAP, unit_list + 2 * REDO_CAP, unit_list, n_list, ix_out, out,
+                         en_out, 0, 3, none, cursor_all);
+    }
+    __shared__ ChainEl wave_tot[CH_THREADS / 64];
+    __shared__ int sh_last, sh_redo, sh_err;
+    __threadfence();
+    __syncthreads();
+    if (threadIdx.x == 0) {
+        sh_redo = 0; sh_err = 0;
+        sh_last = __hip_atomic_fetch_add(&redo[1], 1, __ATOMIC_ACQ_REL, __HIP_MEMORY_SCOPE_AGENT) == (int)gridDim.x - 1;
+    }
+    __syncthreads();
+    if (!sh_last) return;
+    __builtin_amdgcn_fence(__ATOMIC_ACQUIRE, "agent");
+    for (int f = threadIdx.x; f < n_frames; f += CH_THREADS)
+        if (segs[frames[f].stream].first_frame == f) seg_out[frames[f].stream].carry_used = 0;
+    __threadfence();
+    __syncthreads();
+    ChainEl before = chain_identity();
+    int redo_all = 0, err_all = 0;
+    for (int b = 0; b * CH_THREADS < n_frames; b++) {
+        int redo_here, err_here;
+        ChainEl total;
+        chain_walk_block(out, frames, segs, n_frames, b, before, wave_tot, cursor_all, nullptr, seg_out, nullptr, redo_here, err_here, &total);
+        redo_all += redo_here; err_all |= err_here;
+        before = chain_combine(before, total);
+        __threadfence();
+    }
+    const int n_redo = (int)wave_add_u32((uint32_t)redo_all);
+    const bool any_err = __ballot(err_all != 0) != 0;
+    if ((threadIdx.x & 63) == 0) {
+        if (n_redo) atomicAdd(&sh_redo, n_redo);
+        if (any_err) atomicOr(&sh_err, 1);
+    }
+    __syncthreads();
+    if (threadIdx.x == 0) { verdict[0] = sh_redo; verdict[1] = sh_err; }
+}
+
 constexpr int SEL_THREADS = 1024, SEL_WAVES = SEL_THREADS / 64, SEL_D = 128;
 constexpr int SEL_ROUND = SEL_THREADS;
 constexpr int SEL_SAFE = 32;
@@ -204,8 +344,11 @@
 
 __global__ __launch_bounds__(SEL_THREADS) void k_chain_select(const mp3s_chain_seg *__restrict__ segs, const mp3s_select_span *__restrict__ spans,
                                                               int max_reach, const uint8_t *__restrict__ hide,
-                                                              const uint8_t *__restrict__ tabv, const mp3s_gr_out *__restrict__ out,
-                                                              int32_t *__restrict__ cursor, int2 *__restrict__ pairs)
+                                                              const uint8_t *__restrict__ tabv, mp3s_gr_out *out,
+                                                              int32_t *__restrict__ cursor, int2 *pairs,
+                                                              const int16_t *__restrict__ ixv, const int32_t *__restrict__ env,
+                                                              const mp3s_gr_out *__restrict__ outv, int16_t *__restrict__ ix,
+                                                              int32_t *__restrict__ en)
 {
     extern __shared__ uint8_t sel_lds[];
     __shared__ int overflow, d_next, d_try, sat_round;
@@ -310,6 +453,13 @@
         }
         my_pairs[j] = make_int2(src, (int)(u0 + j));
     }
-}
-
-}
+    __threadfence();
+    __syncthreads();
+    if (bad || !ixv) return;
+    for (int j = wave; j < R; j += SEL_WAVES) {
+        const int src = __builtin_amdgcn_readfirstlane(__hip_atomic_load(&my_pairs[j].x, __ATOMIC_RELAXED, __HIP_MEMORY_SCOPE_AGENT));
+        if (src >= 0) scatter_entry(src, u0 + j, lane, ixv, env, outv, ix, en, out);
+    }
+}
+
+}
diff --git a/mp3-steganography-lib_amd/csrc/k_rate.hpp b/mp3-steganography-lib_amd/csrc/k_rate.hpp
--- a/mp3-steganography-lib_amd/csrc/k_rate.hpp
+++ b/mp3-steganography-lib_amd/csrc/k_rate.hpp
@@ -685,16 +685,10 @@
     if (i < n) tables[i] = (uint8_t)outv[i].n_tables;
 }
 
-__global__ __launch_bounds__(256) void k_scatter_entries(const int2 *__restrict__ pairs, int n_pairs, const int16_t *__restrict__ ixv,
-                                                         const int32_t *__restrict__ env, const mp3s_gr_out *__restrict__ outv,
-                                                         int16_t *__restrict__ ix, int32_t *__restrict__ en, mp3s_gr_out *__restrict__ out)
-{
-    const int wave = __builtin_amdgcn_readfirstlane(threadIdx.x >> 6), lane = threadIdx.x & 63;
-    const int j = blockIdx.x * 4 + wave;
-    if (j >= n_pairs) return;
-    const int2 pr = pairs[j];
-    if (pr.x < 0) return;
-    const long src = pr.x, dst = pr.y;
+__device__ __forceinline__ void scatter_entry(long src, long dst, int lane, const int16_t *__restrict__ ixv, const int32_t *__restrict__ env,
+                                              const mp3s_gr_out *__restrict__ outv, int16_t *__restrict__ ix, int32_t *__restrict__ en,
+                                              mp3s_gr_out *out)
+{
     const uint32_t *a = reinterpret_cast<const uint32_t *>(ixv + src * 576);
     uint32_t *b = reinterpret_cast<uint32_t *>(ix + dst * 576);
     for (int i = lane; i < 288; i += 64) b[i] = a[i];
@@ -704,4 +698,16 @@
         reinterpret_cast<uint32_t *>(out + dst)[lane] = reinterpret_cast<const uint32_t *>(outv + src)[lane];
 }
 
-}
+__global__ __launch_bounds__(256) void k_scatter_entries(const int2 *__restrict__ pairs, int n_pairs, const int16_t *__restrict__ ixv,
+                                                         const int32_t *__restrict__ env, const mp3s_gr_out *__restrict__ outv,
+                                                         int16_t *__restrict__ ix, int32_t *__restrict__ en, mp3s_gr_out *__restrict__ out)
+{
+    const int wave = __builtin_amdgcn_readfirstlane(threadIdx.x >> 6), lane = threadIdx.x & 63;
+    const int j = blockIdx.x * 4 + wave;
+    if (j >= n_pairs) return;
+    const int2 pr = pairs[j];
+    if (pr.x < 0) return;
+    scatter_entry(pr.x, pr.y, lane, ixv, env, outv, ix, en, out);
+}
+
+}
diff --git a/mp3-steganography-lib_amd/csrc/mp3s_api.cpp b/mp3-steganography-lib_amd/csrc/mp3s_api.cpp
--- a/mp3-steganography-lib_amd/csrc/mp3s_api.cpp
+++ b/mp3-steganography-lib_amd/csrc/mp3s_api.cpp
@@ -128,13 +128,18 @@
         c->opt[MP3S_OPT_RATE_SIGNALS] = env("MP3S_RATE_SIGNALS", 0) != 0;
         c->opt[MP3S_OPT_PIPE_SIGNALS] = env("MP3S_PIPE_SIGNALS", 0) & 3;
     }
+#ifdef MP3S_ORDER_EVENT_DEVICE_SCOPE
+    const unsigned kOrderEventFlags = hipEventDisableTiming | hipEventDisableSystemFence;
+#else
+    const unsigned kOrderEventFlags = hipEventDisableTiming;
+#endif
     if (hipStreamCreateWithFlags(&c->stream, hipStreamNonBlocking) != hipSuccess ||
         hipEventCreate(&c->ev0) != hipSuccess || hipEventCreate(&c->ev1) != hipSuccess ||
-        hipEventCreateWithFlags(&c->ev_order, hipEventDisableTiming) != hipSuccess) {
+        hipEventCreateWithFlags(&c->ev_order, kOrderEventFlags) != hipSuccess) {
         mp3s_ctx_destroy(c);
         return fail(MP3S_E_NO_DEVICE, "stream/event creation failed");
     }
-    if (hipMalloc((void **)&c->d_sync, 32) != hipSuccess || hipMemsetAsync(c->d_sync, 0, 32, c->stream) != hipSuccess) {
+    if (hipMalloc((void **)&c->d_sync, 64) != hipSuccess || hipMemsetAsync(c->d_sync, 0, 64, c->stream) != hipSuccess) {
         mp3s_ctx_destroy(c);
         return fail(MP3S_E_NO_DEVICE, "device scratch allocation failed");
     }
@@ -363,7 +368,7 @@
         float ms = 0;
         HIPCHK(hipEventElapsedTime(&ms, p.ev[2 * i], p.ev[2 * i + 1]));
         p.total_ms[p.kid[i]] += ms;
-        p.count[p.kid[i]] += 1;
+        p.count[p.kid[i]] += p.kernels[i];
     }
     p.n_pairs = 0;
     if (p.dropped) {
@@ -588,7 +593,7 @@
     if (n_frames <= 0 || n_segs <= 0) return fail(MP3S_E_ARG, "bad sizes");
     void *d_agg = c->grab(30, chain_agg_bytes(n_frames));
     if (!d_agg) return fail(MP3S_E_NOMEM, "hipMalloc failed for the chain scratch");
-    const int e = launch_chain(c->stream, d_gr, d_frames, n_frames, d_segs, d_cursor_in, d_state_in, d_agg, d_verdict, d_seg_out, &c->prof);
+    const int e = launch_chain(c->stream, d_gr, d_frames, n_frames, d_segs, d_cursor_in, d_state_in, d_agg, d_verdict, d_seg_out, &c->prof, nullptr, c->d_sync + mp3s_ctx::kSyncChain);
     if (e) return fail(MP3S_E_HIP, "chain launch: %s", hipGetErrorString((hipError_t)e));
     return MP3S_OK;
 }
@@ -602,7 +607,7 @@
     void *d_agg = c->grab(30, chain_agg_bytes(n_frames));
     if (!d_agg) return fail(MP3S_E_NOMEM, "hipMalloc failed for the chain scratch");
     const ChainRedoArgs redo = {d_mdct, d_hide_bits, n_hide, d_ix, d_en};
-    const int e = launch_chain(c->stream, d_gr, d_frames, n_frames, d_segs, d_cursor, nullptr, d_agg, d_verdict, d_seg_out, &c->prof, &redo);
+    const int e = launch_chain(c->stream, d_gr, d_frames, n_frames, d_segs, d_cursor, nullptr, d_agg, d_verdict, d_seg_out, &c->prof, &redo, c->d_sync + mp3s_ctx::kSyncChain);
     if (e) return fail(MP3S_E_HIP, "chain launch: %s", hipGetErrorString((hipError_t)e));
     return MP3S_OK;
 }
diff --git a/mp3-steganography-lib_amd/csrc/mp3s_device.h b/mp3-steganography-lib_amd/csrc/mp3s_device.h
--- a/mp3-steganography-lib_amd/csrc/mp3s_device.h
+++ b/mp3-steganography-lib_amd/csrc/mp3s_device.h
@@ -18,6 +18,7 @@
     static constexpr int MAX_PAIRS = 8192;
     hipEvent_t ev[2 * MAX_PAIRS];
     int kid[MAX_PAIRS];
+    int kernels[MAX_PAIRS];
     int n_pairs = 0, n_created = 0;
     long dropped = 0;
     bool enabled = false;
@@ -26,6 +27,7 @@
     long count[K_COUNT] = {0};
     int begin(hipStream_t s, int k);
     void end(hipStream_t s, int pair);
+    void launched(int pair, int n) { if (pair >= 0) kernels[pair] = n; }
     bool attach(int k, hipEvent_t *start, hipEvent_t *stop);
 };
 
@@ -67,7 +69,7 @@
 size_t chain_agg_bytes(int n_frames);
 int launch_chain(hipStream_t stream, mp3s_gr_out *d_gr, const mp3s_rate_frame *d_frames, int n_frames, const mp3s_chain_seg *d_segs,
                  const int32_t *d_cursor, const int32_t *d_state, void *d_agg, int32_t *d_verdict, mp3s_chain_seg_out *d_seg_out,
-                 Profiler *prof, const ChainRedoArgs *redo = nullptr);
+                 Profiler *prof, const ChainRedoArgs *redo = nullptr, int32_t *d_look = nullptr);
 
 int launch_select(hipStream_t stream, const mp3s_chain_seg *d_segs, const mp3s_select_span *d_spans, int n_segs, int max_reach,
                   const uint8_t *d_hide, const RateVariantArgs &v, int16_t *d_ix, int32_t *d_en, mp3s_gr_out *d_out, int32_t *d_cursor,
diff --git a/mp3-steganography-lib_amd/csrc/mp3s_device.hip b/mp3-steganography-lib_amd/csrc/mp3s_device.hip
--- a/mp3-steganography-lib_amd/csrc/mp3s_device.hip
+++ b/mp3-steganography-lib_amd/csrc/mp3s_device.hip
@@ -24,6 +24,10 @@
 #include "k_chain.hpp"
 #include "k_wav.hpp"
 
+#ifndef MP3S_TAIL_FUSED
+#define MP3S_TAIL_FUSED 1
+#endif
+
 namespace mp3s {
 
 int Profiler::begin(hipStream_t s, int k)
@@ -34,7 +38,7 @@
         if (hipEventCreate(&ev[n_created]) != hipSuccess) { dropped++; return -1; }
         n_created++;
     }
-    kid[n_pairs] = k;
+    kid[n_pairs] = k; kernels[n_pairs] = 1;
     (void)hipEventRecord(ev[2 * n_pairs], s);
     return n_pairs++;
 }
@@ -50,7 +54,7 @@
         if (hipEventCreate(&ev[n_created]) != hipSuccess) { dropped++; return false; }
         n_created++;
     }
-    kid[n_pairs] = k;
+    kid[n_pairs] = k; kernels[n_pairs] = 1;
     *start = ev[2 * n_pairs]; *stop = ev[2 * n_pairs + 1];
     n_pairs++;
     return true;
@@ -217,23 +221,36 @@
     return (int)hipGetLastError();
 }
 
-static size_t chain_scan_bytes(int n_frames) { return ((size_t)((n_frames + CH_THREADS - 1) / CH_THREADS) * sizeof(ChainEl) + 31) & ~(size_t)15; }
+static size_t chain_scan_bytes(int n_frames) { return CHK_MAX_BLOCKS * sizeof(int2) + (((size_t)((n_frames + CH_THREADS - 1) / CH_THREADS) * sizeof(ChainEl) + 31) & ~(size_t)15); }
 constexpr int kRedoRounds = 1;
 size_t chain_agg_bytes(int n_frames) { return chain_scan_bytes(n_frames) + (size_t)2 * REDO_WORDS * 4; }
 
 int launch_chain(hipStream_t stream, mp3s_gr_out *d_gr, const mp3s_rate_frame *d_frames, int n_frames, const mp3s_chain_seg *d_segs,
                  const int32_t *d_cursor, const int32_t *d_state, void *d_agg, int32_t *d_verdict, mp3s_chain_seg_out *d_seg_out,
-                 Profiler *prof, const ChainRedoArgs *redo)
+                 Profiler *prof, const ChainRedoArgs *redo, int32_t *d_look)
 {
     if (n_frames <= 0) return 0;
     const int blocks = (n_frames + CH_THREADS - 1) / CH_THREADS;
     int32_t *d_redo = redo ? (int32_t *)((uint8_t *)d_agg + chain_scan_bytes(n_frames)) : nullptr;
     int32_t *cursor = const_cast<int32_t *>(d_cursor);
+    int2 *part = (int2 *)d_agg;
+    ChainEl *agg = (ChainEl *)(part + CHK_MAX_BLOCKS);
     const int pp = prof ? prof->begin(stream, K_CHAIN) : -1;
+    if (MP3S_TAIL_FUSED && d_look && blocks <= CHK_MAX_BLOCKS) {
+        static_assert(kRedoRounds == 1, "k_redo_check makes one round");
+        hipLaunchKernelGGL(k_chain_check, dim3(blocks), dim3(CH_THREADS), 0, stream, d_gr, d_frames, d_segs, n_frames, agg, part, cursor, d_state,
+                           d_verdict, d_seg_out, d_redo, reinterpret_cast<ChainLook *>(d_look));
+        if (redo)
+            hipLaunchKernelGGL(k_redo_check, dim3(REDO_GROUPS), dim3(RL_WAVES * 64), 0, stream, redo->d_mdct, d_frames, n_frames, redo->d_hide,
+                               redo->n_hide, d_redo, redo->d_ix, d_gr, redo->d_en, cursor, d_segs, d_verdict, d_seg_out);
+        if (prof) { prof->launched(pp, redo ? 2 : 1); prof->end(stream, pp); }
+        return (int)hipGetLastError();
+    }
+    if (prof) prof->launched(pp, redo ? 2 + 3 * kRedoRounds : 2);
     hipLaunchKernelGGL(k_chain_sum, dim3(blocks), dim3(CH_THREADS), 0, stream, (const mp3s_gr_out *)d_gr, d_frames, d_segs, n_frames,
-                       (ChainEl *)d_agg, d_verdict, d_seg_out, d_redo, (const int32_t *)nullptr);
+                       agg, d_verdict, d_seg_out, d_redo, (const int32_t *)nullptr);
     hipLaunchKernelGGL(k_chain_apply, dim3(blocks), dim3(CH_THREADS), 0, stream, d_gr, d_frames, d_segs, n_frames,
-                       (const ChainEl *)d_agg, cursor, d_state, d_verdict, d_seg_out, d_redo, (const int32_t *)nullptr);
+                       (const ChainEl *)agg, cursor, d_state, d_verdict, d_seg_out, d_redo, (const int32_t *)nullptr);
     if (redo) {
         int32_t *lists[2] = {d_redo, d_redo + REDO_WORDS};
         for (int round = 0; round < kRedoRounds; round++) {
@@ -242,9 +259,9 @@
             hipLaunchKernelGGL(k_rate_redo, dim3(REDO_GROUPS), dim3(RL_WAVES * 64), 0, stream, redo->d_mdct, d_frames, n_frames * 4,
                                redo->d_hide, redo->n_hide, cur, redo->d_ix, d_gr, redo->d_en, (const int32_t *)d_cursor);
             hipLaunchKernelGGL(k_chain_sum, dim3(blocks), dim3(CH_THREADS), 0, stream, (const mp3s_gr_out *)d_gr, d_frames, d_segs, n_frames,
-                               (ChainEl *)d_agg, d_verdict, d_seg_out, nxt, cur);
+                               agg, d_verdict, d_seg_out, nxt, cur);
             hipLaunchKernelGGL(k_chain_apply, dim3(blocks), dim3(CH_THREADS), 0, stream, d_gr, d_frames, d_segs, n_frames,
-                               (const ChainEl *)d_agg, cursor, d_state, d_verdict, d_seg_out, nxt, cur);
+                               (const ChainEl *)agg, cursor, d_state, d_verdict, d_seg_out, nxt, cur);
         }
     }
     if (prof) prof->end(stream, pp);
@@ -258,11 +275,16 @@
     if (n_segs <= 0 || max_reach <= 0 || v.n <= 0) return 0;
     if (max_reach > MP3S_SELECT_MAX_REACH || (int64_t)n_segs * max_reach > 0x3fffffff) return (int)hipErrorInvalidValue;
     const int pp = prof ? prof->begin(stream, K_CHAIN) : -1;
+    const bool own_copy = MP3S_TAIL_FUSED == 1;
     hipLaunchKernelGGL(k_chain_select, dim3(n_segs), dim3(SEL_THREADS), select_lds_bytes(max_reach), stream, d_segs, d_spans, max_reach,
-                       d_hide, (const uint8_t *)v.d_tables, (const mp3s_gr_out *)d_out, d_cursor, (int2 *)d_pairs);
-    const int n_pairs = n_segs * max_reach;
-    hipLaunchKernelGGL(k_scatter_entries, dim3((n_pairs + 3) / 4), dim3(256), 0, stream, (const int2 *)d_pairs, n_pairs,
-                       (const int16_t *)v.d_ix, (const int32_t *)v.d_en, (const mp3s_gr_out *)v.d_out, d_ix, d_en, d_out);
+                       d_hide, (const uint8_t *)v.d_tables, d_out, d_cursor, (int2 *)d_pairs,
+                       own_copy ? (const int16_t *)v.d_ix : (const int16_t *)nullptr, (const int32_t *)v.d_en, (const mp3s_gr_out *)v.d_out, d_ix, d_en);
+    if (!own_copy) {
+        const int n_pairs = n_segs * max_reach;
+        hipLaunchKernelGGL(k_scatter_entries, dim3((n_pairs + 3) / 4), dim3(256), 0, stream, (const int2 *)d_pairs, n_pairs,
+                           (const int16_t *)v.d_ix, (const int32_t *)v.d_en, (const mp3s_gr_out *)v.d_out, d_ix, d_en, d_out);
+        if (prof) prof->launched(pp, 2);
+    }
     if (prof) prof->end(stream, pp);
     return (int)hipGetLastError();
 }
diff --git a/mp3-steganography-lib_amd/csrc/mp3s_encode_pipeline.cpp b/mp3-steganography-lib_amd/csrc/mp3s_encode_pipeline.cpp
--- a/mp3-steganography-lib_amd/csrc/mp3s_encode_pipeline.cpp
+++ b/mp3-steganography-lib_amd/csrc/mp3s_encode_pipeline.cpp
@@ -199,7 +199,7 @@
     if (!rc) {
         const ChainRedoArgs redo = {d_mdct, d_hide, L.n_hide, d.d_ix, d.d_en};
         const int e = launch_chain(ts, d.d_out, d_rf, L.n, d_segs, d_cur, nullptr, d.d_agg, d.d_small,
-                                   (mp3s_chain_seg_out *)((uint8_t *)d.d_small + kSmallHead), &c->prof, !c->opt[MP3S_OPT_REDO] || !L.redo ? nullptr : &redo);
+                                   (mp3s_chain_seg_out *)((uint8_t *)d.d_small + kSmallHead), &c->prof, !c->opt[MP3S_OPT_REDO] || !L.redo ? nullptr : &redo, c->d_sync + mp3s_ctx::kSyncChain);
         if (e) rc = fail(MP3S_E_HIP, "chain launch: %s", hipGetErrorString((hipError_t)e));
     }
     if (!rc) {
diff --git a/mp3-steganography-lib_amd/csrc/mp3s_internal.h b/mp3-steganography-lib_amd/csrc/mp3s_internal.h
--- a/mp3-steganography-lib_amd/csrc/mp3s_internal.h
+++ b/mp3-steganography-lib_amd/csrc/mp3s_internal.h
@@ -42,6 +42,7 @@
     hipEvent_t ev0 = nullptr, ev1 = nullptr, ev_order = nullptr;
     hipEvent_t ev_sel = nullptr; bool sel_pending = false;
     hipEvent_t rate_done = nullptr;
+    static constexpr int kSyncChain = 8;
     int32_t *d_sync = nullptr;
     double synth_eps_scale = 1.0;
     GuardProbe guard_probe = {nullptr, nullptr, 0, 0};
```

Result: slower. 19.12 million frames/s (-1.9%).
